# metasnv-tool/metaSNV

Hardware: AMD Instinct MI355X
Metric: pileup Gbases/s across all samples (higher is better)
Workload: dtype u8

## Files before the change

include/msnv.h:

```cpp
#ifndef MSNV_H
#define MSNV_H

#include <stdint.h>

#ifdef __cplusplus
extern "C" {
#endif

#define MSNV_OK        0
#define MSNV_EINVAL    1
#define MSNV_EIO       2
#define MSNV_EFORMAT   3
#define MSNV_ENODEV    4
#define MSNV_EHIP      5
#define MSNV_ENOMEM    6
#define MSNV_EDOMAIN   7
#define MSNV_ECAPACITY 8

typedef struct msnv_ctx     msnv_ctx;
typedef struct msnv_dataset msnv_dataset;

int         msnv_abi_version(void);
const char *msnv_last_error(void);

// ... 104 lines not shown
                                    const msnv_params *params, msnv_dataset **out);
int  msnv_dataset_attach_ctx(msnv_dataset *ds, msnv_ctx *ctx);
void msnv_dataset_destroy(msnv_dataset *ds);

int  msnv_dataset_set_bed(msnv_dataset *ds, int32_t n, const int32_t *tid, const int64_t *beg, const int64_t *end);
int  msnv_dataset_set_bed_file(msnv_dataset *ds, const char *bed_path);
int  msnv_dataset_set_contig_mask(msnv_dataset *ds, const uint8_t *mask, int32_t n);

int  msnv_dataset_add_sample_records(msnv_dataset *ds, const uint8_t *records, uint64_t n_bytes);
int  msnv_dataset_add_sample_records_many(msnv_dataset *ds, const uint8_t *const *records, const uint64_t *n_bytes, int32_t n, int32_t host_threads);
int  msnv_dataset_add_sample_records_device(msnv_dataset *ds, const void *const *dev_records, const uint64_t *n_bytes, int32_t n);
int  msnv_dataset_add_sample_records_resident(msnv_dataset *ds, void *dev_buffer, uint64_t capacity, const uint64_t *offsets, const uint64_t *n_bytes, int32_t n);
int  msnv_dataset_add_sample_bam(msnv_dataset *ds, const char *bam_path);
int  msnv_dataset_add_sample_bams(msnv_dataset *ds, const char *const *bam_paths, int32_t n, int32_t host_threads);

int  msnv_dataset_stage_sample_bams(msnv_dataset *ds, const char *const *bam_paths, int32_t n, int32_t host_threads);

int  msnv_dataset_pileup_qualities(const msnv_dataset *ds, const uint8_t *records, uint64_t n_bytes, uint8_t *out);

int  msnv_dataset_finalize(msnv_dataset *ds);

typedef struct {
    uint64_t n_samples, n_contigs, n_positions;
    uint64_t n_reads, n_reads_pileup;
    uint64_t n_pileup_bases;
    uint64_t bytes_headers, bytes_cigar, bytes_seq, bytes_qual, bytes_ref, bytes_index;
    uint64_t n_tiles, n_pairs, n_work;
    uint64_t device_bytes;
    uint64_t allele_planes;
    uint64_t sampled_mismatch_ppm;
    uint64_t n_whole_tile_items;
    uint64_t n_listed_tiles;
} msnv_dataset_info;

int  msnv_dataset_info_get(const msnv_dataset *ds, msnv_dataset_info *out);
#define MSNV_PACK_STATS 18
int  msnv_dataset_pack_stats(const msnv_dataset *ds, double *out, int32_t n);
int  msnv_dataset_fetch_column(msnv_dataset *ds, const char *name, uint8_t *out, uint64_t capacity, uint64_t *n_bytes);

typedef struct {
    float    ms_total;
    float    ms_pileup;
    float    ms_gate, ms_gather, ms_decide, ms_coverage;
    uint64_t n_sites;
    uint64_t n_called_pop, n_called_indiv;
    uint64_t n_events, n_overflow;
    uint64_t algorithmic_bytes;
} msnv_run_stats;

int  msnv_pileup_run(msnv_dataset *ds, msnv_run_stats *stats);

int  msnv_pileup_run_many(msnv_dataset *ds, int32_t n, int32_t overlap, msnv_run_stats *stats);
int  msnv_pileup_reserve(msnv_dataset *ds, int32_t n);
int  msnv_coverage_run(msnv_dataset *ds, msnv_run_stats *stats);
int  msnv_fused_run(msnv_dataset *ds, msnv_run_stats *pileup_stats, msnv_run_stats *coverage_stats);
int  msnv_write_coverage(msnv_dataset *ds, int32_t sample_idx, const char *cov_path, const char *detail_path);

typedef struct {
    int32_t        want_median;
    int32_t        window;
    uint32_t       n_regions;
    uint32_t       reserved;
    const int32_t *region_contig;
    const int32_t *region_start;
    const int32_t *region_end;
} msnv_cov_extras;
int  msnv_coverage_extras_run(msnv_dataset *ds, const msnv_cov_extras *what);
int  msnv_coverage_medians(msnv_dataset *ds, int32_t *out, uint64_t capacity);
int  msnv_coverage_window_count(const msnv_dataset *ds, uint64_t *n_windows);
int  msnv_coverage_window_sums(msnv_dataset *ds, int32_t sample_idx, uint64_t *out, uint64_t capacity);
int  msnv_coverage_region_sums(msnv_dataset *ds, uint64_t *out, uint64_t capacity);
int  msnv_coverage_extras_launches(const msnv_dataset *ds, uint32_t *n_launches);
typedef struct { const char *contig; int32_t start, end; const char *alias; } msnv_cov_region;
int  msnv_write_coverage_ex(msnv_dataset *ds, int32_t sample_idx, const char *cov_path, const char *detail_path, const char *profile_path,
                            const char *specific_path, const msnv_cov_region *regions, uint32_t n_regions);
typedef struct {
    const char *bam_path;
    int32_t     max_cov;
    int32_t     min_mapq;
    const char *out_cov_path;
    const char *out_detail_path;
    int32_t     want_median;
    int32_t     window;
    const char *out_profile_path;
    const char *regions_path;
    const char *out_specific_path;
} msnv_cov_ex_args;
int  msnv_coverage_ex(msnv_ctx *ctx, const msnv_cov_ex_args *args);

int  msnv_write_calls(msnv_dataset *ds, const char *called_path, const char *indiv_path,
                      const char *ann_path, const char *fasta_path);

typedef struct {
    int32_t  tid;
    int32_t  pos;
    uint32_t cov;
    uint32_t n[4];
    uint8_t  pop_mask;
    uint8_t  ind_mask;
    uint8_t  refchar;
    uint8_t  dropped;
} msnv_site;

typedef struct { uint16_t cov; uint16_t n[4]; } msnv_site_sample;

#define MSNV_ANN_VALID      1
// ... 104 lines not shown
```

metasnv_amd/_lib.py:

```python
import ctypes as C
import os

from . import knobs

_HERE = os.path.dirname(os.path.abspath(__file__))
LIB_PATH = knobs.library() or os.path.join(_HERE, "csrc", "libmsnv.so")


class MsnvError(RuntimeError):
    def __init__(self, code, msg):
        super().__init__("libmsnv error %d: %s" % (code, msg))
        self.code = code


OK, EINVAL, EIO, EFORMAT, ENODEV, EHIP, ENOMEM, EDOMAIN, ECAPACITY = range(9)
DIV, DIV_NS = 0, 1


class Params(C.Structure):
    _fields_ = [("min_coverage", C.c_int32), ("calling_threshold", C.c_int32), ("min_fraction", C.c_double),
                ("min_baseq", C.c_int32), ("flag_filter", C.c_int32), ("count_orphans", C.c_int32),
                ("max_depth", C.c_int32), ("min_mapq", C.c_int32), ("drop_first_line", C.c_int32),
                ("cov_max", C.c_int32), ("cov_min_mapq", C.c_int32), ("ignore_overlaps", C.c_int32), ("token_limit", C.c_int32)]

# ... 75 lines not shown

class BamData(C.Structure):
    _fields_ = [("n_contigs", C.c_int32), ("names", C.POINTER(C.c_char_p)), ("lengths", C.POINTER(C.c_int64)),
                ("records", C.POINTER(C.c_uint8)), ("n_record_bytes", C.c_uint64), ("header_text", C.c_char_p)]


class SynthParams(C.Structure):
    _fields_ = [("n_species", C.c_int32), ("contig_len", C.c_int64), ("n_samples", C.c_int32), ("read_len", C.c_int32),
                ("mean_cov", C.c_double), ("sigma_cov", C.c_double), ("frac_absent", C.c_double),
                ("snv_density", C.c_double), ("error_rate", C.c_double), ("frac_lowq", C.c_double),
                ("frac_indel_reads", C.c_double), ("frac_clip_reads", C.c_double), ("frac_flagged", C.c_double),
                ("lowercase_ref", C.c_int32), ("seed", C.c_uint64), ("frac_paired", C.c_double),
                ("contigs_per_species_max", C.c_int32), ("species_per_sample", C.c_int32),
                ("frac_aux", C.c_double), ("frac_noseq", C.c_double)]


P = C.POINTER
_vp = C.c_void_p
SYMBOLS = [
    ("msnv_abi_version", C.c_int, []),
    ("msnv_last_error", C.c_char_p, []),
    ("msnv_device_count", C.c_int, []),
    ("msnv_ctx_create", C.c_int, [C.c_int, P(_vp)]),
    ("msnv_ctx_destroy", None, [_vp]),
    ("msnv_params_default", None, [P(Params)]),
    ("msnv_coverage", C.c_int, [_vp, P(CovArgs)]),
    ("msnv_call", C.c_int, [_vp, P(CallArgs)]),
    ("msnv_call_from_mpileup", C.c_int, [_vp, P(MpileupArgs), P(C.c_uint64)]),
    ("msnv_bam_records_many", C.c_int, [_vp, P(C.c_char_p), C.c_int32, C.c_int32, P(P(C.c_uint8)), P(C.c_uint64)]),
    ("msnv_bgzf_inflate", C.c_int, [_vp, C.c_char_p, C.c_int32, P(P(C.c_uint8)), P(C.c_uint64), P(C.c_uint64)]),
    ("msnv_dataset_create", C.c_int, [_vp, P(RefDesc), P(Params), P(_vp)]),
    ("msnv_dataset_create_from_files", C.c_int, [_vp, C.c_char_p, C.c_char_p, P(Params), P(_vp)]),
    ("msnv_dataset_attach_ctx", C.c_int, [_vp, _vp]),
    ("msnv_dataset_set_feed_ctx", C.c_int, [_vp, _vp]),
    ("msnv_dataset_destroy", None, [_vp]),
    ("msnv_dataset_set_bed", C.c_int, [_vp, C.c_int32, P(C.c_int32), P(C.c_int64), P(C.c_int64)]),
    ("msnv_dataset_set_bed_file", C.c_int, [_vp, C.c_char_p]),
    ("msnv_dataset_set_contig_mask", C.c_int, [_vp, P(C.c_uint8), C.c_int32]),
    ("msnv_dataset_add_sample_records", C.c_int, [_vp, _vp, C.c_uint64]),
    ("msnv_dataset_add_sample_records_many", C.c_int, [_vp, P(_vp), P(C.c_uint64), C.c_int32, C.c_int32]),
    ("msnv_dataset_stage_sample_bams", C.c_int, [_vp, P(C.c_char_p), C.c_int32, C.c_int32]),
    ("msnv_dataset_add_sample_records_device", C.c_int, [_vp, P(_vp), P(C.c_uint64), C.c_int32]),
    ("msnv_dataset_add_sample_records_resident", C.c_int, [_vp, _vp, C.c_uint64, P(C.c_uint64), P(C.c_uint64), C.c_int32]),
    ("msnv_dataset_pack_stats", C.c_int, [_vp, P(C.c_double), C.c_int32]),
    ("msnv_dataset_fetch_column", C.c_int, [_vp, C.c_char_p, _vp, C.c_uint64, P(C.c_uint64)]),
    ("msnv_dataset_add_sample_bam", C.c_int, [_vp, C.c_char_p]),
    ("msnv_dataset_add_sample_bams", C.c_int, [_vp, P(C.c_char_p), C.c_int32, C.c_int32]),
    ("msnv_dataset_pileup_qualities", C.c_int, [_vp, _vp, C.c_uint64, _vp]),
    ("msnv_dataset_finalize", C.c_int, [_vp]),
    ("msnv_dataset_info_get", C.c_int, [_vp, P(DatasetInfo)]),
    ("msnv_pileup_run", C.c_int, [_vp, P(RunStats)]),
    ("msnv_pileup_run_many", C.c_int, [_vp, C.c_int32, C.c_int32, P(RunStats)]),
    ("msnv_pileup_reserve", C.c_int, [_vp, C.c_int32]),
    ("msnv_host_cores", C.c_int32, []),
    ("msnv_dataset_deal_bams_device", C.c_int, [_vp, P(C.c_char_p), C.c_int32, C.c_int32, P(C.c_int32), C.c_int32, C.c_int32, C.c_void_p, C.c_uint64, C.c_uint64,
                                                P(C.c_uint64), P(SampleStats), P(C.c_uint64)]),
    ("msnv_dataset_inflate_bams_device", C.c_int, [_vp, P(C.c_char_p), C.c_int32, C.c_int32, C.c_void_p, C.c_uint64, P(C.c_uint64), P(C.c_uint64), P(SampleStats), P(C.c_uint64)]),
    ("msnv_records_deal_device", C.c_int, [_vp, P(C.c_void_p), P(C.c_uint64), C.c_int32, C.c_int32, P(C.c_int32), C.c_int32, C.c_int32, C.c_int32, C.c_void_p, C.c_uint64, C.c_uint64,
                                           P(C.c_uint64), P(SampleStats), P(C.c_uint64)]),
    ("msnv_coverage_run", C.c_int, [_vp, P(RunStats)]),
    ("msnv_fused_run", C.c_int, [_vp, P(RunStats), P(RunStats)]),
    ("msnv_write_coverage", C.c_int, [_vp, C.c_int32, C.c_char_p, C.c_char_p]),
    ("msnv_coverage_extras_run", C.c_int, [_vp, P(CovExtras)]),
    ("msnv_coverage_medians", C.c_int, [_vp, P(C.c_int32), C.c_uint64]),
    ("msnv_coverage_window_count", C.c_int, [_vp, P(C.c_uint64)]),
    ("msnv_coverage_window_sums", C.c_int, [_vp, C.c_int32, P(C.c_uint64), C.c_uint64]),
    ("msnv_coverage_region_sums", C.c_int, [_vp, P(C.c_uint64), C.c_uint64]),
    ("msnv_coverage_extras_launches", C.c_int, [_vp, P(C.c_uint32)]),
    ("msnv_write_coverage_ex", C.c_int, [_vp, C.c_int32, C.c_char_p, C.c_char_p, C.c_char_p, C.c_char_p, P(CovRegion), C.c_uint32]),
    ("msnv_coverage_ex", C.c_int, [_vp, P(CovExArgs)]),
    ("msnv_write_calls", C.c_int, [_vp, C.c_char_p, C.c_char_p, C.c_char_p, C.c_char_p]),
    ("msnv_dataset_first_line", C.c_int, [_vp, P(C.c_int32), P(C.c_int32)]),
    ("msnv_dataset_first_lines", C.c_int, [_vp, P(C.c_int32), P(C.c_int32), C.c_int32]),
    ("msnv_write_calls_records", C.c_int, [P(RefDesc), C.c_int32, P(Site), P(SiteSample), C.c_uint64, C.c_char_p, C.c_char_p, C.c_char_p, C.c_char_p, P(SiteAnn)]),
    ("msnv_records_partition", C.c_int, [_vp, C.c_uint64, P(C.c_int32), C.c_int32, C.c_int32, C.c_int32, _vp, P(C.c_uint64), P(SampleStats)]),
    ("msnv_dataset_sample_stats", C.c_int, [_vp, C.c_int32, P(SampleStats)]),
    ("msnv_coverage_fetch", C.c_int, [_vp, P(C.c_uint64), C.c_uint64]),
    ("msnv_coverage_rows_count", C.c_int, [_vp, P(C.c_uint64)]),
    ("msnv_coverage_fetch_rows", C.c_int, [_vp, P(C.c_uint32), P(C.c_uint32), P(C.c_uint64), C.c_uint64]),
    ("msnv_write_coverage_records", C.c_int, [P(RefDesc), C.c_int32, P(SampleStats), P(C.c_uint64), C.c_char_p, C.c_char_p]),
    ("msnv_annotate_run", C.c_int, [_vp, C.c_char_p, C.c_char_p, P(C.c_double)]),
    ("msnv_results_fetch_ann", C.c_int, [_vp, P(SiteAnn), C.c_uint64]),
    ("msnv_results_count", C.c_int, [_vp, P(C.c_uint64)]),
    ("msnv_results_fetch", C.c_int, [_vp, P(Site), P(SiteSample), C.c_uint64]),
    ("msnv_results_cells_count", C.c_int, [_vp, P(C.c_uint64), P(C.c_uint64)]),
    ("msnv_results_fetch_cells", C.c_int, [_vp, P(Site), P(C.c_uint64), P(C.c_uint32), P(SiteSample), C.c_uint64, C.c_uint64]),
    ("msnv_write_calls_cells", C.c_int, [P(RefDesc), C.c_int32, P(Site), P(C.c_uint64), P(C.c_uint32), P(SiteSample), C.c_uint64, C.c_char_p, C.c_char_p,
                                        C.c_char_p, C.c_char_p, P(SiteAnn)]),
    ("msnv_records_contig_bases", C.c_int, [_vp, C.c_uint64, C.c_int32, P(C.c_uint64)]),
    ("msnv_parse_float", C.c_int, [C.c_char_p, P(C.c_double)]),
    ("msnv_dist_file", C.c_int, [_vp, C.c_char_p, C.c_char_p, C.c_char_p, C.c_double, P(C.c_int32), P(C.c_uint64), P(C.c_double)]),
    ("msnv_div_file", C.c_int, [_vp, C.c_char_p, C.c_int32, C.c_int32, C.c_int64, P(C.c_double), P(C.c_double), C.c_int32, P(C.c_int64),
                                C.c_uint64, C.c_char_p, C.c_char_p, P(C.c_int32), P(C.c_uint64), P(C.c_double)]),
    ("msnv_genotyping_subset", C.c_int, [P(C.c_char_p), C.c_int32, P(C.c_char_p), C.c_int32, C.c_char_p, P(C.c_uint64), P(C.c_uint64)]),
    ("msnv_snv_allele_freq", C.c_int, [_vp, C.c_char_p, C.c_int32, P(C.c_uint64), P(C.c_double)]),
    ("msnv_format_float", C.c_int, [C.c_double, C.c_char_p, C.c_int32]),
    ("msnv_filter_files", C.c_int, [_vp, P(C.c_char_p), C.c_int32, C.c_int32, P(FilterSpecies), C.c_int32, C.c_double, C.c_double,
                                   C.c_char_p, P(C.c_uint64), P(C.c_double)]),
    ("msnv_host_stats", C.c_int, [P(C.c_uint64)]),
    ("msnv_host_timers", C.c_int, [P(C.c_double), C.c_int32, C.c_int32]),
    ("msnv_filter_resident", C.c_int, [_vp, C.c_int32, P(FilterSpecies), C.c_int32, C.c_double, C.c_double, C.c_char_p, C.c_char_p, C.c_char_p,
                                      P(C.c_uint64), P(C.c_double)]),
    ("msnv_bam_write_bed_header", C.c_int, [C.c_char_p, C.c_char_p]),
    ("msnv_bam_read", C.c_int, [C.c_char_p, P(BamData)]),
    ("msnv_bam_read_header", C.c_int, [C.c_char_p, P(BamData)]),
    ("msnv_bam_data_free", None, [P(BamData)]),
# ... 37 lines not shown
```

metasnv_amd/core.py:

```python
import ctypes as C

import numpy as np

from . import _lib
from ._lib import lib, check, Params, SynthParams, DatasetInfo, RunStats, Site, SiteSample, SiteAnn, RefDesc, SampleStats, COV_WORDS

SITE_DTYPE = np.dtype([("tid", "<i4"), ("pos", "<i4"), ("cov", "<u4"), ("n", "<u4", (4,)),
                       ("pop_mask", "u1"), ("ind_mask", "u1"), ("refchar", "u1"), ("dropped", "u1")])
SAMPLE_DTYPE = np.dtype([("cov", "<u2"), ("n", "<u2", (4,))])
ANN_DTYPE = np.dtype([("gene", "<i4"), ("codon", "u1", (4, 8))])
STATS_FIELDS = [n for n, _ in SampleStats._fields_]
assert SITE_DTYPE.itemsize == C.sizeof(Site) and SAMPLE_DTYPE.itemsize == C.sizeof(SiteSample) and ANN_DTYPE.itemsize == C.sizeof(SiteAnn)


def default_params(**kw):
    p = Params()
    lib.msnv_params_default(C.byref(p))
    for k, v in kw.items():
        if not hasattr(p, k):
            raise AttributeError("msnv_params has no field %r" % k)
        setattr(p, k, v)
    return p


# ... 158 lines not shown
        return out

    def add_sample_bam(self, path):
        check(lib.msnv_dataset_add_sample_bam(self._h, path.encode()))
        self.n_samples += 1

    def add_sample_bams(self, paths, host_threads=0):
        arr = _cstr_array(paths)
        check(lib.msnv_dataset_add_sample_bams(self._h, arr, len(paths), host_threads))
        self.n_samples += len(paths)

    def stage_sample_bams(self, paths, host_threads=0):
        arr = _cstr_array(paths)
        check(lib.msnv_dataset_stage_sample_bams(self._h, arr, len(paths), host_threads))
        self.n_samples += len(paths)

    def add_synth_samples(self, synth_p, first, count, host_threads=0):
        check(lib.msnv_dataset_add_synth_samples(self._h, C.byref(synth_p), first, count, host_threads))
        self.n_samples += count

    def finalize(self):
        check(lib.msnv_dataset_finalize(self._h))
        return self.info()

    def info(self):
        i = DatasetInfo()
        check(lib.msnv_dataset_info_get(self._h, C.byref(i)))
        return {k: getattr(i, k) for k, _ in DatasetInfo._fields_}

    PACK_STATS = ["scan_ms", "measure_ms", "depth_ms", "emit_ms", "tile_sort_ms", "upload_wall_s", "download_wall_s", "host_prepass_wall_s",
                  "record_bytes", "records", "pieces", "prepass_samples", "scan_segments_redone", "deep_runs_split", "dense_samples", "quick_rounds_redone", "device_edit_samples",
                  "columns_adopted"]

    def pack_stats(self):
        a = (C.c_double * len(self.PACK_STATS))()
        check(lib.msnv_dataset_pack_stats(self._h, a, len(self.PACK_STATS)))
        return dict(zip(self.PACK_STATS, [float(x) for x in a]))

    def column(self, name):
        n = C.c_uint64()
        check(lib.msnv_dataset_fetch_column(self._h, name.encode(), None, 0, C.byref(n)))
        out = np.zeros(n.value, dtype=np.uint8)
        if n.value:
            check(lib.msnv_dataset_fetch_column(self._h, name.encode(), out.ctypes.data, out.size, C.byref(n)))
        return out

    def run(self):
        st = RunStats()
        check(lib.msnv_pileup_run(self._h, C.byref(st)))
        return {k: getattr(st, k) for k, _ in RunStats._fields_}

    def reserve_passes(self, n):
        check(lib.msnv_pileup_reserve(self._h, int(n)))

    def run_many(self, n, overlap=False):
        arr = (RunStats * n)()
        check(lib.msnv_pileup_run_many(self._h, n, 1 if overlap else 0, arr))
        return [{k: getattr(s, k) for k, _ in RunStats._fields_} for s in arr]

    def coverage_run(self):
        st = RunStats()
        check(lib.msnv_coverage_run(self._h, C.byref(st)))
        return {k: getattr(st, k) for k, _ in RunStats._fields_}

    def fused_run(self):
        sp, sc = RunStats(), RunStats()
        check(lib.msnv_fused_run(self._h, C.byref(sp), C.byref(sc)))
        return ({k: getattr(sp, k) for k, _ in RunStats._fields_}, {k: getattr(sc, k) for k, _ in RunStats._fields_})

    def coverage_accumulators(self):
        acc = np.zeros((max(1, self.n_samples), len(self.names), COV_WORDS), dtype=np.uint64)
        check(lib.msnv_coverage_fetch(self._h, acc.ctypes.data_as(C.POINTER(C.c_uint64)), acc.size))
        return acc

    def coverage_rows(self):
        n = C.c_uint64()
        check(lib.msnv_coverage_rows_count(self._h, C.byref(n)))
        smp, ctg = np.zeros(n.value, dtype=np.uint32), np.zeros(n.value, dtype=np.uint32)
        acc = np.zeros((n.value, COV_WORDS), dtype=np.uint64)
        check(lib.msnv_coverage_fetch_rows(self._h, smp.ctypes.data_as(C.POINTER(C.c_uint32)), ctg.ctypes.data_as(C.POINTER(C.c_uint32)),
                                           acc.ctypes.data_as(C.POINTER(C.c_uint64)), n.value))
        return smp, ctg, acc

    def sample_stats(self, sample_idx):
        st = SampleStats()
        check(lib.msnv_dataset_sample_stats(self._h, sample_idx, C.byref(st)))
        return np.array([getattr(st, k) for k in STATS_FIELDS], dtype=np.uint32)

    def write_coverage(self, sample_idx, cov_path, detail_path, profile_path=None, specific_path=None, regions=None):
        if profile_path is None and specific_path is None and not getattr(self, "_extras_median", False):
            check(lib.msnv_write_coverage(self._h, sample_idx, cov_path.encode(), detail_path.encode()))
            return
        regions = list(regions or [])
        arr = (_lib.CovRegion * max(1, len(regions)))()
        for i, (name, start, end, alias) in enumerate(regions):
            arr[i] = _lib.CovRegion(name.encode(), int(start), int(end), alias.encode())
        check(lib.msnv_write_coverage_ex(self._h, sample_idx, cov_path.encode(), detail_path.encode(),
                                         profile_path.encode() if profile_path is not None else None,
                                         specific_path.encode() if specific_path is not None else None, arr, len(regions)))

    def coverage_extras(self, median=False, window=0, regions=None):
        regions = [(self.names.index(c) if isinstance(c, str) else int(c), int(s), int(e)) for c, s, e in (regions or [])]
        cols = [np.ascontiguousarray([r[k] for r in regions], dtype=np.int32) for k in range(3)]
        what = _lib.CovExtras(1 if median else 0, int(window), len(regions), 0, *[c.ctypes.data_as(C.POINTER(C.c_int32)) for c in cols])
        check(lib.msnv_coverage_extras_run(self._h, C.byref(what)))
        self._extras_median = bool(median)
# ... 318 lines not shown
```

metasnv_amd/csrc/api.cpp:

```cpp
#include <algorithm>
#include <chrono>
#include <climits>
#include <cstring>
#include <stdexcept>
#include <thread>
#include <unordered_map>

#include "bamfeed.h"
#include "devpack.h"
#include "filter.h"

using namespace msnv;

extern "C" int msnv_abi_version(void) { return 3; }

extern "C" void msnv_params_default(msnv_params *p) {
    if (!p) return;
    p->min_coverage = 4; p->calling_threshold = 4; p->min_fraction = 0.01;
    p->min_baseq = 13; p->flag_filter = 0x704; p->count_orphans = 0; p->max_depth = 8000; p->min_mapq = 0;
    p->drop_first_line = 1;
    p->cov_max = 10; p->cov_min_mapq = 1;
    p->ignore_overlaps = 0;
    p->token_limit = 10000;
}
// ... 463 lines not shown
    HostTimerScope ts(HT_UPLOAD_WALL);
    try { return finalize_dataset(*ds); }
    catch (const std::exception &e) { return fail(MSNV_ENOMEM, "building the device dataset failed: %s", e.what()); }
}

extern "C" int msnv_dataset_pack_stats(const msnv_dataset *ds, double *out, int32_t n) {
    clear_error();
    if (!ds || !out || n < 0) return fail(MSNV_EINVAL, "msnv_dataset_pack_stats: bad argument");
    if (devpack_sync_pending(*const_cast<msnv_dataset *>(ds))) clear_error();
    const DevPackTables &t = ds->dp;
    const double v[MSNV_PACK_STATS] = {t.ms_scan, t.ms_measure, t.ms_depth, t.ms_emit, t.ms_sort, t.wall_upload_s, t.wall_download_s, t.wall_prepass_s,
                                       (double)t.raw_bytes, (double)t.n_records, (double)t.n_pieces, (double)t.n_prepass_samples, (double)t.n_scan_redone, (double)t.n_deep_runs_split, (double)t.n_dense_samples, (double)t.n_quick_redone, (double)t.n_device_edit_samples,
                                       (double)t.n_columns_adopted};
    for (int i = 0; i < n; ++i) out[i] = i < MSNV_PACK_STATS ? v[i] : 0.0;
    return MSNV_OK;
}

extern "C" int msnv_dataset_fetch_column(msnv_dataset *ds, const char *name, uint8_t *out, uint64_t capacity, uint64_t *n_bytes) {
    clear_error();
    if (!ds || !name || !n_bytes) return fail(MSNV_EINVAL, "msnv_dataset_fetch_column: NULL argument");
    if (!ds->finalized || !ds->dev) return fail(MSNV_EINVAL, "msnv_dataset_fetch_column: dataset is not finalized");
    if (int rc = dev_set_device(ds->ctx->device)) return rc;
    const DeviceCols &d = *ds->dev;
    const std::string k(name);
    const void *p = nullptr; uint64_t n = 0;
    const uint64_t S = d.n_samples, nt = d.n_tiles;
    if (k == "hdr") { p = d.hdr; n = d.n_reads * sizeof(ReadHdr); }
    else if (k == "hdr4") { p = d.hdr4; n = d.hdr4 ? d.n_reads * 4 : 0; }
    else if (k == "hdr8m") { p = d.hdr8m; n = d.n_hdr8m * sizeof(PieceHdr); }
    else if (k == "blk") { p = d.blk; n = d.blk ? d.n_blk * 4 : 0; }
    else if (k == "seq") { p = d.seq; n = d.n_seq_bytes; }
    else if (k == "qual") { p = d.qual; n = d.n_seq_bytes / 4; }
    else if (k == "s_read_base") { p = d.s_read_base; n = (S + 1) * 8; }
    else if (k == "s_seq_base") { p = d.s_seq_base; n = (S + 1) * 8; }
    else if (k == "ref4") { p = d.ref4; n = (nt * TILE / 8 + 1) * 4; }
    else if (k == "pairs") { p = d.pairs; n = (uint64_t)d.n_pairs * sizeof(TilePair); }
    else if (k == "work") { p = d.work; n = (uint64_t)d.n_work * sizeof(WorkItem); }
    else if (k == "chunks") { p = d.chunks; n = d.n_chunks * sizeof(ChunkDesc); }
    else if (k == "cov_iv") { p = d.cov_iv; n = d.n_cov_iv * sizeof(Pair32); }
    else if (k == "cov_pairs") { p = d.cov_pairs; n = (uint64_t)d.n_cov_pairs * sizeof(TilePair); }
    else if (k == "cov_work") { p = d.cov_work; n = (uint64_t)d.n_cov_work * sizeof(WorkItem); }
    else return fail(MSNV_EINVAL, "msnv_dataset_fetch_column: no column named %s", name);
    *n_bytes = n;
    if (!out) return MSNV_OK;
    if (capacity < n) return fail(MSNV_ECAPACITY, "msnv_dataset_fetch_column: %s holds %llu bytes, capacity %llu", name, (unsigned long long)n, (unsigned long long)capacity);
    if (n && !p) return fail(MSNV_EINVAL, "msnv_dataset_fetch_column: %s is not allocated in this layout", name);
    return dev_download(out, p, n);
}

extern "C" int msnv_dataset_info_get(const msnv_dataset *ds, msnv_dataset_info *out) {
    clear_error();
    if (!ds || !out) return fail(MSNV_EINVAL, "msnv_dataset_info_get: NULL argument");
    *out = ds->info;
    if (ds->dev) { out->n_whole_tile_items = ds->dev->n_fused_tiles; out->n_listed_tiles = ds->dev->last_ovf_tiles; }
    return MSNV_OK;
}

extern "C" int msnv_pileup_reserve(msnv_dataset *ds, int32_t n) {
    clear_error();
    if (!ds || !ds->finalized || n <= 0) return fail(MSNV_EINVAL, "msnv_pileup_reserve: dataset is not finalized or n <= 0");
    if (int rc = dev_set_device(ds->ctx->device)) return rc;
    return dev_reserve_passes(*ds->dev, n);
}

extern "C" int msnv_pileup_run_many(msnv_dataset *ds, int32_t n, int32_t overlap, msnv_run_stats *stats) {
    clear_error();
    if (!ds || !ds->finalized || n <= 0) return fail(MSNV_EINVAL, "msnv_pileup_run_many: dataset is not finalized or n <= 0");
    if (!ds->have_results) return fail(MSNV_EINVAL, "msnv_pileup_run_many: run msnv_pileup_run once first (it sizes the sparse buffers)");
    if (int rc = dev_set_device(ds->ctx->device)) return rc;
    RunCounts c{};
    std::vector<msnv_run_stats> tmp((size_t)n);
    int rc = dev_run_pipeline_many(*ds->dev, ds->params, ds->ctx->stream, n, overlap != 0, tmp.data(), &c);
    if (rc == MSNV_ECAPACITY) return fail(rc, "%s", msnv_last_error());
    if (rc) return rc;
    ds->have_results = true; ds->results_fetched = false; ds->ann_valid = false;
    ds->last_counts_sites = c.n_sites;
    ds->last_stats = tmp.back();
    if (stats) memcpy(stats, tmp.data(), tmp.size() * sizeof(msnv_run_stats));
    return MSNV_OK;
}

static void gpos_to_contig(const msnv_dataset &ds, uint32_t gpos, int32_t &tid, int32_t &pos) {
    const uint32_t tile = gpos / TILE;
    tid = (int32_t)ds.tile_contig[tile];
    pos = (int32_t)(gpos - ds.tile_base[(size_t)tid] * TILE);
}

extern "C" int msnv_pileup_run(msnv_dataset *ds, msnv_run_stats *stats) {
    clear_error();
    if (!ds || !ds->finalized) return fail(MSNV_EINVAL, "msnv_pileup_run: dataset is not finalized");
    if (int rc = dev_set_device(ds->ctx->device)) return rc;
    DeviceCols &d = *ds->dev;
    msnv_run_stats st{};
    RunCounts c{};
    int rc = dev_run_pipeline(d, ds->params, ds->ctx->stream, &st, &c);
    for (int attempt = 0; rc == MSNV_ECAPACITY && attempt < 3; ++attempt) {
        auto grow = [&](void **p, uint32_t &cap, uint32_t need, size_t elem) -> int {
            if (need <= cap) return MSNV_OK;
            dev_free(*p); *p = nullptr;
            cap = (uint32_t)std::min<uint64_t>(0x7fffffffull, (uint64_t)need + need / 4 + 1024);
            return dev_alloc(p, (uint64_t)cap * elem, &d.device_bytes);
        };
        if (int r2 = grow((void **)&d.events, d.cap_events, c.n_events, sizeof(Pair32))) return r2;
        if (int r2 = grow((void **)&d.overflow, d.cap_overflow, c.n_overflow, sizeof(Pair32))) return r2;
        const uint32_t old_cap_sites = d.cap_sites;
        if (int r2 = grow((void **)&d.sites, d.cap_sites, c.n_sites, sizeof(SiteRec))) return r2;
        if (d.cap_sites != old_cap_sites) {
            dev_free(d.unc_sites); d.unc_sites = nullptr;
            if (int r2 = dev_alloc((void **)&d.unc_sites, (uint64_t)d.cap_sites * sizeof(uint32_t), &d.device_bytes)) return r2;
        }
        clear_error();
        rc = dev_run_pipeline(d, ds->params, ds->ctx->stream, &st, &c);
    }
    if (rc == MSNV_ECAPACITY) return fail(rc, "%s", msnv_last_error());
    if (rc) return rc;

    ds->have_results = true;
    ds->results_fetched = false;
    ds->ann_valid = false;
    ds->last_counts_sites = c.n_sites;
    ds->last_stats = st;
    if (stats) *stats = st;
    return MSNV_OK;
}

static int fetch_results(msnv_dataset *ds) {
    if (ds->results_fetched) return MSNV_OK;
    DeviceCols &d = *ds->dev;
    const uint32_t n = ds->last_counts_sites;
    std::vector<SiteRec> sites(n);
    std::vector<uint8_t> flags(n);
    std::vector<uint32_t> tbase(ds->n_tiles + 1), tcnt(ds->n_tiles + 1);
    if (int r2 = dev_download(sites.data(), d.sites, (uint64_t)n * sizeof(SiteRec))) return r2;
    if (int r2 = dev_download(flags.data(), d.site_flags, n)) return r2;
    if (int r2 = dev_download(tbase.data(), d.tile_site_base, (uint64_t)ds->n_tiles * 4)) return r2;
    if (int r2 = dev_download(tcnt.data(), d.tile_site_cnt, (uint64_t)ds->n_tiles * 4)) return r2;
    std::vector<unsigned long long> tcell(ds->n_tiles + 1);
    if (int r2 = dev_download(tcell.data(), d.tile_cell_base, (uint64_t)ds->n_tiles * sizeof(unsigned long long))) return r2;
    const uint64_t n_cells = d.last_cells;
    std::vector<msnv_site_sample> raw((size_t)n_cells);
    {
        std::vector<uint16_t> col((size_t)n_cells);
        if (int r2 = dev_download(col.data(), d.cov_col, col.size() * sizeof(uint16_t))) return r2;
        for (size_t i = 0; i < raw.size(); ++i) raw[i].cov = col[i];
        for (int x = 0; x < 4; ++x) {
            if (int r2 = dev_download(col.data(), d.ncol + (uint64_t)x * d.cap_cells, col.size() * sizeof(uint16_t))) return r2;
            for (size_t i = 0; i < raw.size(); ++i) raw[i].n[x] = col[i];
        }
    }

    ds->sites.clear(); ds->site_samples.clear(); ds->site_dev_index.clear();
    ds->site_row.clear(); ds->site_cell_sample.clear(); ds->site_cells.clear();
    ds->sites.reserve(n);
    ds->site_row.push_back(0);
    for (uint32_t t = 0; t < ds->n_tiles; ++t) {
// ... 620 lines not shown
```

metasnv_amd/csrc/device.h:

```cpp
#pragma once

#include <cstdint>

#include <string>
#include <vector>

#include "dataset.h"

namespace msnv {

struct Pair32 { uint32_t x, y; };
struct MergedGroupDev { uint64_t hdr_base; uint32_t tile, pair_lo, n_pairs, n_pieces; };

constexpr uint8_t ANN_GENE_MINUS = 1, ANN_GENE_LINEAR = 2;
struct AnnGene   { int64_t start; int32_t contig; uint32_t flags; };
struct AnnContig { int64_t cg_base, cg_len; uint32_t goff, pad; };
struct AnnHost {
    std::vector<uint32_t> seg_beg, seg_end;
    std::vector<int32_t>  seg_gene;
    std::vector<AnnGene>  genes;
    std::vector<AnnContig> contigs;
    std::vector<uint8_t>  codons;
};
struct AnnDev {
    uint32_t *seg_beg = nullptr, *seg_end = nullptr; int32_t *seg_gene = nullptr;
    AnnGene *genes = nullptr; AnnContig *contigs = nullptr; uint8_t *codons = nullptr;
    uint32_t n_seg = 0;
    msnv_site_ann *out = nullptr; uint64_t cap_out = 0;
    uint32_t *err = nullptr;
    bool ready = false;
    std::string key;
    std::vector<std::string> gene_names;
};
int  ann_build(msnv_dataset &ds, const Annotation &an, AnnHost &h);
void ann_gene_names(const Annotation &an, const std::vector<std::string> &contigs, std::vector<std::string> &out);
int  dev_ann_upload(DeviceCols &d, const AnnHost &h);
int  dev_annotate(DeviceCols &d, uint32_t n_sites, uint32_t drop_gpos, void *stream, double *ms, uint32_t err_gpos[2]);

struct DeviceCols {
    ReadHdr  *hdr = nullptr;
    PieceHdr *hdr8 = nullptr;
    uint32_t *hdr4 = nullptr;
    PieceHdr *hdr8m = nullptr;
    uint32_t *tile_pair_merged = nullptr;
    uint32_t  n_work_merged = 0;
    MergedGroupDev *merged_groups = nullptr; uint32_t n_merged_groups = 0;
    uint32_t *blk = nullptr;
    bool      dense = true;
    uint8_t  *seq = nullptr;
    uint8_t  *qual = nullptr;
    uint64_t *s_read_base = nullptr, *s_seq_base = nullptr;
    uint32_t *ref4 = nullptr;
    uint32_t *ref_lc = nullptr;
    TilePair *pairs = nullptr;
    uint32_t *tile_pair_start = nullptr;
    WorkItem *work = nullptr;
    ChunkDesc *chunks = nullptr;
    uint32_t *tile_vbeg = nullptr, *tile_vend = nullptr;
    uint32_t  n_tiles = 0, n_pairs = 0, n_work = 0, n_work_narrow = 0, n_samples = 0;
    uint64_t  n_reads = 0, n_seq_bytes = 0, n_chunks = 0, n_hdr8m = 0, n_blk = 0;
    uint32_t *tot = nullptr;
    uint32_t *active_tiles = nullptr;
    uint32_t  n_active_tiles = 0;
    uint8_t  *part = nullptr;
    uint64_t *slot_off = nullptr;
    uint32_t *tile_slot_u16 = nullptr;
    uint32_t *tile_slot_wide = nullptr;
    uint64_t  part_bytes = 0;
    uint32_t *tile_slot_start = nullptr;
    uint8_t  *spill = nullptr;
    uint8_t  *aspill = nullptr;
    bool      allele_planes = false;
    Pair32   *events = nullptr;
    Pair32   *overflow = nullptr;
    uint32_t *counters = nullptr;
    uint32_t  cnt_parity = 0;
    uint32_t *ind4 = nullptr;
    uint32_t *unc_bits = nullptr;
    uint32_t *tile_dirty = nullptr;
    uint32_t *unc_sites = nullptr;
    struct GateTileH { uint32_t tile, slot_lo, slot_16, slot_w, slot_hi, vbeg, vend, n_slots; uint64_t row0; uint32_t tot_mode, staged, pair_lo, n_plane_pairs, pad0, pad1; } *gate_tiles = nullptr;
    unsigned long long *site_row = nullptr;
    GateTileH *gate_tiles_dense = nullptr, *gate_tiles_staged = nullptr;
    uint32_t *gather_tiles = nullptr; uint32_t n_gather_tiles = 0;
    TileStage *tile_stage = nullptr;
    uint32_t *tile_stage_idx = nullptr;
    uint32_t  max_group_pairs = 0;
    uint32_t  n_groups_solo = 0;
    uint32_t  n_work_fused = 0;
    uint32_t  n_fused_tiles = 0;
    bool      fuse_disabled = false;
    int       qlow_cutoff = 0;
    uint32_t  last_ovf_tiles = 0;
    bool      wide_tot = false;
    bool      use_dirty = false;
    uint32_t  gather_split = 4;
    bool      any_split = false;
    unsigned long long *site_bits = nullptr;
    uint32_t *site_rank = nullptr;
    uint32_t  cap_events = 0, cap_overflow = 0, cap_sites = 0;
    SiteRec  *sites = nullptr;
    uint32_t *tile_site_base = nullptr, *tile_site_cnt = nullptr;
    uint32_t *tile_nslots = nullptr;
    unsigned long long *tile_cell_base = nullptr;
    uint64_t  cap_cells = 0, last_cells = 0;
    uint16_t *ncol = nullptr;
    uint16_t *cov_col = nullptr;
    uint8_t  *site_flags = nullptr;
    uint8_t  *site_elig = nullptr;
    uint64_t  cap_out_sites = 0, last_sites = 0;
    Pair32   *cov_iv = nullptr;
    uint64_t *s_cov_base = nullptr;
    TilePair *cov_pairs = nullptr;
    WorkItem *cov_work = nullptr;
    uint32_t *tile_len = nullptr;
    uint32_t *tile_contig_dev = nullptr;
    unsigned long long *cov_acc = nullptr;
    uint64_t  n_cov_rows = 0;
    uint32_t  cov_copies = 1;
    uint32_t  n_cov_pairs = 0, n_cov_work = 0, n_cov_work_wide = 0, n_contigs = 0;
    uint64_t  n_cov_iv = 0;
    uint64_t  device_bytes = 0;
    uint64_t  algorithmic_bytes = 0;
    std::vector<std::pair<void *, uint64_t>> blocks;
    AnnDev    ann;
    struct AltBufs {
        uint32_t *tot = nullptr; uint8_t *part = nullptr; uint8_t *spill = nullptr, *aspill = nullptr; Pair32 *events = nullptr, *overflow = nullptr;
        TileStage *tile_stage = nullptr;
        uint32_t *counters = nullptr; SiteRec *sites = nullptr; uint32_t *tile_site_base = nullptr, *tile_site_cnt = nullptr; unsigned long long *tile_cell_base = nullptr;
        uint16_t *ncol = nullptr; uint16_t *cov_col = nullptr; uint8_t *site_flags = nullptr, *site_elig = nullptr; uint32_t *ind4 = nullptr, *unc_bits = nullptr, *tile_dirty = nullptr, *unc_sites = nullptr; unsigned long long *site_row = nullptr; unsigned long long *site_bits = nullptr; uint32_t *site_rank = nullptr;
        uint32_t cap_events = 0, cap_overflow = 0, cap_sites = 0, cnt_parity = 0; uint64_t cap_out_sites = 0, cap_cells = 0;
    } alt;
    void     *stream2 = nullptr;
    std::vector<void *> event_pool;
    uint32_t *pinned_cnt = nullptr; size_t pinned_cnt_cap = 0;
    void     *timing_events[6] = {nullptr, nullptr, nullptr, nullptr, nullptr, nullptr};
};

constexpr uint32_t EV_LISTS = 32, EV_CNT_STRIDE = 16;
constexpr uint32_t CNT_CELLS = 16 + EV_LISTS * EV_CNT_STRIDE;
constexpr uint32_t CNT_TALLY = CNT_CELLS + 16;
constexpr uint32_t CNT_UNC = CNT_TALLY + 16;
constexpr uint32_t CNT_STAGE = CNT_UNC + 8;
constexpr uint32_t CNT_WORDS = CNT_UNC + 16;

struct RunCounts { uint32_t n_events, n_overflow, n_sites, err; uint64_t n_cells; };

int  dev_set_device(int device);
uint32_t dev_resident_workgroups(uint32_t per_cu);
int  dev_alloc(void **p, uint64_t bytes, uint64_t *acct);
void dev_free(void *p);
void dev_free_batch(const std::vector<void *> &ptrs);
int dev_memset_async(void *dst, int v, uint64_t bytes, void *stream);
void dev_cache_trim();
int  dev_upload(void *dst, const void *src, uint64_t bytes);
int  dev_download(void *dst, const void *src, uint64_t bytes);
int  dev_copy_bytes(void *dst_device, const void *src, uint64_t bytes, bool src_on_device, void *stream);
int  dev_memset(void *dst, int v, uint64_t bytes);
int  dev_stream_wait(void *stream);
int  dev_stream_create(void **stream);
void dev_stream_destroy(void *stream);

constexpr int COV_BINS = 16;
int  dev_run_coverage(DeviceCols &d, int max_cov, void *stream, msnv_run_stats *stats);
int  dev_coverage_scanned(DeviceCols &d, void *stream, unsigned long long *scanned);
constexpr uint32_t CX_BINS = 2048, CX_ROW_WORDS = CX_BINS + 2;
struct CovxRegion { uint32_t start, end, max_end, id; };
struct CovxJob {
    bool want_median = false; uint32_t window = 0, n_samples = 0;
    std::vector<uint32_t> contig_tile_base;
    std::vector<uint32_t> row_contig;
    std::vector<uint64_t> row_len, row_scanned, row_win_off;
    std::vector<CovxRegion> regs; std::vector<uint32_t> reg_off;
    std::vector<int32_t> row_median; std::vector<uint64_t> win, reg_sum;
    uint32_t n_launches = 0;
};
int  dev_run_coverage_extras(DeviceCols &d, CovxJob &job, void *stream);
int  dev_run_pipeline(DeviceCols &d, const msnv_params &p, void *stream, msnv_run_stats *stats, RunCounts *counts);
int  dev_run_pipeline_many(DeviceCols &d, const msnv_params &p, void *stream, int n, bool overlap, msnv_run_stats *stats, RunCounts *counts);
void dev_free_all(DeviceCols &d);
int  dev_reserve_passes(DeviceCols &d, int n);
void warm_devpack(void *stream), warm_kernels(void *stream), warm_textcall(void *stream), warm_annotate(void *stream);

struct InfBlock { unsigned long long in_off, out_off; uint32_t in_size, out_size; };
int  dev_inflate_staging(msnv_ctx *ctx, uint64_t in_bytes, uint64_t out_bytes, uint8_t **in, uint8_t **out);
void dev_inflate_release(msnv_ctx *ctx);
void dev_inflate_release_device(msnv_ctx *ctx);
int  dev_inflate(msnv_ctx *ctx, uint64_t comp_bytes, const std::vector<InfBlock> &blocks, uint64_t out_bytes, std::vector<uint32_t> &status, double *ms_kernel);
int  dev_inflate_device_buffers(msnv_ctx *ctx, uint64_t in_bytes, uint64_t out_bytes);
int  dev_inflate_resident(msnv_ctx *ctx, const uint8_t *host_in, uint64_t comp_bytes, const std::vector<InfBlock> &blocks, const std::vector<uint32_t> &blk_in_file,
                          uint32_t check_every, std::vector<uint32_t> &status, double *ms_kernel);
int  dev_inflate_patch(msnv_ctx *ctx, uint64_t out_off, const uint8_t *data, uint32_t n);

int  text_call(msnv_ctx *ctx, const char *text, uint64_t n_text, const msnv_params &p, const char *ref_fasta, const char *ann_path,
               const char *called_path, const char *indiv_path, uint64_t stats[8]);
int  dist_file(msnv_ctx *ctx, const char *freq_path, const char *mann_path, const char *allele_path, double threshold,
               int32_t *n_samples_out, uint64_t *n_pos_out, double *ms_kernel);
int  div_file(msnv_ctx *ctx, const char *freq_path, int32_t mode, int32_t matched, int64_t genome_length, const double *h, const double *v,
              int32_t n_cov, const int64_t *row_order, uint64_t n_order, const char *out_a, const char *out_b, int32_t *n_samples_out,
              uint64_t *n_rows_out, double *ms_kernel);
int dev_dist(const double *xt_host, int n_samples, long n_pos, double threshold, void *stream, double *mann, double *allele, double *ms_kernel);
int dev_div(const double *xs, const uint64_t *bits, long n_single, long n_words, const double *xg, const long *goff, long n_groups, long n_grouped,
            int n_samples, void *stream, double *out, double *ms_kernel);
int dev_allele_freq(const std::vector<uint32_t> &cov, const std::vector<uint32_t> &cnt, const std::vector<uint32_t> &row_line,
                    uint32_t n_samples, long long min_depth, void *stream, std::vector<double> &freq, double *ms_kernel);

}
```

metasnv_amd/csrc/kernels.hip:

```cpp
#include <hip/hip_runtime.h>

#include <algorithm>
#include <cstdio>
#include <cstdlib>
#include <cstring>
#include <mutex>
#include <unordered_map>
#include <vector>

#include "device.h"

namespace msnv {

#define HIP_TRY(expr)                                                                         \
    do {                                                                                      \
        hipError_t e_ = (expr);                                                               \
        if (e_ != hipSuccess) return fail(MSNV_EHIP, "%s failed: %s", #expr, hipGetErrorString(e_)); \
    } while (0)

constexpr int LANES_PER_READ = 8;
static_assert(LANES_PER_READ * 16 == SEG_MAX, "segment pieces are sized for 8 lanes of 16 bases");

struct PileupArgs {
    const ReadHdr  *hdr;
    const uint32_t *blk;
    const PieceHdr *hdr8;
    const uint32_t *hdr4;
    const PieceHdr *hdr8m;
    uint32_t        n_narrow;
    const uint8_t  *seq;
    const uint8_t  *qual;
    const uint64_t *s_read_base, *s_seq_base;
    const uint32_t *ref4;
    const TilePair *pairs;
    const WorkItem *work;
    const ChunkDesc *chunks;
    uint32_t       *tot;
    uint8_t        *part;
    uint64_t        npos;
    uint8_t        *spill;
    uint8_t        *aspill;
    Pair32         *events;   uint32_t cap_events;
    Pair32         *overflow; uint32_t cap_overflow;
    uint32_t       *counters;
    uint32_t       *ev_count;
    uint32_t        min_baseq;
    uint32_t       *ind4;
    uint32_t       *unc_bits;
    uint32_t       *slot_dirty;
    uint32_t        min_snvs;
    uint32_t        n_fused_lo;
    int             min_cov; double min_frac;
    const uint32_t *ref_lc, *tile_vbeg, *tile_vend, *tile_stage_idx;
    TileStage      *tile_stage;
    uint32_t       *stage_ovf;
};

__device__ __forceinline__ uint32_t allele_index(uint32_t code) {
    return (code == 1u) ? 0u : (code == 2u) ? 1u : (code == 4u) ? 2u : (code == 8u) ? 3u : 4u;
}
__device__ __forceinline__ uint32_t nz_bytes(uint32_t x) {
    return (((x & 0x7f7f7f7fu) + 0x7f7f7f7fu) | x) & 0x80808080u;
}
__device__ __forceinline__ uint32_t count_nz_bytes(const uint4 a, const uint4 b) {
    return (uint32_t)__popc(nz_bytes(a.x) | nz_bytes(a.y) >> 1 | nz_bytes(a.z) >> 2 | nz_bytes(a.w) >> 3 |
                            nz_bytes(b.x) >> 4 | nz_bytes(b.y) >> 5 | nz_bytes(b.z) >> 6 | nz_bytes(b.w) >> 7);
}
__device__ __forceinline__ uint32_t nz_nibbles(uint32_t x) {
    return (((x & 0x77777777u) + 0x77777777u) | x) & 0x88888888u;
}
__device__ __forceinline__ uint32_t nibflags_to_bits(uint32_t f) {
    const uint32_t e = f & 0x08080808u, o = (f >> 4) & 0x08080808u;
    return (__builtin_amdgcn_udot4(o, 0x80200802u, __builtin_amdgcn_udot4(e, 0x40100401u, 0u, false), false)) >> 3;
}
__device__ __forceinline__ uint4 any_uint4() {
    uint4 v;
    asm volatile("" : "=v"(v.x), "=v"(v.y), "=v"(v.z), "=v"(v.w));
    return v;
}
__device__ __forceinline__ uint2 lowq_fetch(const uint8_t *qlow, const uint64_t bit) {
    uint2 v;
    __builtin_memcpy(&v, qlow + (bit >> 3), 8);
    return v;
}
__device__ __forceinline__ uint32_t lowq_bits(const uint2 v, const uint32_t shift) {
    return (uint32_t)(((unsigned long long)v.y << 32 | v.x) >> shift);
}

template <int CTRL, int ROW_MASK>
__device__ __forceinline__ int dpp_add(int x) {
    return x + __builtin_amdgcn_update_dpp(0, x, CTRL, ROW_MASK, 0xf, false);
}
__device__ __forceinline__ int wave_inclusive_scan(int x) {
    x = dpp_add<0x111, 0xf>(x);
    x = dpp_add<0x112, 0xf>(x);
    x = dpp_add<0x114, 0xf>(x);
    x = dpp_add<0x118, 0xf>(x);
    x = dpp_add<0x142, 0xa>(x);
    x = dpp_add<0x143, 0xc>(x);
    return x;
}

__device__ __forceinline__ uint32_t tot_mode_of(const WorkItem &w) { return (w.part_lo >> 1) & 3u; }
__device__ __forceinline__ void tot_add(uint32_t *tot, const uint32_t mode, const uint32_t t0, const uint32_t p, const uint32_t n0, const uint32_t n1,
                                        const uint32_t n2, const uint32_t n3) {
    uint32_t *base = tot + 4ull * t0;
    if (mode == 0u) atomicAdd(base + p, n0 | n1 << 8 | n2 << 16 | n3 << 24);
    else if (mode == 1u) {
        if (n0 | n1) atomicAdd(base + 2u * p, n0 | n1 << 16);
        if (n2 | n3) atomicAdd(base + 2u * p + 1u, n2 | n3 << 16);
    } else {
        if (n0) atomicAdd(base + 4u * p, n0);
        if (n1) atomicAdd(base + 4u * p + 1u, n1);
        if (n2) atomicAdd(base + 4u * p + 2u, n2);
        if (n3) atomicAdd(base + 4u * p + 3u, n3);
    }
}
__device__ __forceinline__ void tot_add_one(uint32_t *tile_tot, const uint32_t mode, const uint32_t p, const uint32_t x, const uint32_t n) {
    const uint32_t shpack = mode == 0u ? 0x18100800u : mode == 1u ? 0x10001000u : 0u;
    const uint32_t byte_off = ((p << mode) + (x >> (2u - mode))) * 4u;
    atomicAdd(reinterpret_cast<uint32_t *>(reinterpret_cast<char *>(tile_tot) + byte_off), n << ((shpack >> (8u * x)) & 0xffu));
}

constexpr int W_NT = 512;
constexpr int W_PPT = TILE / W_NT;
constexpr int W_HCAP = 256;
constexpr int W_EVCAP = 1024;
static_assert(W_PPT == 4, "wide per-sample pass is written for 4 positions per thread");

struct WideLds {
    int32_t  span[TILE + 4];
    uint32_t exc[TILE / 2];
    unsigned long long al[TILE];
    uint32_t ref[TILE / 8 + 4];
    uint4    hdr[2][W_HCAP];
    Pair32   ev[W_EVCAP];
    int32_t  wsum[W_NT / 64];
    uint32_t evn, ev_base;
};

__device__ __forceinline__ void ev_list(PileupArgs &a) {
    const uint32_t k = blockIdx.x % EV_LISTS;
    a.events += (uint64_t)k * a.cap_events;
    a.ev_count = a.counters + 16u + k * EV_CNT_STRIDE;
}

template <typename LDS, int NT, int CAP>
__device__ __forceinline__ void flush_events(LDS &L, const PileupArgs &a, int tid) {
    const uint32_t n = min(L.evn, (uint32_t)CAP);
    if (tid == 0) L.ev_base = n ? atomicAdd(a.ev_count, n) : 0u;
    __syncthreads();
    const uint32_t base = L.ev_base;
    for (uint32_t i = tid; i < n; i += NT)
        if (base + i < a.cap_events) a.events[base + i] = L.ev[i];
    __syncthreads();
    if (tid == 0) L.evn = 0;
}

template <typename LDS, int CAP>
__device__ __forceinline__ void stage_allele_event(LDS &L, const PileupArgs &a, Pair32 e) {
    const uint32_t i = atomicAdd(&L.evn, 1u);
    if (i < (uint32_t)CAP) { L.ev[i] = e; return; }
    const uint32_t g = atomicAdd(a.ev_count, 1u);
    if (g < a.cap_events) a.events[g] = e;
}

__device__ __forceinline__ void wide_classify(WideLds &L, const uint32_t lq, const uint32_t s0, const uint32_t s1,
                                              const uint32_t P0, const uint32_t vmask) {
    const uint32_t pr = P0;
    const uint32_t wi = pr >> 3, sh = (pr & 7u) * 4u;
    const uint32_t w0 = L.ref[wi], w1 = L.ref[wi + 1], w2 = L.ref[wi + 2];
    const uint32_t r0 = __builtin_amdgcn_alignbit(w1, w0, sh), r1 = __builtin_amdgcn_alignbit(w2, w1, sh);
    const uint32_t nm = nibflags_to_bits(nz_nibbles(s0 ^ r0)) | nibflags_to_bits(nz_nibbles(s1 ^ r1)) << 8;
    uint32_t e = (lq | nm) & vmask;
    while (e) {
        const uint32_t j = (uint32_t)__builtin_ctz(e);
        e &= e - 1u;
        const uint32_t p = P0 + j;
        uint32_t ai = 4u;
        if (!((lq >> j) & 1u)) ai = allele_index(((j < 8u ? s0 : s1) >> (4u * (j & 7u))) & 0xfu);
        if (ai < 4u) atomicAdd(&L.al[p], 1ull << (16u * ai));
        else atomicAdd(&L.exc[p >> 1], 1u << (16u * (p & 1u)));
    }
}

__global__ __launch_bounds__(W_NT) void msnv_pileup_tiles_wide(PileupArgs a) {
    ev_list(a);
    __shared__ WideLds L;
    const WorkItem w = a.work[blockIdx.x];
    const uint32_t t0 = w.tile * TILE;
    const int tid = threadIdx.x, lane = tid & 63, wave = tid >> 6;
    const int lane8 = tid & (LANES_PER_READ - 1), grp = tid / LANES_PER_READ;
    const int b0 = 16 * lane8;

    for (int i = tid; i < (int)(TILE / 8 + 4); i += W_NT)
        L.ref[i] = (i < (int)(TILE / 8)) ? a.ref4[(t0 >> 3) + i] : 0xffffffffu;
    for (int i = tid; i < (int)(TILE + 4); i += W_NT) L.span[i] = 0;
    for (int i = tid; i < (int)(TILE / 2); i += W_NT) L.exc[i] = 0;
    for (int i = tid; i < (int)TILE; i += W_NT) L.al[i] = 0;
    if (tid == 0) L.evn = 0;

    uint32_t tc[W_PPT], tn[W_PPT][4];
#pragma unroll
    for (int j = 0; j < W_PPT; ++j) { tc[j] = 0; tn[j][0] = tn[j][1] = tn[j][2] = tn[j][3] = 0; }

    uint32_t k = w.pair_lo;
    TilePair pr = (k < w.pair_hi) ? a.pairs[k] : TilePair{0, 0, 0, 0};
    uint32_t rbeg = pr.read_lo;
    uint4 hreg = make_uint4(0, 0, 0, 0);
    if (k < w.pair_hi && tid < W_HCAP && rbeg + (uint32_t)tid < pr.read_hi)
        hreg = *reinterpret_cast<const uint4 *>(a.hdr + a.s_read_base[pr.sample] + rbeg + tid);
    int buf = 0;

    while (k < w.pair_hi) {
        const uint32_t nrd = min((uint32_t)W_HCAP, pr.read_hi - rbeg);
        const bool last_chunk = rbeg + nrd >= pr.read_hi;
        const uint32_t sample = pr.pad >> 8;
        if (tid < W_HCAP) L.hdr[buf][tid] = hreg;
        uint32_t nk = k, nrbeg = rbeg + nrd;
        TilePair npr = pr;
        if (last_chunk) { nk = k + 1; if (nk < w.pair_hi) { npr = a.pairs[nk]; nrbeg = npr.read_lo; } }
        hreg = make_uint4(0, 0, 0, 0);
        if (nk < w.pair_hi && tid < W_HCAP && nrbeg + (uint32_t)tid < npr.read_hi)
            hreg = *reinterpret_cast<const uint4 *>(a.hdr + a.s_read_base[npr.sample] + nrbeg + tid);
        __syncthreads();

        const uint8_t *seq = a.seq + a.s_seq_base[pr.sample];
        const uint64_t qbit0 = 2ull * a.s_seq_base[pr.sample];
        for (uint32_t r = (uint32_t)grp; r < nrd; r += W_NT / LANES_PER_READ) {
            const uint4 h = L.hdr[buf][r];
            if (!(h.w & META_PILEUP_OK)) continue;
            const uint32_t s = h.x - t0, len = h.z;
            if (lane8 == 0) { atomicAdd(&L.span[s], 1); atomicAdd(&L.span[s + len], -1); }
            const int vhi = min(max((int)len - b0, 0), 16);
            if (vhi <= 0) continue;
            uint2 sv;
            const uint64_t qbit = qbit0 + 2ull * h.y + (uint32_t)b0;
            const uint2 qv = lowq_fetch(a.qual, qbit);
            __builtin_memcpy(&sv, seq + (uint64_t)h.y + (uint32_t)(b0 >> 1), 8);
            wide_classify(L, lowq_bits(qv, (uint32_t)qbit & 7u), sv.x, sv.y, s + (uint32_t)b0, (1u << vhi) - 1u);
        }

// ... 41 lines not shown
                }
            }
            *reinterpret_cast<uint32_t *>(a.spill + (uint64_t)k * TILE + W_PPT * tid) = packed;
        }
        k = nk; pr = npr; rbeg = nrbeg; buf ^= 1;
        if (last_chunk && k < w.pair_hi) {
            __syncthreads();
            if (L.evn >= (uint32_t)(W_EVCAP / 2)) flush_events<WideLds, W_NT, W_EVCAP>(L, a, tid);
        }
    }
    __syncthreads();
    flush_events<WideLds, W_NT, W_EVCAP>(L, a, tid);

    *reinterpret_cast<uint4 *>(a.part + ((uint64_t)w.part_hi << 32 | (w.part_lo & ~15u)) + 4u * W_PPT * tid) = make_uint4(tc[0], tc[1], tc[2], tc[3]);
    bool any_allele = false;
#pragma unroll
    for (int j = 0; j < W_PPT; ++j) {
        if (tn[j][0] | tn[j][1] | tn[j][2] | tn[j][3]) {
            tot_add(a.tot, tot_mode_of(w), t0, W_PPT * tid + j, tn[j][0], tn[j][1], tn[j][2], tn[j][3]);
            any_allele = true;
        }
    }
    if (any_allele && tot_mode_of(w) != 0u) atomicOr(&a.slot_dirty[w.slot], 1u << ((W_PPT * (uint32_t)tid) >> 6));
}

__device__ __forceinline__ unsigned long long spread_bits(const uint32_t byte) {
    return (unsigned long long)(__umul24(byte >> 4, 0x00204081u) & 0x01010101u) << 32 | (__umul24(byte & 0xfu, 0x00204081u) & 0x01010101u);
}

constexpr int N_NT = 256;
constexpr int N_PPT = TILE / N_NT;
constexpr int N_HCAP = CHUNK_READS;
#if !defined(MSNV_N_EVCAP)
#define MSNV_N_EVCAP 224
#endif
#if !defined(MSNV_N32_WAVES)
#define MSNV_N32_WAVES 8
#endif
constexpr int N_EVCAP = MSNV_N_EVCAP;

static_assert(N_PPT == 8, "narrow per-sample pass is written for 8 positions per thread");

struct alignas(16) NarrowLds {
    uint32_t start[TILE / 4 + 4];
    uint32_t end[TILE / 4 + 4];
    unsigned long long exc[TILE / 8 + 4];
    uint32_t al[TILE];
    uint32_t ref[TILE / 8 + 4];
    uint2    hdr[2][N_HCAP];
    Pair32   ev[N_EVCAP];
    ChunkDesc desc[MAX_CHUNKS_PER_ITEM];
    uint32_t carry[N_NT / 64 + 1];
    uint32_t evn, ev_base;
    uint32_t emask[SEQ_ALIGN_LOG2 < 3 ? 33 : 1];
};

template <typename LDS, int EXC_PAD, bool MERGED = false, bool FUSED = false, bool DA = false>
__device__ __forceinline__ void narrow_pass(LDS &L, const PileupArgs &a, uint32_t (&tc)[N_PPT / 2], bool &dirty, const uint32_t t0,
                                            const int tid, const int lane, const int wave, const uint32_t sample, const uint32_t k,
                                            const uint32_t split, const uint32_t tmode) {
    const uint2 st = *reinterpret_cast<uint2 *>(&L.start[2 * tid]);
    const uint2 en = *reinterpret_cast<uint2 *>(&L.end[2 * tid]);
    const uint2 ex = *reinterpret_cast<uint2 *>(&L.exc[EXC_PAD + tid]);
    int d = (int)L.carry[wave];
    *reinterpret_cast<uint2 *>(&L.start[2 * tid]) = make_uint2(0u, 0u);
    *reinterpret_cast<uint2 *>(&L.end[2 * tid]) = make_uint2(0u, 0u);
    L.exc[EXC_PAD + tid] = 0ull;
    if (lane == 0) L.carry[wave] = 0u;
    if (tid == 0) L.end[TILE / 4] = 0;
    const int mine = (int)(__builtin_amdgcn_udot4(st.x, 0x01010101u, __builtin_amdgcn_udot4(st.y, 0x01010101u, 0u, false), false)) -
                     (int)(__builtin_amdgcn_udot4(en.x, 0x01010101u, __builtin_amdgcn_udot4(en.y, 0x01010101u, 0u, false), false));
    d += wave_inclusive_scan(mine) - mine;
    const uint32_t v0 = ((uint32_t)d + st.x - en.x) * 0x01010101u;
    const uint32_t v1 = ((v0 >> 24) + st.y - en.y) * 0x01010101u;
    const uint32_t c0 = v0 - ex.x, c1 = v1 - ex.y;
    tc[0] += c0 & 0x00ff00ffu; tc[1] += (c0 >> 8) & 0x00ff00ffu;
    tc[2] += c1 & 0x00ff00ffu; tc[3] += (c1 >> 8) & 0x00ff00ffu;
    if (!MERGED) *reinterpret_cast<uint2 *>(a.spill + (uint64_t)k * TILE + N_PPT * tid) = make_uint2(c0, c1);
    if (MERGED && FUSED) {
        *reinterpret_cast<uint2 *>(&L.start[2 * tid]) = make_uint2(c0, c1);
        return;
    }
    if constexpr (DA && !MERGED) {
        uint32_t *row = reinterpret_cast<uint32_t *>(a.aspill) + (uint64_t)k * TILE + N_PPT * tid;
        const uint32_t ge = (0x80u - min(a.min_snvs, 127u)) * 0x01010101u;
#pragma unroll
        for (uint32_t half = 0; half < 2u; ++half) {
            const uint4 v = *reinterpret_cast<uint4 *>(&L.al[N_PPT * tid + 4u * half]);
            const uint32_t w4[4] = {v.x, v.y, v.z, v.w};
            *reinterpret_cast<uint4 *>(row + 4u * half) = v;
            if (!(v.x | v.y | v.z | v.w)) continue;
            *reinterpret_cast<uint4 *>(&L.al[N_PPT * tid + 4u * half]) = make_uint4(0u, 0u, 0u, 0u);
            dirty = true;
            uint32_t todo = 0;
#pragma unroll
            for (uint32_t j = 0; j < 4u; ++j) todo |= (split ? w4[j] != 0u : ((((w4[j] & 0x7f7f7f7fu) + ge) | w4[j]) & 0x80808080u) != 0u) ? 1u << j : 0u;
            while (todo) {
                const uint32_t j = (uint32_t)__builtin_ctz(todo);
                todo &= todo - 1u;
                const uint32_t word = j == 0u ? w4[0] : j == 1u ? w4[1] : j == 2u ? w4[2] : w4[3];
                const uint32_t gpos = t0 + N_PPT * tid + 4u * half + j;
#pragma unroll
                for (uint32_t x = 0; x < 4u; ++x) {
                    const uint32_t n = (word >> (8u * x)) & 0xffu;
                    if (n >= a.min_snvs) atomicOr(&a.ind4[gpos >> 3], 1u << (4u * (gpos & 7u) + x));
                    else if (n && split) atomicOr(&a.unc_bits[gpos >> 5], 1u << (gpos & 31u));
                }
            }
        }
        return;
    }
    uint32_t pm = 0, myev;
    {
        const uint4 a0 = *reinterpret_cast<uint4 *>(&L.al[N_PPT * tid]);
        const uint4 a1 = *reinterpret_cast<uint4 *>(&L.al[N_PPT * tid + 4]);
        const uint32_t alw[N_PPT] = {a0.x, a0.y, a0.z, a0.w, a1.x, a1.y, a1.z, a1.w};
#pragma unroll
        for (int j = 0; j < N_PPT; ++j) pm |= (alw[j] ? 1u : 0u) << j;
        myev = count_nz_bytes(a0, a1);
    }
    if (!__any(pm != 0u)) return;
    dirty |= pm != 0u;
    if (MERGED) {
        while (pm) {
            const uint32_t j = (uint32_t)__builtin_ctz(pm);
            pm &= pm - 1u;
            const uint32_t word = L.al[N_PPT * tid + j];
            L.al[N_PPT * tid + j] = 0u;
            const uint32_t gpos = t0 + N_PPT * tid + j;
            for (uint32_t m = nz_bytes(word); m; m &= m - 1u) {
                const uint32_t x = (uint32_t)__builtin_ctz(m) >> 3;
                const uint32_t n = (word >> (8u * x)) & 0xffu;
                tot_add_one(a.tot + 4ull * t0, tmode, N_PPT * tid + j, x, n);
                if (n >= a.min_snvs) atomicOr(&a.unc_bits[gpos >> 5], 1u << (gpos & 31u));
            }
        }
        return;
    }
    const uint32_t ei = (uint32_t)wave_inclusive_scan((int)myev);
    uint32_t res = 0;
    if (lane == 63 && ei) {
        uint32_t cur = atomicAdd(&L.evn, 0u);
        for (;;) {
            if (cur + ei > (uint32_t)N_EVCAP) { res = 0x80000000u | atomicAdd(a.ev_count, ei); break; }
            const uint32_t seen = atomicCAS(&L.evn, cur, cur + ei);
            if (seen == cur) { res = cur; break; }
            cur = seen;
        }
    }
    res = (uint32_t)__builtin_amdgcn_readlane((int)res, 63);
    const bool direct = (res & 0x80000000u) != 0u;
    uint32_t slot = (res & 0x7fffffffu) + ei - myev;
    while (pm) {
        const uint32_t j = (uint32_t)__builtin_ctz(pm);
        pm &= pm - 1u;
        const uint32_t word = L.al[N_PPT * tid + j];
        L.al[N_PPT * tid + j] = 0u;
        const uint32_t gpos = t0 + N_PPT * tid + j;
        for (uint32_t m = nz_bytes(word); m; m &= m - 1u) {
            const uint32_t x = (uint32_t)__builtin_ctz(m) >> 3;
            const uint32_t n = (word >> (8u * x)) & 0xffu;
            tot_add_one(a.tot + 4ull * t0, tmode, N_PPT * tid + j, x, n);
            if (n >= a.min_snvs) atomicOr(&a.ind4[gpos >> 3], 1u << (4u * (gpos & 7u) + x));
            else if (split) atomicOr(&a.unc_bits[gpos >> 5], 1u << (gpos & 31u));
            const Pair32 e{gpos, sample << 18 | x << 16 | n};
            if (direct) { if (slot < a.cap_events) a.events[slot] = e; }
            else L.ev[slot] = e;
            ++slot;
        }
    }
}

__device__ __forceinline__ void store_part_row(uint8_t *part, const WorkItem &w, const uint32_t (&tc)[N_PPT / 2], const int tid) {
    uint8_t *row = part + ((uint64_t)w.part_hi << 32 | (w.part_lo & ~15u));
    if (w.part_lo & 1u) {
        const uint32_t lo = (tc[0] & 0xffu) | (tc[1] & 0xffu) << 8 | (tc[0] >> 16 & 0xffu) << 16 | (tc[1] >> 16) << 24;
        const uint32_t hi = (tc[2] & 0xffu) | (tc[3] & 0xffu) << 8 | (tc[2] >> 16 & 0xffu) << 16 | (tc[3] >> 16) << 24;
        *reinterpret_cast<uint2 *>(row + N_PPT * tid) = make_uint2(lo, hi);
    } else {
        *reinterpret_cast<uint4 *>(row + 2u * N_PPT * tid) =
            make_uint4((tc[0] & 0xffffu) | tc[1] << 16, tc[0] >> 16 | (tc[1] & 0xffff0000u), (tc[2] & 0xffffu) | tc[3] << 16, tc[2] >> 16 | (tc[3] & 0xffff0000u));
    }
}

__device__ __forceinline__ void store_item_dirty(uint32_t *slot_dirty, const WorkItem &w, const bool dirty, const int tid) {
    if (tot_mode_of(w) == 0u) return;
    const unsigned long long b = __ballot(dirty);
    uint32_t byte = 0;
#pragma unroll
    for (int i = 0; i < 8; ++i) byte |= ((b >> (8 * i)) & 0xffull) ? 1u << i : 0u;
    if ((tid & 63) == 0 && byte) atomicOr(&slot_dirty[w.slot], byte << (8 * (tid >> 6)));
}

__device__ __forceinline__ void desc_refill(ChunkDesc *ring, const ChunkDesc *src, const uint32_t c, const uint32_t nch, const int tid) {
    constexpr uint32_t H = MAX_CHUNKS_PER_ITEM / 2;
    if (c == 0u || (c % H) != 0u || c + H >= nch) return;
    const uint32_t first = c + H, n = min(H, nch - first);
    if ((uint32_t)tid < 2u * n) {
        const uint32_t d = first + (uint32_t)tid / 2u;
        reinterpret_cast<uint4 *>(ring + d % MAX_CHUNKS_PER_ITEM)[tid & 1] = reinterpret_cast<const uint4 *>(src + d)[tid & 1];
    }
}

constexpr int N32_LANES = 4;
constexpr int N32_GROUPS = N_NT / N32_LANES;
constexpr int N32_ROUNDS = N_HCAP / N32_GROUPS;
static_assert(N32_LANES * 32 == SEG_MAX && N32_ROUNDS == 2, "narrow32 is written for 128-base pieces, 128-piece chunks");

__device__ __forceinline__ void narrow_classify32(NarrowLds &L, const uint32_t lq_all, const uint4 sq, const uint32_t P0, const int vhi) {
    const uint32_t wi = P0 >> 3, sh = (P0 & 7u) * 4u;
    const uint32_t w0 = L.ref[wi], w1 = L.ref[wi + 1], w2 = L.ref[wi + 2], w3 = L.ref[wi + 3], w4 = L.ref[wi + 4];
    const uint32_t vmask = (vhi >= 32) ? 0xffffffffu : ((1u << vhi) - 1u);
    const uint32_t lq = lq_all & vmask;
    const unsigned long long m = (unsigned long long)lq << (P0 & 7u);
#pragma unroll
    for (int w = 0; w < 5; ++w) {
        const uint32_t byte = (uint32_t)(m >> (8 * w)) & 0xffu;
        if (byte) atomicAdd(&L.exc[wi + w], spread_bits(byte));
    }
// ... 52 lines not shown
#pragma unroll
            for (int x = 0; x < 4; ++x) {
                if ((int)n[x] < (int)a.min_snvs) continue;
                const bool is_pop = (double)n[x] >= lim;
                ok = true;
                if (lc && rc == (1u << x)) continue;
                if (is_pop) pop |= 1u << x;
                else if (a.solo) ind |= 1u << x;
                else elig |= 1u << x;
            }
            if (!ok) continue;
            const uint32_t slot = atomicAdd(&L.evn, 1u);
            if (slot < STAGE_CAP) st->rec[slot] = StageRec{p | (elig ? 1u << 11 : 0u) | (pop | ind << 4) << 16 | elig << 24, cov, word, 0u};
        }
    }
counted:
    __syncthreads();
    const uint32_t n_cand = L.evn;
    if (tid == 0) st->count = n_cand;
    return n_cand > STAGE_CAP;
}

__device__ __attribute__((noinline)) void fused_tile_spill(NarrowLds &L, const FusedSpillArgs a, const uint32_t t0, const int tid) {
    {
        WorkItem w{};
        w.slot = 0u; w.part_lo = a.flags_snvs & 15u; w.part_hi = 0u;
        const uint2 cv = *reinterpret_cast<uint2 *>(&L.start[2 * tid]);
        const uint32_t tc[N_PPT / 2] = {cv.x & 0x00ff00ffu, (cv.x >> 8) & 0x00ff00ffu, cv.y & 0x00ff00ffu, (cv.y >> 8) & 0x00ff00ffu};
        store_part_row(a.row, w, tc, tid);
        const uint32_t tmode = tot_mode_of(w);
        bool dirty = false;
#pragma unroll 1
        for (uint32_t j = 0; j < (uint32_t)N_PPT; ++j) {
            const uint32_t word = L.al[N_PPT * tid + j];
            if (!word) continue;
            dirty = true;
            const uint32_t gpos = t0 + N_PPT * tid + j;
#pragma unroll
            for (uint32_t x = 0; x < 4; ++x) {
                const uint32_t n = (word >> (8u * x)) & 0xffu;
                if (n) {
                    tot_add_one(a.tot + 4ull * t0, tmode, N_PPT * tid + j, x, n);
                    if (n >= (a.flags_snvs >> 4)) atomicOr(&a.unc_bits[gpos >> 5], 1u << (gpos & 31u));
                }
            }
        }
        store_item_dirty(a.item_dirty, w, dirty, tid);
        if (tid == 0) a.stage_ovf[atomicAdd(&a.counters[CNT_STAGE], 1u)] = a.stage_idx;
    }
}

template <bool MERGED, bool FUSED = false, bool DA = false>
__device__ __forceinline__ void pileup_tiles_narrow32_body(PileupArgs a, NarrowLds &L) {
    ev_list(a);
    const WorkItem w = a.work[blockIdx.x];
    const uint32_t t0 = w.tile * TILE;
    const int tid = threadIdx.x, lane = tid & 63, wave = tid >> 6;
    const int lane4 = tid & (N32_LANES - 1), grp = tid / N32_LANES;
    const int b0 = 32 * lane4;

    for (int i = tid; i < (int)(TILE / 8 + 4); i += N_NT)
        L.ref[i] = (i < (int)(TILE / 8)) ? a.ref4[(t0 >> 3) + i] : 0xffffffffu;
    {
        static_assert(offsetof(NarrowLds, start) == 0 && offsetof(NarrowLds, ref) % 16 == 0 && alignof(NarrowLds) >= 16, "the bins are zeroed as 16-byte words");
        constexpr int n16 = (int)(offsetof(NarrowLds, ref) / 16);
        uint4 *z = reinterpret_cast<uint4 *>(&L);
#pragma unroll
        for (int i = 0; i < (n16 + N_NT - 1) / N_NT; ++i) if (i * N_NT + tid < n16) z[i * N_NT + tid] = make_uint4(0u, 0u, 0u, 0u);
    }
    if (tid == 0) L.evn = 0;
    if (tid < N_NT / 64 + 1) L.carry[tid] = 0;
    if constexpr (SEQ_ALIGN_LOG2 < 3) {
        if (tid < 33) {
            uint32_t m = 0;
#pragma unroll
            for (int k = 0; k < 4; ++k) {
                const int c = min(max(tid - 8 * k, 0), 8);
                m |= (c >= 8 ? 0xffffffffu : (1u << (4 * c)) - 1u) & (0x11111111u << k);
            }
            L.emask[tid] = m;
        }
    }
    uint32_t tc[N_PPT / 2] = {0u, 0u, 0u, 0u};
    bool dirty = false;

    const uint32_t nch = w.chunk_hi - w.chunk_lo;
    constexpr bool fused = MERGED && FUSED;
    uint32_t g_sidx = 0, g_vb = 0, g_ve = 0, g_lcb = 0;
    if constexpr (fused) {
        g_sidx = a.tile_stage_idx[w.tile]; g_vb = a.tile_vbeg[w.tile]; g_ve = a.tile_vend[w.tile];
        g_lcb = reinterpret_cast<const uint8_t *>(a.ref_lc)[(t0 >> 3) + (uint32_t)tid];
    }
    constexpr bool H4 = HDR4 && !MERGED;
    auto fetch_hdr = [&](const uint64_t hdr_base) -> uint2 {
        if constexpr (H4) return make_uint2(a.hdr4[hdr_base + (uint32_t)tid], 0u);
        else return *reinterpret_cast<const uint2 *>(a.hdr8 + hdr_base + tid);
    };
    auto put_hdr = [&](const uint32_t buf, const uint2 h) {
        if constexpr (H4) reinterpret_cast<uint32_t *>(L.hdr[buf])[tid] = h.x; else L.hdr[buf][tid] = h;
    };
    auto get_hdr = [&](const uint32_t buf, const uint32_t i) -> uint2 {
        if constexpr (H4) return make_uint2(reinterpret_cast<const uint32_t *>(L.hdr[buf])[i], 0u); else return L.hdr[buf][i];
    };
    uint2 hreg0 = make_uint2(0, 0);
    if (nch && tid < N_HCAP && (uint32_t)tid < (w.first.nrd_flags & 0xffffu)) hreg0 = fetch_hdr(w.first.hdr_base);
    for (uint32_t i = tid; i < min(nch, (uint32_t)MAX_CHUNKS_PER_ITEM) * 2; i += N_NT)
        reinterpret_cast<uint4 *>(L.desc)[i] = reinterpret_cast<const uint4 *>(a.chunks + w.chunk_lo)[i];
    __syncthreads();
// ... 216 lines not shown
                const bool is_pop = (double)n[x] >= lim;
                ok = true;
                if (lc && rc == (1u << x)) continue;
                if (is_pop) pop |= 1u << x;
                else if (solo) ind |= 1u << x;
                else elig |= 1u << x;
            }
            if (ok) {
                const uint32_t slot = atomicAdd(&L.ev_base, 1u);
                if (slot < STAGE_CAP) st->rec[slot] = StageRec{p | (elig ? 1u << 11 : 0u) | (pop | ind << 4) << 16 | elig << 24, cov, word, 0u};
            }
        }
    }
    __syncthreads();
    const uint32_t n_rec = L.ev_base;
    if (n_rec > STAGE_CAP) return false;
    if (tid == 0) st->count = n_rec;
    return true;
}
__global__ __launch_bounds__(N_NT, MSNV_N32_WAVES) void msnv_pileup_tiles_lean(PileupArgs a) {
    __shared__ NarrowLds L;
    a.hdr8 = a.hdr8m;
    a.work += a.n_fused_lo;
    const WorkItem w = a.work[blockIdx.x];
    const uint32_t nch = w.chunk_hi - w.chunk_lo;
    if (nch >= 1u && nch <= LEAN_MAX_CHUNKS && a.min_snvs >= 1u && a.min_snvs <= 127u && lean_tile(a, L, w, nch)) return;
    __syncthreads();
    pileup_tiles_narrow32_body<true, true>(a, L);
}

__global__ __launch_bounds__(N_NT, MSNV_N32_WAVES) void msnv_pileup_tiles_narrow32(PileupArgs a) {
    __shared__ NarrowLds L;
    if (blockIdx.x < a.n_narrow) pileup_tiles_narrow32_body<false>(a, L);
    else if (blockIdx.x < a.n_fused_lo) { a.hdr8 = a.hdr8m; pileup_tiles_narrow32_body<true>(a, L); }
    else { a.hdr8 = a.hdr8m; pileup_tiles_narrow32_body<true, true>(a, L); }
}
__global__ __launch_bounds__(N_NT, MSNV_N32_WAVES) void msnv_pileup_tiles_narrow32_planes(PileupArgs a) {
    __shared__ NarrowLds L;
    if (blockIdx.x < a.n_narrow) pileup_tiles_narrow32_body<false, false, true>(a, L);
    else if (blockIdx.x < a.n_fused_lo) { a.hdr8 = a.hdr8m; pileup_tiles_narrow32_body<true>(a, L); }
    else { a.hdr8 = a.hdr8m; pileup_tiles_narrow32_body<true, true>(a, L); }
}
constexpr int D_PAD = 4;
struct DenseLds {
    uint32_t start[TILE / 4 + 4];
    uint32_t end[TILE / 4 + 4];
    unsigned long long exc[TILE / 8 + D_PAD + 8];
    uint32_t al[TILE];
    uint32_t ref[TILE / 8 + D_PAD + 8];
    Pair32   ev[N_EVCAP];
    ChunkDesc desc[MAX_CHUNKS_PER_ITEM];
    uint32_t carry[N_NT / 64 + 1];
    uint32_t evn, ev_base;
};

__device__ __forceinline__ uint32_t range_nibbles(const int lo, const int hi, const int k) {
    const int h = min(max(hi - 8 * k, 0), 8), l = min(max(lo - 8 * k, 0), 8);
    const uint32_t below_h = (h == 8) ? 0xffffffffu : ((1u << (4 * h)) - 1u);
    const uint32_t below_l = (l == 8) ? 0xffffffffu : ((1u << (4 * l)) - 1u);
    return below_h & ~below_l & 0x88888888u;
}

__device__ __forceinline__ void dense_segment(DenseLds &L, const uint4 sq, const uint32_t lq, const uint32_t P, const int lo, const int hi) {
    const uint32_t wi = P >> 3, sh = (P & 7u) * 4u;
    const uint32_t below_hi = (hi >= 32) ? 0xffffffffu : ((1u << hi) - 1u);
    const uint32_t below_lo = (lo >= 32) ? 0xffffffffu : ((1u << lo) - 1u);
    const uint32_t lqm = lq & below_hi & ~below_lo;
    const unsigned long long m = (unsigned long long)lqm << (P & 7u);
#pragma unroll
    for (int w = 0; w < 5; ++w) {
        const uint32_t byte = (uint32_t)(m >> (8 * w)) & 0xffu;
        if (byte) atomicAdd(&L.exc[wi + w], spread_bits(byte));
    }
    const uint32_t w0 = L.ref[wi], w1 = L.ref[wi + 1], w2 = L.ref[wi + 2], w3 = L.ref[wi + 3], w4 = L.ref[wi + 4];
    const uint32_t sw[4] = {sq.x, sq.y, sq.z, sq.w};
    const uint32_t rw[4] = {__builtin_amdgcn_alignbit(w1, w0, sh), __builtin_amdgcn_alignbit(w2, w1, sh),
                            __builtin_amdgcn_alignbit(w3, w2, sh), __builtin_amdgcn_alignbit(w4, w3, sh)};
    uint32_t e[4];
#pragma unroll
    for (int k = 0; k < 4; ++k) e[k] = nz_nibbles(sw[k] ^ rw[k]) & range_nibbles(lo, hi, k);
    uint32_t E = (e[0] >> 3) | (e[1] >> 2) | (e[2] >> 1) | e[3];
    while (E) {
        const uint32_t b = (uint32_t)__builtin_ctz(E);
        E &= E - 1u;
        const uint32_t k = b & 3u, j = (b >> 2) + 8u * k;
        const unsigned long long pair = (k & 2u) ? ((unsigned long long)sw[3] << 32 | sw[2]) : ((unsigned long long)sw[1] << 32 | sw[0]);
        if ((lq >> j) & 1u) continue;
        const uint32_t code = (uint32_t)(pair >> (((b & 1u) << 5) | (b & 28u))) & 0xfu;
        const uint32_t pp = P + j;
        if ((code & (code - 1u)) == 0u) atomicAdd(&L.al[pp - 32u], __umul24(code, 0x00204081u) & 0x01010101u);
        else atomicAdd(&L.exc[pp >> 3], 1ull << (8u * (pp & 7u)));
    }
}

__global__ __launch_bounds__(N_NT) void msnv_pileup_tiles_dense(PileupArgs a) {
    ev_list(a);
    __shared__ DenseLds L;
    const WorkItem w = a.work[blockIdx.x];
    const uint32_t t0 = w.tile * TILE;
    const int tid = threadIdx.x, lane = tid & 63, wave = tid >> 6;

    for (int i = tid; i < (int)(TILE / 8 + D_PAD + 8); i += N_NT) {
        const int r = i - D_PAD;
        L.ref[i] = (r >= 0 && r < (int)(TILE / 8)) ? a.ref4[(t0 >> 3) + r] : 0xffffffffu;
        L.exc[i] = 0;
    }
    for (int i = tid; i < (int)(TILE / 4 + 4); i += N_NT) { L.start[i] = 0; L.end[i] = 0; }
    for (int i = tid; i < (int)TILE; i += N_NT) L.al[i] = 0;
    if (tid == 0) L.evn = 0;
    if (tid < N_NT / 64 + 1) L.carry[tid] = 0;
    uint32_t tc[N_PPT / 2] = {0u, 0u, 0u, 0u};
    bool dirty = false;

    const uint32_t nch = w.chunk_hi - w.chunk_lo;
    for (uint32_t i = tid; i < min(nch, (uint32_t)MAX_CHUNKS_PER_ITEM) * 2; i += N_NT)
        reinterpret_cast<uint4 *>(L.desc)[i] = reinterpret_cast<const uint4 *>(a.chunks + w.chunk_lo)[i];
    __syncthreads();
    constexpr int ROUNDS = DENSE_CHUNK_BLOCKS / N_NT;
    uint32_t dnext[ROUNDS];
#pragma unroll
    for (int r = 0; r < ROUNDS; ++r) {
        dnext[r] = BLK_EMPTY;
        if (nch && (uint32_t)(r * N_NT + tid) < (L.desc[0].nrd_flags & 0xffffu)) dnext[r] = a.blk[L.desc[0].hdr_base + (uint32_t)(r * N_NT + tid)];
    }

    for (uint32_t c = 0; c < nch; ++c) {
        const ChunkDesc cd = L.desc[c % MAX_CHUNKS_PER_ITEM];
        const bool last_chunk = (cd.nrd_flags >> 16) != 0u;
        const uint32_t nblk = cd.nrd_flags & 0xffffu;
        uint32_t dcur[ROUNDS];
#pragma unroll
        for (int r = 0; r < ROUNDS; ++r) {
            dcur[r] = dnext[r];
            dnext[r] = BLK_EMPTY;
            if (c + 1 < nch && (uint32_t)(r * N_NT + tid) < (L.desc[(c + 1) % MAX_CHUNKS_PER_ITEM].nrd_flags & 0xffffu))
                dnext[r] = a.blk[L.desc[(c + 1) % MAX_CHUNKS_PER_ITEM].hdr_base + (uint32_t)(r * N_NT + tid)];
        }
        __syncthreads();
        desc_refill(L.desc, a.chunks + w.chunk_lo, c, nch, tid);
        if (L.evn >= (uint32_t)(N_EVCAP / 2)) flush_events<DenseLds, N_NT, N_EVCAP>(L, a, tid);

        const uint8_t *seq = a.seq + cd.seq_base;
        const uint64_t qbit0 = 2ull * cd.seq_base;
        uint4 sq[ROUNDS]; uint2 ql[ROUNDS];
#pragma unroll
        for (int r = 0; r < ROUNDS; ++r) {
            const uint32_t b = (uint32_t)(r * N_NT + tid);
            sq[r] = any_uint4(); ql[r] = make_uint2(0u, 0u);
            if (b < nblk) {
                ql[r] = lowq_fetch(a.qual, qbit0 + 32ull * b);
                sq[r] = *reinterpret_cast<const uint4 *>(seq + 16ull * b);
// ... 52 lines not shown
    if (tail0 + 2u * tid < n) *reinterpret_cast<uint16_t *>(p + tail0 + 2u * tid) = 0;
}

template <int NT>
__device__ __forceinline__ void zero_cells(uint16_t *ncol, uint16_t *cov_col, const unsigned long long cap_cells, const unsigned long long first, const unsigned long long n, const uint32_t tid) {
    if (n <= (unsigned long long)NT) {
        if (tid < (uint32_t)n) {
#pragma unroll
            for (int x = 0; x < 4; ++x) ncol[(uint64_t)x * cap_cells + first + tid] = 0;
            cov_col[first + tid] = 0;
        }
        return;
    }
#pragma unroll
    for (int x = 0; x < 4; ++x) zero_span<NT>(reinterpret_cast<uint8_t *>(ncol + (uint64_t)x * cap_cells + first), n * sizeof(uint16_t), tid);
    zero_span<NT>(reinterpret_cast<uint8_t *>(cov_col + first), n * sizeof(uint16_t), tid);
}

struct GateTile { uint32_t tile, slot_lo, slot_16, slot_w, slot_hi, vbeg, vend, n_slots; uint64_t row0; uint32_t tot_mode, staged, pair_lo, n_plane_pairs, pad0, pad1; };

struct GateArgs {
    uint32_t *tot; const uint8_t *part; const uint64_t *slot_off; const uint32_t *tile_slot_start, *tile_slot_u16, *tile_slot_wide; uint64_t npos;
    const uint32_t *tile_vbeg, *tile_vend; int min_cov, min_snvs; double min_frac;
    uint32_t *ind4, *unc_bits;
    const uint32_t *ref4, *ref_lc;
    unsigned long long *site_bits; uint32_t *site_rank; SiteRec *sites; uint32_t cap_sites; uint32_t *counters, *counters_next;
    uint32_t *tile_site_base, *tile_site_cnt; const uint32_t *active_tiles;
    uint16_t *ncol; uint16_t *cov_col; uint8_t *site_flags; uint32_t cap_out;
    const uint32_t *tile_nslots; unsigned long long *tile_cell_base; unsigned long long cap_cells;
    const GateTile *gate_tiles; uint32_t *tile_dirty; uint32_t *unc_sites; uint32_t use_dirty; unsigned long long *block_row;
    uint8_t *site_elig; uint32_t any_split;
    uint32_t n_active, tiles_per_wg;
    const TileStage *tile_stage;
    const uint8_t *aspill;
    uint32_t zero_next;
    const uint32_t *tile_list;
    uint32_t solo_cells;
};

constexpr uint32_t GATE_STAGE = 384;
constexpr uint32_t GATE_MAX_TILES = 8;
struct GateStageTile { uint32_t tile, site_rel, total, n_slots; unsigned long long cell_rel; };
struct GateLds {
    SiteRec  rec[GATE_STAGE];
    uint16_t fl[GATE_STAGE];
    uint8_t  unc[GATE_STAGE];
    uint32_t blk_rel[GATE_MAX_TILES][TILE / 64];
    GateStageTile tiles[GATE_MAX_TILES];
    uint32_t wave[GATE_NT / 64];
    uint32_t pop, ind, base;
    unsigned long long cell;
};

__device__ __forceinline__ void gate_flush(GateLds &L, const GateArgs &a, const uint32_t n_tiles, const uint32_t n_sites, const unsigned long long n_cells, const int tid) {
    if (n_tiles == 0u) return;
    if (tid == 0) {
        L.base = atomicAdd(&a.counters[2], n_sites);
        L.cell = atomicAdd(reinterpret_cast<unsigned long long *>(&a.counters[CNT_CELLS]), (n_cells + 7ull) & ~7ull);
    }
    __syncthreads();
    const uint32_t base = L.base; const unsigned long long cb = L.cell;
    if ((uint32_t)tid < n_tiles) {
        const GateStageTile t = L.tiles[tid];
        a.tile_site_base[t.tile] = base + t.site_rel; a.tile_site_cnt[t.tile] = t.total; a.tile_cell_base[t.tile] = cb + t.cell_rel;
    }
    if ((unsigned long long)base + n_sites <= a.cap_out && cb + n_cells <= a.cap_cells) {
        zero_cells<GATE_NT>(a.ncol, a.cov_col, a.cap_cells, cb, n_cells, (uint32_t)tid);
    }
    if ((uint32_t)tid < n_tiles * (TILE / 64)) {
        const uint32_t k = (uint32_t)tid / (TILE / 64), blk = (uint32_t)tid % (TILE / 64);
        const GateStageTile t = L.tiles[k];
        const uint32_t rel = L.blk_rel[k][blk];
        a.site_rank[(uint64_t)t.tile * (TILE / 64) + blk] = base + rel;
        a.block_row[(uint64_t)t.tile * (TILE / 64) + blk] = cb + t.cell_rel + (unsigned long long)(rel - t.site_rel) * t.n_slots;
    }
    for (uint32_t i = (uint32_t)tid; i < n_sites; i += GATE_NT) {
        const uint32_t idx = base + i;
        if (idx >= a.cap_sites) continue;
        a.sites[idx] = L.rec[i];
        if (idx < a.cap_out) { a.site_flags[idx] = (uint8_t)(L.fl[i] & 0xffu); a.site_elig[idx] = (uint8_t)(L.fl[i] >> 8); }
        if (L.unc[i]) {
            const uint32_t u = atomicAdd(&a.counters[CNT_UNC], 1u);
            if (u < a.cap_sites) a.unc_sites[u] = idx;
        }
    }
    __syncthreads();
}

template <bool MULTI, bool WIDE_TOT, bool PLANES = false>
__global__ __launch_bounds__(GATE_NT) void msnv_gate_sites(const GateArgs a) {
    constexpr int NN = WIDE_TOT ? 4 * GATE_PPT : 2 * GATE_PPT;
    constexpr int ROWS = MULTI ? 8 : 16;
    uint32_t *const tot = a.tot; const uint8_t *const part = a.part;
    const int min_cov = a.min_cov, min_snvs = a.min_snvs; const double min_frac = a.min_frac;
    unsigned long long *const site_bits = a.site_bits; SiteRec *const sites = a.sites;
    const uint32_t cap_sites = a.cap_sites; uint32_t *const counters = a.counters;
    uint16_t *const cov_col = a.cov_col;
    const uint32_t cap_out = a.cap_out;
    __shared__ GateLds L;
    const int tid = threadIdx.x, lane = tid & 63, wave = tid >> 6;
    const uint32_t p0 = (uint32_t)GATE_PPT * (uint32_t)tid;
    if (tid == 0) { L.pop = 0; L.ind = 0; }
    if (blockIdx.x == 0 && a.zero_next) for (uint32_t i = threadIdx.x; i < CNT_WORDS; i += GATE_NT) a.counters_next[i] = 0u;
    const bool listed = MULTI && a.tile_list != nullptr;
    const uint32_t ti_step = listed ? gridDim.x : 1u;
    const uint32_t ti_lo = listed ? blockIdx.x : MULTI ? blockIdx.x * a.tiles_per_wg : blockIdx.x;
    const uint32_t ti_hi = listed ? min(a.counters[CNT_STAGE], a.n_active) : MULTI ? min(a.n_active, ti_lo + a.tiles_per_wg) : ti_lo + 1u;
    if (MULTI && ti_lo >= ti_hi) return;
    auto tile_at = [&](const uint32_t ti) -> GateTile { return a.gate_tiles[listed ? a.tile_list[ti] : ti]; };
    uint32_t st_tiles = 0, st_sites = 0; unsigned long long st_cells = 0;
    GateTile gt_next = tile_at(ti_lo);
    for (uint32_t ti = ti_lo; ti < ti_hi; ti += ti_step) {
        const GateTile gt = gt_next;
        if (ti + ti_step < ti_hi) gt_next = tile_at(ti + ti_step);
        const uint32_t tile = gt.tile;
        const uint32_t t0 = tile * TILE;
        const uint32_t vb = gt.vbeg, ve = gt.vend;
        const uint64_t g0 = (uint64_t)t0 + p0;

        const uint32_t slot_lo = gt.slot_lo, slot_hi = gt.slot_hi;
        const uint32_t slot_16 = gt.slot_16, slot_w = gt.slot_w;
        const bool solo = MULTI && a.solo_cells && gt.staged == 2u;
        const bool consult = a.use_dirty && gt.tot_mode != 0u;
        uint32_t dirty = 0;
        if (consult) for (uint32_t sl = slot_lo; sl < slot_hi; ++sl) dirty |= a.tile_dirty[sl];
        const bool my_dirty = !consult || ((dirty >> (p0 >> 6)) & 1u);
        uint32_t *const tb = tot + 4ull * t0;
        const uint4 z4 = make_uint4(0u, 0u, 0u, 0u);
        uint4 e0 = z4, e1 = z4;
        if (gt.tot_mode == 0u) { e0 = reinterpret_cast<const uint4 *>(tb + p0)[0]; e1 = reinterpret_cast<const uint4 *>(tb + p0)[1]; }
        const uint32_t ind4w = my_dirty ? a.ind4[g0 >> 3] : 0u;
        const uint32_t uncb = my_dirty ? reinterpret_cast<const uint8_t *>(a.unc_bits)[g0 >> 3] : 0u;
        const uint32_t refw = a.ref4[g0 >> 3];
        const uint32_t lcb = reinterpret_cast<const uint8_t *>(a.ref_lc)[g0 >> 3];
        uint32_t covs[GATE_PPT];
    #pragma unroll
        for (int j = 0; j < GATE_PPT; ++j) covs[j] = 0;
        if (slot_16 > slot_lo) {
            const uint8_t *p8 = part + gt.row0 + p0;
            const uint32_t n8 = slot_16 - slot_lo;
            for (uint32_t r0 = 0; r0 < n8; r0 += 255u) {
                uint32_t h[4] = {0u, 0u, 0u, 0u};
                const uint32_t r1 = min(n8, r0 + 255u);
                uint32_t s = r0;
                for (; s + (uint32_t)ROWS <= r1; s += (uint32_t)ROWS) {
                    uint2 v[ROWS];
    #pragma unroll
                    for (int u = 0; u < ROWS; ++u) v[u] = *reinterpret_cast<const uint2 *>(p8 + (uint64_t)(s + (uint32_t)u) * TILE);
    #pragma unroll
                    for (int u = 0; u < ROWS; ++u) {
                        h[0] += v[u].x & 0x00ff00ffu; h[1] += (v[u].x >> 8) & 0x00ff00ffu;
                        h[2] += v[u].y & 0x00ff00ffu; h[3] += (v[u].y >> 8) & 0x00ff00ffu;
// ... 87 lines not shown
                        for (int u = 0; u < 4; ++u) {
                            const uint32_t w8[8] = {v[u][0].x, v[u][0].y, v[u][0].z, v[u][0].w, v[u][1].x, v[u][1].y, v[u][1].z, v[u][1].w};
#pragma unroll
                            for (int j = 0; j < GATE_PPT; ++j) { ae[j] += w8[j] & 0x00ff00ffu; ao[j] += (w8[j] >> 8) & 0x00ff00ffu; }
                        }
                    }
                    for (; sidx < r1; ++sidx) {
                        const uint4 *q = reinterpret_cast<const uint4 *>(p32 + (uint64_t)sidx * TILE);
                        const uint4 v0 = q[0], v1 = q[1];
                        const uint32_t w8[8] = {v0.x, v0.y, v0.z, v0.w, v1.x, v1.y, v1.z, v1.w};
#pragma unroll
                        for (int j = 0; j < GATE_PPT; ++j) { ae[j] += w8[j] & 0x00ff00ffu; ao[j] += (w8[j] >> 8) & 0x00ff00ffu; }
                    }
#pragma unroll
                    for (int j = 0; j < GATE_PPT; ++j) {
                        if (WIDE_TOT) { nn[4 * j] += ae[j] & 0xffffu; nn[4 * j + 1] += ao[j] & 0xffffu; nn[4 * j + 2] += ae[j] >> 16; nn[4 * j + 3] += ao[j] >> 16; }
                        else { nn[2 * j] += (ae[j] & 0xffffu) | ao[j] << 16; nn[2 * j + 1] += (ae[j] >> 16) | (ao[j] & 0xffff0000u); }
                    }
                }
            }
        }
        auto n_of = [&](const int j, const int x) -> uint32_t { return WIDE_TOT ? nn[4 * j + x] : (nn[2 * j + (x >> 1)] >> (16 * (x & 1))) & 0xffffu; };
        if (ind4w) a.ind4[g0 >> 3] = 0u;
        if (uncb) reinterpret_cast<uint8_t *>(a.unc_bits)[g0 >> 3] = 0;
        uint32_t okm = 0, uncm = 0, flw[2] = {0u, 0u}, elig[2] = {0u, 0u};
    #pragma unroll
        for (int j = 0; j < GATE_PPT; ++j) {
            const uint32_t p = p0 + (uint32_t)j, cov = covs[j];
            if (cov != 0u && p >= vb && p < ve && (int)cov >= min_cov &&
                (int)(n_of(j, 0) + n_of(j, 1) + n_of(j, 2) + n_of(j, 3)) >= min_snvs) {
                const uint32_t indx = (ind4w >> (4 * j)) & 15u;
                const bool unc = (uncb >> j) & 1u;
                const double lim = (double)(int)cov * min_frac;
                const uint32_t rc = (refw >> (4 * j)) & 15u;
                const bool lc = (lcb >> j) & 1u;
                bool ok = false;
                uint32_t pop = 0, ind = 0;
    #pragma unroll
                for (int x = 0; x < 4; ++x) {
                    if ((int)n_of(j, x) < min_snvs) continue;
                    const bool is_pop = (double)n_of(j, x) >= lim, is_ind = ((indx >> x) & 1u) || (solo && unc);
                    ok |= is_pop || is_ind || unc;
                    if (lc && rc == (1u << x)) continue;
                    if (is_pop) pop |= 1u << x; else if (is_ind) ind |= 1u << x;
                    else if (unc) { uncm |= 1u << j; elig[j >> 2] |= (1u << x) << (8 * (j & 3)); }
                }
                okm |= (ok ? 1u : 0u) << j;
                flw[j >> 2] |= (pop | ind << 4) << (8 * (j & 3));
            }
        }
        {
            unsigned long long w = (unsigned long long)okm << (8u * ((uint32_t)lane & 7u));
            w |= __shfl_xor(w, 1); w |= __shfl_xor(w, 2); w |= __shfl_xor(w, 4);
            if ((lane & 7) == 0) site_bits[g0 >> 6] = w;
        }
        const uint32_t mycnt = (uint32_t)__popc(okm);
        const uint32_t incl = (uint32_t)wave_inclusive_scan((int)mycnt);
        if (lane == 63) L.wave[wave] = incl;
        __syncthreads();
        uint32_t total = 0, mybase = incl - mycnt;
#pragma unroll
        for (int wv = 0; wv < GATE_NT / 64; ++wv) {
            if (wv < wave) mybase += L.wave[wv];
            total += L.wave[wv];
        }
        const uint32_t n_slots = gt.n_slots;
        if (tid == 0 && dirty) for (uint32_t sl = slot_lo; sl < slot_hi; ++sl) a.tile_dirty[sl] = 0u;
        const uint32_t okm_certain = a.any_split ? okm & ~uncm : okm;
        if (okm_certain) {
            uint32_t np = 0, ni = 0;
#pragma unroll
            for (int j = 0; j < GATE_PPT; ++j) { const uint32_t f = ((okm_certain >> j) & 1u) ? (flw[j >> 2] >> (8 * (j & 3))) & 0xffu : 0u; np += (f & 15u) ? 1u : 0u; ni += (f >> 4) ? 1u : 0u; }
            if (np) atomicAdd(&L.pop, np);
            if (ni) atomicAdd(&L.ind, ni);
        }
        if (total == 0u) {
            if (tid == 0) { a.tile_site_base[tile] = 0u; a.tile_site_cnt[tile] = 0u; a.tile_cell_base[tile] = 0ull; }
            __syncthreads();
            continue;
        }
        if (st_sites + total > GATE_STAGE || st_tiles == GATE_MAX_TILES) {
            gate_flush(L, a, st_tiles, st_sites, st_cells, tid);
            st_tiles = 0; st_sites = 0; st_cells = 0;
        }
        if (total <= GATE_STAGE && !solo) {
            if ((n_slots & 7u) == 0u) st_cells = (st_cells + 7ull) & ~7ull;
            if (tid == 0) L.tiles[st_tiles] = GateStageTile{tile, st_sites, total, n_slots, st_cells};
            if ((lane & 7) == 0) L.blk_rel[st_tiles][p0 >> 6] = st_sites + mybase;
            uint32_t i = st_sites + mybase;
#pragma unroll
            for (int j = 0; j < GATE_PPT; ++j) {
                if (okm & (1u << j)) {
                    SiteRec s;
                    s.gpos = (uint32_t)(g0 + (uint32_t)j); s.cov = covs[j];
                    s.n[0] = n_of(j, 0); s.n[1] = n_of(j, 1); s.n[2] = n_of(j, 2); s.n[3] = n_of(j, 3);
                    L.rec[i] = s;
                    L.fl[i] = (uint16_t)(((flw[j >> 2] >> (8 * (j & 3))) & 0xffu) | ((elig[j >> 2] >> (8 * (j & 3))) & 0xffu) << 8);
                    L.unc[i] = (uint8_t)((a.any_split && ((uncm >> j) & 1u)) ? 1u : 0u);
                    ++i;
                }
            }
            ++st_tiles; st_sites += total; st_cells += (unsigned long long)total * n_slots;
            __syncthreads();
            continue;
        }
        if (tid == 0) {
            const uint32_t base = atomicAdd(&counters[2], total);
            L.base = base;
            a.tile_site_base[tile] = base;
            a.tile_site_cnt[tile] = total;
            const unsigned long long cb = atomicAdd(reinterpret_cast<unsigned long long *>(&counters[CNT_CELLS]), ((unsigned long long)total * n_slots + 7ull) & ~7ull);
            L.cell = cb;
            a.tile_cell_base[tile] = cb;
        }
        __syncthreads();
        const uint32_t base = L.base; const unsigned long long s_cell = L.cell;
        const bool fits = (uint64_t)base + total <= cap_out && s_cell + (unsigned long long)total * n_slots <= a.cap_cells;
        if (fits && !solo) {
            const uint64_t n_cells = (uint64_t)total * n_slots;
            zero_cells<GATE_NT>(a.ncol, cov_col, a.cap_cells, s_cell, n_cells, (uint32_t)tid);
        }
        if ((lane & 7) == 0) {
            a.site_rank[g0 >> 6] = base + mybase;
            a.block_row[g0 >> 6] = s_cell + (unsigned long long)mybase * n_slots;
        }
        uint32_t idx = base + mybase;
#pragma unroll
        for (int j = 0; j < GATE_PPT; ++j) {
            if (okm & (1u << j)) {
                if (idx < cap_sites) {
                    SiteRec s;
                    s.gpos = (uint32_t)(g0 + (uint32_t)j); s.cov = covs[j];
                    s.n[0] = n_of(j, 0); s.n[1] = n_of(j, 1); s.n[2] = n_of(j, 2); s.n[3] = n_of(j, 3);
                    sites[idx] = s;
                    if (idx < cap_out) a.site_flags[idx] = (uint8_t)((flw[j >> 2] >> (8 * (j & 3))) & 0xffu);
                    if (idx < cap_out) a.site_elig[idx] = (uint8_t)((elig[j >> 2] >> (8 * (j & 3))) & 0xffu);
                    if (a.any_split && ((uncm >> j) & 1u)) {
                        const uint32_t u = atomicAdd(&counters[CNT_UNC], 1u);
                        if (u < cap_sites) a.unc_sites[u] = idx;
                    }
                    if (solo && fits) {
                        const unsigned long long cell = s_cell + (idx - base);
#pragma unroll
                        for (int x = 0; x < 4; ++x) a.ncol[(uint64_t)x * a.cap_cells + cell] = (uint16_t)s.n[x];
                        cov_col[cell] = (uint16_t)s.cov;
                    }
                }
                ++idx;
            }
        }
        __syncthreads();
    }
    gate_flush(L, a, st_tiles, st_sites, st_cells, tid);
    __syncthreads();
    if (tid == 0 && (L.pop | L.ind)) atomicAdd(reinterpret_cast<unsigned long long *>(&counters[CNT_TALLY]), (unsigned long long)L.pop | (unsigned long long)L.ind << 32);
}

constexpr int GS_WAVES = 4;
constexpr int GS_TILES = 16;
__global__ __launch_bounds__(64 * GS_WAVES) void msnv_gate_staged(const GateArgs a, const GateTile *__restrict__ tiles, const uint32_t n_tiles) {
    __shared__ uint32_t s_sites[GS_WAVES]; __shared__ unsigned long long s_cells[GS_WAVES];
    __shared__ uint32_t s_base, s_np, s_ni; __shared__ unsigned long long s_cb;
    const int lane = threadIdx.x & 63, wave = threadIdx.x >> 6;
    const uint32_t w0 = (blockIdx.x * (uint32_t)GS_WAVES + (uint32_t)wave) * (uint32_t)GS_TILES;
    if (blockIdx.x == 0 && a.zero_next) for (uint32_t i = threadIdx.x; i < CNT_WORDS; i += 64 * GS_WAVES) a.counters_next[i] = 0u;
    if (threadIdx.x == 0) { s_np = 0; s_ni = 0; }
    const uint32_t n_here = w0 < n_tiles ? min((uint32_t)GS_TILES, n_tiles - w0) : 0u;
    GateTile gt{};
    uint32_t cnt = 0;
    bool mine = (uint32_t)lane < n_here;
    if (mine) {
        gt = tiles[w0 + (uint32_t)lane]; cnt = a.tile_stage[gt.row0].count;
        if (cnt > STAGE_CAP) { mine = false; cnt = 0u; }
    }
    const unsigned long long cells = (unsigned long long)cnt * gt.n_slots;
    uint32_t site_rel = cnt; unsigned long long cell_rel = cells;
#pragma unroll
    for (int o = 1; o < GS_TILES; o <<= 1) {
        const uint32_t t = (uint32_t)__shfl_up((int)site_rel, o); const unsigned long long u = (unsigned long long)__shfl_up((long long)cell_rel, o);
        if (lane >= o) { site_rel += t; cell_rel += u; }
    }
    const uint32_t tot_sites = (uint32_t)__shfl((int)site_rel, GS_TILES - 1); const unsigned long long tot_cells = (unsigned long long)__shfl((long long)cell_rel, GS_TILES - 1);
    site_rel -= cnt; cell_rel -= cells;
    if (lane == 0) { s_sites[wave] = tot_sites; s_cells[wave] = tot_cells; }
    __syncthreads();
    if (threadIdx.x == 0) {
        uint32_t ts = 0; unsigned long long tc = 0;
        for (int k = 0; k < GS_WAVES; ++k) { ts += s_sites[k]; tc += s_cells[k]; }
        s_base = ts ? atomicAdd(&a.counters[2], ts) : 0u;
        s_cb = ts ? atomicAdd(reinterpret_cast<unsigned long long *>(&a.counters[CNT_CELLS]), (tc + 7ull) & ~7ull) : 0ull;
    }
    __syncthreads();
    uint32_t base = s_base; unsigned long long cb = s_cb;
    uint32_t wg_sites = 0; unsigned long long wg_cells = 0;
    for (int k = 0; k < GS_WAVES; ++k) { if (k < wave) { base += s_sites[k]; cb += s_cells[k]; } wg_sites += s_sites[k]; wg_cells += s_cells[k]; }
    if (mine) { a.tile_site_base[gt.tile] = cnt ? base + site_rel : 0u; a.tile_site_cnt[gt.tile] = cnt; a.tile_cell_base[gt.tile] = cnt ? cb + cell_rel : 0ull; }
    const bool fits = (unsigned long long)s_base + wg_sites <= a.cap_out && s_cb + wg_cells <= a.cap_cells;
    uint32_t np = 0, ni = 0;
    const unsigned long long mine_mask = __ballot(mine);
    for (uint32_t t = 0; t < n_here; ++t) {
        if (!((mine_mask >> t) & 1ull)) continue;
        const uint32_t tile = (uint32_t)__shfl((int)gt.tile, (int)t), n = (uint32_t)__shfl((int)cnt, (int)t), n_slots = (uint32_t)__shfl((int)gt.n_slots, (int)t);
        const uint32_t kind = (uint32_t)__shfl((int)gt.staged, (int)t), srel = (uint32_t)__shfl((int)site_rel, (int)t);
        const unsigned long long crel = (unsigned long long)__shfl((long long)cell_rel, (int)t), sidx = (unsigned long long)__shfl((long long)gt.row0, (int)t);
        StageRec r{0xffffffffu, 0u, 0u, 0u};
        if ((uint32_t)lane < n) r = a.tile_stage[sidx].rec[lane];
        const uint32_t pos = r.pos_flags & (TILE - 1u);
        uint32_t rank = 0, before = 0; unsigned long long word = 0;
// ... 412 lines not shown
#pragma unroll
                    for (uint32_t x = 0; x < 4; ++x) {
                        const uint32_t cnt = (al >> (8u * x)) & 0xffu;
                        if (cnt) a.ncol[(uint64_t)x * a.cells.cap_cells + cell] = (uint16_t)cnt;
                        if (cnt >= a.min_snvs) ind |= 1u << x;
                    }
                    if (ind && a.ind_in_gather) {
                        const uint32_t site = base + j0 + i / m;
                        ind &= a.site_elig[site];
                        if (ind) {
                            uint32_t *wordp = reinterpret_cast<uint32_t *>(a.site_flags + (site & ~3u));
                            const uint32_t sh = 8u * (site & 3u);
                            const uint32_t old = atomicOr(wordp, (ind << 4) << sh);
                            if ((((old >> sh) & 0xffu) >> 4) == 0u) ++my_tally;
                        }
                    }
                }
            }
            sync();
        }
    }
#pragma unroll
    for (int o = 32; o >= 1; o >>= 1) my_tally += (uint32_t)__shfl_xor((int)my_tally, o);
    if ((tid & 63u) == 0u && my_tally) atomicAdd(reinterpret_cast<unsigned long long *>(&a.counters[CNT_TALLY]), (unsigned long long)my_tally << 32);
}
__device__ __forceinline__ void gather_merged_block(const TailArgs &a, const uint32_t bid, uint32_t *s_pool) {
    if (a.merged_per_block == 1u) { gather_merged_group<256, GM_CELLS, MERGE_MAX_PAIRS, GM_HITS>(a, a.merged_groups[bid], s_pool, threadIdx.x); return; }
    const uint32_t gi = bid * GMW_GROUPS + (threadIdx.x >> 6);
    if (gi < a.n_merged_run) gather_merged_group<64, GMW_CELLS, GMW_PAIRS, GMW_HITS>(a, a.merged_groups[gi], s_pool + (threadIdx.x >> 6) * GMW_WORDS, threadIdx.x & 63u);
}
static bool merged_wave_form(const DeviceCols &d) {
    const int forced = knob::merged_gather();
    return d.max_group_pairs <= GMW_PAIRS && forced != 1;
}

template <bool HAS_MERGED>
__global__ __launch_bounds__(256) void msnv_gather_scatter(TailArgs a) {
    const uint32_t n_scatter = a.scatter_blocks * EV_LISTS;
    if (blockIdx.x == gridDim.x - 1u) {
        if (threadIdx.x < 64) {
            const uint32_t c = threadIdx.x < EV_LISTS ? a.counters[16u + threadIdx.x * EV_CNT_STRIDE] : 0u;
            unsigned long long total = c; uint32_t fullest = c;
#pragma unroll
            for (int o = 32; o >= 1; o >>= 1) { total += __shfl_xor(total, o); fullest = max(fullest, (uint32_t)__shfl_xor((int)fullest, o)); }
            if (fullest > a.cap_list) total = (unsigned long long)fullest * EV_LISTS;
            if (threadIdx.x == 0) a.counters[0] = (uint32_t)min(total, 0xffffffffull);
        }
        return;
    }
    __shared__ __attribute__((aligned(16))) uint32_t s_pool[TAIL_POOL_WORDS];
    if (blockIdx.x < n_scatter) { if (!(a.debug_skip & 1u)) scatter_events_block(a, blockIdx.x % a.scatter_blocks, blockIdx.x / a.scatter_blocks); }
    else if (HAS_MERGED && blockIdx.x < n_scatter + a.n_merged_blocks) { if (!(a.debug_skip & 4u)) gather_merged_block(a, blockIdx.x - n_scatter, s_pool); }
    else if (!(a.debug_skip & 2u)) gather_cov_block(a, blockIdx.x - n_scatter - a.n_merged_blocks, s_pool);
}

__global__ __launch_bounds__(256) void msnv_decide_sites(const SiteRec *sites, const uint32_t *unc_sites, uint32_t *counters, uint32_t cap_sites, uint32_t cap_out,
                                                         const uint32_t *ref4, const uint32_t *ref_lc, const uint16_t *ncol,
                                                         const CellMap cells, int min_snvs, double min_frac, uint8_t *site_flags) {
    __shared__ uint32_t s_pop, s_ind;
    if (threadIdx.x == 0) { s_pop = 0; s_ind = 0; }
    __syncthreads();
    const uint32_t n_unc = min(counters[CNT_UNC], cap_sites), n_sites = counters[2];
    const int lane = threadIdx.x & 63;
    if (n_sites <= cap_sites && n_sites <= cap_out && *reinterpret_cast<const unsigned long long *>(&counters[CNT_CELLS]) <= cells.cap_cells) {
        for (uint32_t u = blockIdx.x * (blockDim.x >> 6) + (threadIdx.x >> 6); u < n_unc; u += gridDim.x * (blockDim.x >> 6)) {
            const uint32_t site = unc_sites[u];
            const SiteRec s = sites[site];
            const uint32_t rc = (ref4[s.gpos >> 3] >> (4 * (s.gpos & 7))) & 0xfu;
            const bool lc = (ref_lc[s.gpos >> 5] >> (s.gpos & 31)) & 1u;
            uint32_t pop = 0, ind = 0;
            for (int x = 0; x < 4; ++x) {
                if (lc && rc == (1u << x)) continue;
                const uint32_t nx = s.n[x];
                if ((int)nx < min_snvs) continue;
                if ((double)nx >= (double)(int)s.cov * min_frac) { pop |= 1u << x; continue; }
                bool any = false;
                const uint32_t tile = s.gpos / TILE, n_slots = cells.tile_nslots[tile];
                const uint64_t row = cell_of(cells, tile, site, 0u);
                for (uint32_t i = lane; i < n_slots; i += 64)
                    any |= (int)ncol[(uint64_t)x * cells.cap_cells + row + i] >= min_snvs;
                if (__any(any)) ind |= 1u << x;
            }
            if (lane == 0) {
                site_flags[site] = (uint8_t)(pop | ind << 4);
                if (pop) atomicAdd(&s_pop, 1u);
                if (ind) atomicAdd(&s_ind, 1u);
            }
        }
    }
    __syncthreads();
    if (threadIdx.x == 0) {
        if (s_pop) atomicAdd(&counters[4], s_pop);
        if (s_ind) atomicAdd(&counters[5], s_ind);
    }
}

constexpr int C_NT = 64;
static_assert(C_NT / 64 * COV_PW == COV_ITEM_PAIRS, "coverage work items are sized for COV_PW pairs per wavefront");

__device__ __forceinline__ int wave_reduce_add(int x) {
    x = wave_inclusive_scan(x);
    return __builtin_amdgcn_readlane(x, 63);
}
__device__ __forceinline__ uint32_t row_sum16(uint32_t x) {
    x = (uint32_t)dpp_add<0xB1, 0xf>((int)x);
    x = (uint32_t)dpp_add<0x4E, 0xf>((int)x);
// ... 292 lines not shown
    {
        std::lock_guard<std::mutex> lk(g_cache_mu);
        for (void *p : ptrs) {
            if (!p) continue;
            auto it = g_cache_live.find(p);
            if (it == g_cache_live.end()) { foreign.push_back(p); continue; }
            g_cache_free.push_back(it->second); g_cache_free_bytes += it->second.bytes;
            g_cache_live.erase(it);
        }
    }
    int dev = 0;
    (void)hipGetDevice(&dev);
    const uint64_t cap = cache_cap_bytes(dev);
    {
        std::lock_guard<std::mutex> lk(g_cache_mu);
        while (g_cache_free_bytes > cap && !g_cache_free.empty()) {
            size_t big = 0;
            for (size_t i = 1; i < g_cache_free.size(); ++i) if (g_cache_free[i].bytes > g_cache_free[big].bytes) big = i;
            evict.push_back(g_cache_free[big]); g_cache_free_bytes -= g_cache_free[big].bytes;
            g_cache_free[big] = g_cache_free.back(); g_cache_free.pop_back();
        }
    }
    for (const CacheBlock &e : evict) (void)hipFree(e.p);
    for (void *p : foreign) (void)hipFree(p);
}
int dev_upload(void *dst, const void *src, uint64_t bytes) {
    if (!bytes) return MSNV_OK;
    HIP_TRY(hipMemcpy(dst, src, bytes, hipMemcpyHostToDevice));
    return MSNV_OK;
}
int dev_download(void *dst, const void *src, uint64_t bytes) { if (bytes) HIP_TRY(hipMemcpy(dst, src, bytes, hipMemcpyDeviceToHost)); return MSNV_OK; }
int dev_copy_bytes(void *dst_device, const void *src, uint64_t bytes, bool src_on_device, void *stream) {
    if (!bytes) return MSNV_OK;
    HIP_TRY(hipMemcpyAsync(dst_device, src, bytes, src_on_device ? hipMemcpyDeviceToDevice : hipMemcpyHostToDevice, (hipStream_t)stream));
    HIP_TRY(hipStreamSynchronize((hipStream_t)stream));
    return MSNV_OK;
}
int dev_memset(void *dst, int v, uint64_t bytes) {
    if (bytes) { HIP_TRY(hipMemset(dst, v, bytes)); HIP_TRY(hipStreamSynchronize(nullptr)); }
    return MSNV_OK;
}
int dev_memset_async(void *dst, int v, uint64_t bytes, void *stream) {
    if (bytes) HIP_TRY(hipMemsetAsync(dst, v, bytes, (hipStream_t)stream));
    return MSNV_OK;
}
int dev_stream_wait(void *stream) { HIP_TRY(hipStreamSynchronize((hipStream_t)stream)); return MSNV_OK; }
int dev_stream_create(void **stream) { hipStream_t s; HIP_TRY(hipStreamCreateWithFlags(&s, hipStreamNonBlocking)); *stream = s; return MSNV_OK; }
void dev_stream_destroy(void *stream) { if (stream) (void)hipStreamDestroy((hipStream_t)stream); }

void dev_free_all(DeviceCols &d) {
    void *ptrs[] = {d.hdr, d.hdr8, d.hdr4, d.hdr8m, d.merged_groups, d.tile_pair_merged, d.blk, d.seq, d.qual, d.s_read_base, d.s_seq_base, d.ref4, d.ref_lc, d.pairs,
                    d.tile_pair_start, d.work, d.chunks, d.tile_vbeg, d.tile_vend, d.tot, d.part, d.tile_slot_start, d.tile_slot_u16, d.tile_slot_wide, d.slot_off, d.spill, d.events, d.overflow, d.counters, d.ind4, d.tile_dirty, d.unc_sites, d.site_row, d.gate_tiles,
                    d.sites, d.tile_site_base, d.tile_site_cnt, d.tile_cell_base, d.tile_nslots, d.ncol, d.cov_col, d.site_flags, d.site_elig,
                    d.cov_iv, d.s_cov_base, d.cov_pairs, d.cov_work, d.tile_len, d.tile_contig_dev, d.cov_acc, d.tile_stage, d.tile_stage_idx, d.alt.tile_stage, d.gate_tiles_dense, d.gate_tiles_staged, d.gather_tiles};
    auto in_block = [&](void *p) { for (const auto &b : d.blocks) if ((char *)p >= (char *)b.first && (char *)p < (char *)b.first + b.second) return true; return false; };
    for (void *p : ptrs) if (p && !in_block(p)) dev_free(p);
    void *aptrs[] = {d.ann.seg_beg, d.ann.seg_end, d.ann.seg_gene, d.ann.genes, d.ann.contigs, d.ann.codons, d.ann.out, d.ann.err};
    for (void *p : aptrs) dev_free(p);
    for (void *e : d.timing_events) if (e) (void)hipEventDestroy((hipEvent_t)e);
    for (void *e : d.event_pool) (void)hipEventDestroy((hipEvent_t)e);
    if (d.pinned_cnt) (void)hipHostFree(d.pinned_cnt);
    void *alts[] = {d.aspill, d.alt.aspill, d.alt.tot, d.alt.part, d.alt.spill, d.alt.events, d.alt.overflow, d.alt.counters, d.alt.ind4, d.alt.tile_dirty, d.alt.unc_sites, d.alt.site_row, d.alt.sites, d.alt.tile_site_base,
                    d.alt.tile_site_cnt, d.alt.tile_cell_base, d.alt.ncol, d.alt.cov_col, d.alt.site_flags, d.alt.site_elig, d.alt.site_bits, d.site_bits, d.alt.site_rank, d.site_rank, d.active_tiles};
    for (void *p : alts) if (p && !in_block(p)) dev_free(p);
    for (const auto &b : d.blocks) dev_free(b.first);
    if (d.stream2) (void)hipStreamDestroy((hipStream_t)d.stream2);
    d = DeviceCols{};
}

static int ensure_out(DeviceCols &d, uint64_t n_sites, uint64_t n_cells) {
    if (n_sites > d.cap_out_sites) {
        dev_free(d.site_flags); d.site_flags = nullptr;
        dev_free(d.site_elig); d.site_elig = nullptr;
        const uint64_t cap = std::max<uint64_t>(n_sites + n_sites / 4, 1024);
        if (int rc = dev_alloc((void **)&d.site_flags, cap + 4, &d.device_bytes)) return rc;
        if (int rc = dev_alloc((void **)&d.site_elig, cap + 4, &d.device_bytes)) return rc;
        d.cap_out_sites = cap;
    }
    if (n_cells > d.cap_cells) {
        dev_free(d.ncol); dev_free(d.cov_col);
        d.ncol = nullptr; d.cov_col = nullptr;
        const uint64_t cap = (std::max<uint64_t>(n_cells + n_cells / 4, 1u << 16) + 7) & ~7ull;
        if (int rc = dev_alloc((void **)&d.ncol, 4 * cap * sizeof(uint16_t) + 16, &d.device_bytes)) return rc;
        if (int rc = dev_alloc((void **)&d.cov_col, cap * sizeof(uint16_t) + 16, &d.device_bytes)) return rc;
        d.cap_cells = cap;
    }
    return MSNV_OK;
}

static inline uint32_t *stage_ovf_list(const DeviceCols &d) { return d.tile_stage ? reinterpret_cast<uint32_t *>(d.tile_stage + d.n_active_tiles) : nullptr; }

static int enqueue_pass(DeviceCols &d, const msnv_params &p, hipStream_t st, hipEvent_t ev_begin, hipEvent_t ev_pile0, hipEvent_t ev_pile1,
                        hipEvent_t ev3, hipEvent_t ev4, uint32_t *host_cnt, hipEvent_t wait_before_pileup = nullptr) {
    const uint64_t npos = (uint64_t)d.n_tiles * TILE;
    if (p.min_baseq != d.qlow_cutoff) return fail(MSNV_EINVAL, "the dataset's quality column was packed for -Q %d, the pass asks for -Q %d", d.qlow_cutoff, p.min_baseq);
    if (ev_begin) HIP_TRY(hipEventRecord(ev_begin, st));
    uint32_t *const counters = d.counters + d.cnt_parity * CNT_WORDS, *const counters_next = d.counters + (d.cnt_parity ^ 1u) * CNT_WORDS;
    d.cnt_parity ^= 1u;
    if (wait_before_pileup) HIP_TRY(hipStreamWaitEvent(st, wait_before_pileup, 0));
    const uint32_t use_stage = (d.n_fused_tiles && !d.fuse_disabled && p.calling_threshold >= 1) ? 1u : 0u;
    HIP_TRY(hipEventRecord(ev_pile0, st));
    if (d.n_work) {
        PileupArgs a;
        a.hdr = d.hdr; a.hdr8 = d.hdr8; a.hdr4 = d.hdr4; a.blk = d.blk; a.seq = d.seq; a.qual = d.qual;
        a.s_read_base = d.s_read_base; a.s_seq_base = d.s_seq_base;
        a.ref4 = d.ref4; a.pairs = d.pairs; a.work = d.work; a.chunks = d.chunks; a.tot = d.tot; a.part = d.part; a.npos = npos; a.spill = d.spill; a.aspill = d.aspill;
        a.events = d.events; a.cap_events = d.cap_events / EV_LISTS; a.ev_count = nullptr; a.overflow = d.overflow; a.cap_overflow = d.cap_overflow;
        a.counters = counters; a.min_baseq = (uint32_t)std::max(0, p.min_baseq);
        a.ind4 = d.ind4; a.unc_bits = d.unc_bits; a.slot_dirty = d.tile_dirty; a.min_snvs = (uint32_t)std::max(0, p.calling_threshold);
        a.n_fused_lo = d.n_work_narrow + d.n_work_merged - (use_stage ? d.n_work_fused : 0u); a.min_cov = p.min_coverage; a.min_frac = p.min_fraction; a.ref_lc = d.ref_lc; a.tile_vbeg = d.tile_vbeg; a.tile_vend = d.tile_vend;
        a.tile_stage = d.tile_stage; a.tile_stage_idx = d.tile_stage_idx; a.stage_ovf = stage_ovf_list(d);
        const uint32_t n_narrow = d.n_work_narrow, n_merged = d.n_work_merged;
        a.hdr8m = d.hdr8m; a.n_narrow = n_narrow;
        if (n_narrow && d.dense) hipLaunchKernelGGL(msnv_pileup_tiles_dense, dim3(n_narrow), dim3(N_NT), 0, st, a);
        else {
            const bool lean_off = knob::lean_off();
            const uint32_t n_lean = (use_stage && !lean_off) ? d.n_work_fused : 0u, n_all = n_narrow + n_merged - n_lean;
            if (n_all && d.allele_planes) hipLaunchKernelGGL(msnv_pileup_tiles_narrow32_planes, dim3(n_all), dim3(N_NT), 0, st, a);
            else if (n_all) hipLaunchKernelGGL(msnv_pileup_tiles_narrow32, dim3(n_all), dim3(N_NT), 0, st, a);
            if (n_lean) hipLaunchKernelGGL(msnv_pileup_tiles_lean, dim3(n_lean), dim3(N_NT), 0, st, a);
        }
        if (d.n_work > n_narrow + n_merged) {
            PileupArgs b = a;
            b.work = d.work + n_narrow + n_merged;
            hipLaunchKernelGGL(msnv_pileup_tiles_wide, dim3(d.n_work - n_narrow - n_merged), dim3(W_NT), 0, st, b);
        }
        HIP_TRY(hipGetLastError());
    }
    HIP_TRY(hipEventRecord(ev_pile1, st));
    const uint32_t cap_out = (uint32_t)std::min<uint64_t>(d.cap_out_sites, 0xffffffffull);
    const bool need_decide = d.any_split;
    if (d.n_active_tiles) {
        GateArgs g;
        g.tot = d.tot; g.part = d.part; g.slot_off = d.slot_off; g.tile_slot_start = d.tile_slot_start; g.tile_slot_u16 = d.tile_slot_u16; g.tile_slot_wide = d.tile_slot_wide;
        g.npos = npos; g.tile_vbeg = d.tile_vbeg; g.tile_vend = d.tile_vend; g.min_cov = p.min_coverage; g.min_snvs = p.calling_threshold; g.min_frac = p.min_fraction;
        g.ind4 = d.ind4; g.unc_bits = d.unc_bits; g.ref4 = d.ref4; g.ref_lc = d.ref_lc;
        g.site_bits = d.site_bits; g.site_rank = d.site_rank; g.sites = d.sites; g.cap_sites = d.cap_sites; g.counters = counters; g.counters_next = counters_next;
        g.tile_site_base = d.tile_site_base; g.tile_site_cnt = d.tile_site_cnt; g.active_tiles = d.active_tiles;
        g.ncol = d.ncol; g.cov_col = d.cov_col; g.site_flags = d.site_flags; g.cap_out = cap_out;
        g.gate_tiles = reinterpret_cast<const GateTile *>(d.gate_tiles); g.tile_dirty = d.tile_dirty; g.unc_sites = d.unc_sites;
        g.use_dirty = d.use_dirty ? 1u : 0u; g.block_row = d.site_row; g.site_elig = d.site_elig; g.any_split = d.any_split ? 1u : 0u;
        static_assert(sizeof(GateTile) == sizeof(DeviceCols::GateTileH) && sizeof(GateTile) == 64, "gate tile descriptor");
        g.tile_nslots = d.tile_nslots; g.tile_cell_base = d.tile_cell_base; g.cap_cells = d.cap_cells;
        g.tile_stage = d.tile_stage; g.tiles_per_wg = 1u;
        const uint32_t n_staged = use_stage ? d.n_fused_tiles : 0u, n_dense = d.n_active_tiles - n_staged;
        if (use_stage) g.gate_tiles = reinterpret_cast<const GateTile *>(d.gate_tiles_dense);
        g.n_active = n_dense;
        g.zero_next = 1u; g.tile_list = nullptr; g.solo_cells = 0u;
        if (n_dense) {
            g.tiles_per_wg = knob::gate_tiles(n_dense >= 32768u ? 8u : n_dense >= 8192u ? 4u : 1u, (int)GATE_MAX_TILES);
            const dim3 grid((n_dense + g.tiles_per_wg - 1) / g.tiles_per_wg);
            g.aspill = d.aspill;
            if (d.allele_planes) {
                if (g.tiles_per_wg == 1u) {
                    if (d.wide_tot) hipLaunchKernelGGL((msnv_gate_sites<false, true, true>), grid, dim3(GATE_NT), 0, st, g);
                    else hipLaunchKernelGGL((msnv_gate_sites<false, false, true>), grid, dim3(GATE_NT), 0, st, g);
                } else {
                    if (d.wide_tot) hipLaunchKernelGGL((msnv_gate_sites<true, true, true>), grid, dim3(GATE_NT), 0, st, g);
                    else hipLaunchKernelGGL((msnv_gate_sites<true, false, true>), grid, dim3(GATE_NT), 0, st, g);
                }
            } else if (g.tiles_per_wg == 1u) {
                if (d.wide_tot) hipLaunchKernelGGL((msnv_gate_sites<false, true>), grid, dim3(GATE_NT), 0, st, g);
                else hipLaunchKernelGGL((msnv_gate_sites<false, false>), grid, dim3(GATE_NT), 0, st, g);
            } else {
                if (d.wide_tot) hipLaunchKernelGGL((msnv_gate_sites<true, true>), grid, dim3(GATE_NT), 0, st, g);
                else hipLaunchKernelGGL((msnv_gate_sites<true, false>), grid, dim3(GATE_NT), 0, st, g);
            }
            g.zero_next = 0u;
        }
        if (n_staged) {
            hipLaunchKernelGGL(msnv_gate_staged, dim3((n_staged + GS_WAVES * GS_TILES - 1) / (GS_WAVES * GS_TILES)), dim3(64 * GS_WAVES), 0, st, g, reinterpret_cast<const GateTile *>(d.gate_tiles_staged), n_staged);
            g.gate_tiles = reinterpret_cast<const GateTile *>(d.gate_tiles); g.tile_list = stage_ovf_list(d); g.n_active = n_staged; g.solo_cells = 1u;
            g.tiles_per_wg = 1u; g.zero_next = 0u; g.aspill = d.aspill;
            const dim3 grid(std::min<uint32_t>(n_staged, std::max<uint32_t>(64u, std::min<uint32_t>(4096u, d.last_ovf_tiles))));
            if (d.allele_planes) {
                if (d.wide_tot) hipLaunchKernelGGL((msnv_gate_sites<true, true, true>), grid, dim3(GATE_NT), 0, st, g);
                else hipLaunchKernelGGL((msnv_gate_sites<true, false, true>), grid, dim3(GATE_NT), 0, st, g);
            } else {
                if (d.wide_tot) hipLaunchKernelGGL((msnv_gate_sites<true, true>), grid, dim3(GATE_NT), 0, st, g);
                else hipLaunchKernelGGL((msnv_gate_sites<true, false>), grid, dim3(GATE_NT), 0, st, g);
            }
        }
        HIP_TRY(hipGetLastError());
    } else HIP_TRY(hipMemsetAsync(counters_next, 0, CNT_WORDS * sizeof(uint32_t), st));
    if (ev3) HIP_TRY(hipEventRecord(ev3, st));
    if (d.n_active_tiles) {
        TailArgs ta;
        ta.sites = d.sites; ta.tile_site_base = d.tile_site_base; ta.tile_site_cnt = d.tile_site_cnt; ta.tile_pair_start = d.tile_pair_start;
        ta.pairs = d.pairs; ta.spill = d.spill; ta.ncol = d.ncol; ta.cov_col = d.cov_col; ta.cap_out = cap_out; ta.active_tiles = d.gather_tiles;
        ta.cells = CellMap{d.tile_site_base, d.tile_cell_base, d.tile_nslots, d.cap_cells, d.site_row};
        ta.gather_split = d.gather_split;
        ta.has_wide = d.n_work > d.n_work_narrow + d.n_work_merged ? 1u : 0u;
        ta.aspill = d.allele_planes ? d.aspill : nullptr;
        const uint32_t tail_skip = knob::tail_skip();
        ta.debug_skip = tail_skip;
        ta.n_gather_blocks = d.n_gather_tiles * d.gather_split;
        ta.tile_pair_merged = d.tile_pair_merged; ta.merged_groups = d.merged_groups; ta.chunks = d.chunks; ta.hdr8m = d.hdr8m;
        ta.seq = d.seq; ta.qual = d.qual; ta.ref4 = d.ref4; ta.n_merged_run = d.n_merged_groups - (use_stage ? d.n_groups_solo : 0u);
        ta.merged_per_block = merged_wave_form(d) ? GMW_GROUPS : 1u; ta.n_merged_blocks = (ta.n_merged_run + ta.merged_per_block - 1u) / ta.merged_per_block; ta.min_baseq = (uint32_t)std::max(0, p.min_baseq);
        ta.site_flags = d.site_flags; ta.site_elig = d.site_elig; ta.ind_in_gather = d.any_split ? 0u : 1u; ta.min_snvs = (uint32_t)std::max(1, p.calling_threshold);
        ta.events = d.events; ta.overflow = d.overflow; ta.counters = counters; ta.cap_list = d.cap_events / EV_LISTS; ta.cap_overflow = d.cap_overflow;
        ta.site_bits = d.site_bits; ta.site_rank = d.site_rank;
        const uint32_t scatter_blocks = knob::scatter_blocks(SCATTER_BLOCKS_PER_LIST);
        ta.scatter_blocks = scatter_blocks;
        const dim3 grid(ta.n_gather_blocks + ta.n_merged_blocks + ta.scatter_blocks * EV_LISTS + 1u);
        if (ta.n_merged_blocks) hipLaunchKernelGGL(msnv_gather_scatter<true>, grid, dim3(256), 0, st, ta);
        else hipLaunchKernelGGL(msnv_gather_scatter<false>, grid, dim3(256), 0, st, ta);
        HIP_TRY(hipGetLastError());
    }
    if (ev4) HIP_TRY(hipEventRecord(ev4, st));
    if (need_decide && d.n_active_tiles) {
        static const uint32_t decide_grid = dev_resident_workgroups(8);
        hipLaunchKernelGGL(msnv_decide_sites, dim3(decide_grid), dim3(256), 0, st, d.sites, d.unc_sites, counters, d.cap_sites, cap_out, d.ref4, d.ref_lc,
                           d.ncol, CellMap{d.tile_site_base, d.tile_cell_base, d.tile_nslots, d.cap_cells, d.site_row}, p.calling_threshold, p.min_fraction, d.site_flags);
        HIP_TRY(hipGetLastError());
    }
    HIP_TRY(hipMemcpyAsync(host_cnt, counters, CNT_WORDS * sizeof(uint32_t), hipMemcpyDeviceToHost, st));
    return MSNV_OK;
}

static int check_counts(DeviceCols &d, const uint32_t *cnt, RunCounts *counts) {
    RunCounts c{cnt[0], cnt[1], cnt[2], cnt[3], (uint64_t)cnt[CNT_CELLS] | (uint64_t)cnt[CNT_CELLS + 1] << 32};
    d.last_sites = c.n_sites; d.last_cells = c.n_cells;
    if (counts) *counts = c;
    d.last_ovf_tiles = cnt[CNT_STAGE];
    if (c.n_events > d.cap_events / EV_LISTS * EV_LISTS || c.n_overflow > d.cap_overflow || c.n_sites > d.cap_sites || c.n_sites > d.cap_out_sites || c.n_cells > d.cap_cells)
        return fail_quiet(MSNV_ECAPACITY, "device buffer too small: events %u/%u overflow %u/%u sites %u/%u out %u/%llu cells %llu/%llu",
                          c.n_events, d.cap_events, c.n_overflow, d.cap_overflow, c.n_sites, d.cap_sites, c.n_sites,
                          (unsigned long long)d.cap_out_sites, (unsigned long long)c.n_cells, (unsigned long long)d.cap_cells);
    return MSNV_OK;
}

int dev_run_pipeline(DeviceCols &d, const msnv_params &p, void *stream_, msnv_run_stats *stats, RunCounts *counts) {
    hipStream_t st = (hipStream_t)stream_;
    hipEvent_t ev[6];
    for (int i = 0; i < 6; ++i) {
        if (!d.timing_events[i]) { hipEvent_t e; HIP_TRY(hipEventCreate(&e)); d.timing_events[i] = e; }
        ev[i] = (hipEvent_t)d.timing_events[i];
    }
    const bool phase_times = knob::phase_times();
    if (int rc = ensure_out(d, std::max<uint64_t>(d.last_sites + d.last_sites / 2, 4096), std::max<uint64_t>(d.last_cells + d.last_cells / 2, 1u << 18))) return rc;
    uint32_t cnt[CNT_WORDS] = {0};
    if (int rc = enqueue_pass(d, p, st, ev[0], ev[1], ev[2], phase_times ? ev[3] : nullptr, phase_times ? ev[4] : nullptr, cnt)) return rc;
    HIP_TRY(hipEventRecord(ev[5], st));
    HIP_TRY(hipStreamSynchronize(st));
    if (int rc = check_counts(d, cnt, counts)) return rc;
    if (stats) {
        float ms = 0;
        HIP_TRY(hipEventElapsedTime(&ms, ev[0], ev[5])); stats->ms_total = ms;
        HIP_TRY(hipEventElapsedTime(&ms, ev[1], ev[2])); stats->ms_pileup = ms;
        if (phase_times) {
            HIP_TRY(hipEventElapsedTime(&ms, ev[2], ev[3])); stats->ms_gate = ms;
            HIP_TRY(hipEventElapsedTime(&ms, ev[3], ev[4])); stats->ms_gather = ms;
            HIP_TRY(hipEventElapsedTime(&ms, ev[4], ev[5])); stats->ms_decide = ms;
        }
        stats->n_sites = cnt[2]; stats->n_events = cnt[0]; stats->n_overflow = cnt[1];
        stats->n_called_pop = cnt[4] + cnt[CNT_TALLY]; stats->n_called_indiv = cnt[5] + cnt[CNT_TALLY + 1];
        stats->algorithmic_bytes = d.algorithmic_bytes;
    }
    return MSNV_OK;
}

static int ensure_alt(DeviceCols &d) {
    DeviceCols::AltBufs &a = d.alt;
    const uint64_t npos = (uint64_t)d.n_tiles * TILE;
    if (a.tot && a.cap_events == d.cap_events && a.cap_overflow == d.cap_overflow && a.cap_sites == d.cap_sites && a.cap_out_sites == d.cap_out_sites && a.cap_cells == d.cap_cells) return MSNV_OK;
    void *old[] = {a.aspill, a.tot, a.part, a.spill, a.events, a.overflow, a.counters, a.ind4, a.tile_dirty, a.unc_sites, a.site_row, a.sites, a.tile_site_base, a.tile_site_cnt, a.tile_cell_base, a.ncol, a.cov_col, a.site_flags, a.site_elig, a.site_bits, a.site_rank, a.tile_stage};
    for (void *p : old) dev_free(p);
    a = DeviceCols::AltBufs{};
    if (int rc = dev_alloc((void **)&a.tot, std::max<uint64_t>(1, 4 * npos) * sizeof(uint32_t), &d.device_bytes)) return rc;
    if (int rc = dev_memset(a.tot, 0, std::max<uint64_t>(1, 4 * npos) * sizeof(uint32_t))) return rc;
    if (int rc = dev_alloc((void **)&a.part, d.part_bytes, &d.device_bytes)) return rc;
    if (int rc = dev_alloc((void **)&a.spill, std::max<uint64_t>(1, d.n_pairs) * TILE, &d.device_bytes)) return rc;
    if (d.allele_planes) {
        if (int rc = dev_alloc((void **)&a.aspill, (uint64_t)d.n_pairs * 4 * TILE, &d.device_bytes)) return rc;
        if (int rc = dev_memset(a.aspill, 0, (uint64_t)d.n_pairs * 4 * TILE)) return rc;
    }
    if (int rc = dev_alloc((void **)&a.events, (uint64_t)d.cap_events * sizeof(Pair32), &d.device_bytes)) return rc;
    if (int rc = dev_alloc((void **)&a.overflow, (uint64_t)d.cap_overflow * sizeof(Pair32), &d.device_bytes)) return rc;
    if (int rc = dev_alloc((void **)&a.sites, (uint64_t)d.cap_sites * sizeof(SiteRec), &d.device_bytes)) return rc;
    if (int rc = dev_alloc((void **)&a.unc_sites, (uint64_t)d.cap_sites * sizeof(uint32_t), &d.device_bytes)) return rc;
    if (int rc = dev_alloc((void **)&a.site_row, (npos / 64 + 1) * sizeof(unsigned long long), &d.device_bytes)) return rc;
    if (int rc = dev_alloc((void **)&a.tile_dirty, ((uint64_t)d.n_work + 1) * sizeof(uint32_t), &d.device_bytes)) return rc;
    if (int rc = dev_memset(a.tile_dirty, 0, ((uint64_t)d.n_work + 1) * sizeof(uint32_t))) return rc;
    if (int rc = dev_alloc((void **)&a.counters, 2 * CNT_WORDS * sizeof(uint32_t), &d.device_bytes)) return rc;
    if (int rc = dev_memset(a.counters, 0, 2 * CNT_WORDS * sizeof(uint32_t))) return rc;
    if (int rc = dev_alloc((void **)&a.ind4, (npos / 8 + npos / 32 + 2) * sizeof(uint32_t), &d.device_bytes)) return rc;
    if (int rc = dev_memset(a.ind4, 0, (npos / 8 + npos / 32 + 2) * sizeof(uint32_t))) return rc;
    a.unc_bits = a.ind4 + npos / 8 + 1; a.cnt_parity = 0;
    if (int rc = dev_alloc((void **)&a.site_bits, (npos / 64 + 1) * sizeof(unsigned long long), &d.device_bytes)) return rc;
    if (int rc = dev_alloc((void **)&a.site_rank, (npos / 64 + 1) * sizeof(uint32_t), &d.device_bytes)) return rc;
    if (int rc = dev_alloc((void **)&a.tile_site_base, ((uint64_t)d.n_tiles + 1) * sizeof(uint32_t), &d.device_bytes)) return rc;
    if (int rc = dev_alloc((void **)&a.tile_site_cnt, ((uint64_t)d.n_tiles + 1) * sizeof(uint32_t), &d.device_bytes)) return rc;
    if (int rc = dev_memset(a.tile_site_cnt, 0, ((uint64_t)d.n_tiles + 1) * sizeof(uint32_t))) return rc;
    if (int rc = dev_memset(a.tile_site_base, 0, ((uint64_t)d.n_tiles + 1) * sizeof(uint32_t))) return rc;
    if (int rc = dev_alloc((void **)&a.tile_cell_base, ((uint64_t)d.n_tiles + 1) * sizeof(unsigned long long), &d.device_bytes)) return rc;
    if (int rc = dev_alloc((void **)&a.ncol, 4 * d.cap_cells * sizeof(uint16_t) + 16, &d.device_bytes)) return rc;
    if (int rc = dev_alloc((void **)&a.cov_col, d.cap_cells * sizeof(uint16_t) + 16, &d.device_bytes)) return rc;
    if (int rc = dev_alloc((void **)&a.site_flags, d.cap_out_sites + 4, &d.device_bytes)) return rc;
    if (int rc = dev_alloc((void **)&a.site_elig, d.cap_out_sites + 4, &d.device_bytes)) return rc;
    if (d.n_fused_tiles && !a.tile_stage) {
        if (int rc = dev_alloc((void **)&a.tile_stage, (uint64_t)d.n_active_tiles * sizeof(TileStage) + (uint64_t)d.n_fused_tiles * sizeof(uint32_t), &d.device_bytes)) return rc;
        if (int rc = dev_memset(a.tile_stage, 0, (uint64_t)d.n_active_tiles * sizeof(TileStage))) return rc;
    }
    a.cap_events = d.cap_events; a.cap_overflow = d.cap_overflow; a.cap_sites = d.cap_sites; a.cap_out_sites = d.cap_out_sites; a.cap_cells = d.cap_cells;
    return MSNV_OK;
}
static void swap_sets(DeviceCols &d) {
    DeviceCols::AltBufs &a = d.alt;
    std::swap(d.tot, a.tot); std::swap(d.part, a.part); std::swap(d.spill, a.spill); std::swap(d.events, a.events);
    if (a.aspill) std::swap(d.aspill, a.aspill);
    std::swap(d.overflow, a.overflow); std::swap(d.counters, a.counters); std::swap(d.sites, a.sites);
    std::swap(d.tile_site_base, a.tile_site_base); std::swap(d.tile_site_cnt, a.tile_site_cnt); std::swap(d.tile_cell_base, a.tile_cell_base); std::swap(d.ncol, a.ncol); std::swap(d.cov_col, a.cov_col);
    std::swap(d.site_flags, a.site_flags); std::swap(d.site_elig, a.site_elig); std::swap(d.ind4, a.ind4); std::swap(d.unc_bits, a.unc_bits); std::swap(d.cnt_parity, a.cnt_parity);
    if (a.tile_stage) std::swap(d.tile_stage, a.tile_stage);
    std::swap(d.tile_dirty, a.tile_dirty); std::swap(d.unc_sites, a.unc_sites); std::swap(d.site_row, a.site_row); std::swap(d.site_bits, a.site_bits); std::swap(d.site_rank, a.site_rank);
}

int dev_reserve_passes(DeviceCols &d, int n) {
    while (d.event_pool.size() < (size_t)4 * n + 2) { hipEvent_t e; HIP_TRY(hipEventCreate(&e)); d.event_pool.push_back(e); }
    if (d.pinned_cnt_cap < (size_t)n) {
        if (d.pinned_cnt) (void)hipHostFree(d.pinned_cnt);
        d.pinned_cnt = nullptr; d.pinned_cnt_cap = 0;
        if (hipHostMalloc((void **)&d.pinned_cnt, (size_t)n * CNT_WORDS * sizeof(uint32_t), hipHostMallocDefault) != hipSuccess) return fail(MSNV_ENOMEM, "pinned host memory for %d counter blocks", n);
        d.pinned_cnt_cap = (size_t)n;
    }
    return MSNV_OK;
}

int dev_run_pipeline_many(DeviceCols &d, const msnv_params &p, void *stream_, int n, bool overlap, msnv_run_stats *stats, RunCounts *counts) {
    if (n <= 0) return MSNV_OK;
    hipStream_t s0 = (hipStream_t)stream_, s1 = s0;
    if (int rc = ensure_out(d, std::max<uint64_t>(d.last_sites + d.last_sites / 2, 4096), std::max<uint64_t>(d.last_cells + d.last_cells / 2, 1u << 18))) return rc;
    if (overlap && n > 1) {
        if (!d.stream2) { hipStream_t s; HIP_TRY(hipStreamCreateWithFlags(&s, hipStreamNonBlocking)); d.stream2 = s; }
        s1 = (hipStream_t)d.stream2;
        if (int rc = ensure_alt(d)) return rc;
    }
    const bool two = s1 != s0;
    if (int rc = dev_reserve_passes(d, n)) return rc;
    hipEvent_t *ev = reinterpret_cast<hipEvent_t *>(d.event_pool.data());
    auto cleanup = [] {};
    uint32_t *cnt = d.pinned_cnt;
    int rc = MSNV_OK;
    hipError_t he = hipSuccess;
    bool swapped = false;
    for (int i = 0; i < n && !rc && he == hipSuccess; ++i) {
        hipStream_t st = (i & 1) ? s1 : s0;
        if (two && (i & 1) != (swapped ? 1 : 0)) { swap_sets(d); swapped = !swapped; }
        rc = enqueue_pass(d, p, st, i == 0 ? ev[0] : nullptr, ev[4 * i + 1], ev[4 * i + 2], nullptr, nullptr, cnt + (size_t)CNT_WORDS * i, (two && i > 0) ? ev[4 * (i - 1) + 2] : nullptr);
    }
    if (!rc && he == hipSuccess) he = hipEventRecord(ev[4 * n], s0);
    if (!rc && he == hipSuccess) he = hipEventRecord(ev[4 * n + 1], s1);
    if (he == hipSuccess) he = hipStreamSynchronize(s0);
    if (he == hipSuccess && two) he = hipStreamSynchronize(s1);
    if (two && swapped != (((n - 1) & 1) != 0)) { swap_sets(d); swapped = !swapped; }
    if (!rc && he != hipSuccess) rc = fail(MSNV_EHIP, "batched passes: %s", hipGetErrorString(he));
    float total = 0, t1 = 0;
    if (!rc) {
        (void)hipEventElapsedTime(&total, ev[0], ev[4 * n]);
        if (two && hipEventElapsedTime(&t1, ev[0], ev[4 * n + 1]) == hipSuccess) total = std::max(total, t1);
    }
    for (int i = 0; i < n && !rc; ++i) {
        rc = check_counts(d, cnt + (size_t)CNT_WORDS * i, counts);
        if (rc || !stats) continue;
        float ms = 0;
        msnv_run_stats &s = stats[i];
        s = msnv_run_stats{};
        s.ms_total = total / (float)n;
        if (hipEventElapsedTime(&ms, ev[4 * i + 1], ev[4 * i + 2]) == hipSuccess) s.ms_pileup = ms;
        const uint32_t *c = cnt + (size_t)CNT_WORDS * i;
        s.n_sites = c[2]; s.n_events = c[0]; s.n_overflow = c[1]; s.n_called_pop = c[4] + c[CNT_TALLY]; s.n_called_indiv = c[5] + c[CNT_TALLY + 1];
        s.algorithmic_bytes = d.algorithmic_bytes;
    }
    cleanup();
    return rc;
}

int dev_run_coverage(DeviceCols &d, int max_cov, void *stream_, msnv_run_stats *stats) {
    hipStream_t st = (hipStream_t)stream_;
    if (max_cov < 1 || max_cov >= COV_BINS) return fail(MSNV_EINVAL, "coverage histogram cutoff must be in [1, %d]", COV_BINS - 1);
    hipEvent_t e0, e1;
    HIP_TRY(hipEventCreate(&e0)); HIP_TRY(hipEventCreate(&e1));
    HIP_TRY(hipEventRecord(e0, st));
    HIP_TRY(hipMemsetAsync(d.cov_acc, 0, (uint64_t)d.cov_copies * std::max<uint64_t>(1, d.n_cov_rows) * (1 + COV_BINS) * sizeof(unsigned long long), st));
    if (d.n_cov_work) {
        const uint32_t n_narrow = d.n_cov_work - d.n_cov_work_wide;
        if (n_narrow) hipLaunchKernelGGL(msnv_coverage_tiles<false>, dim3(n_narrow), dim3(C_NT), 0, st, d.cov_iv, d.cov_pairs, d.cov_work,
                                         d.tile_len, d.cov_acc, (uint32_t)d.n_cov_rows, max_cov, d.cov_copies, d.n_cov_iv);
        if (d.n_cov_work_wide) hipLaunchKernelGGL(msnv_coverage_tiles<true>, dim3(d.n_cov_work_wide), dim3(C_NT), 0, st, d.cov_iv, d.cov_pairs, d.cov_work + n_narrow,
                                                  d.tile_len, d.cov_acc, (uint32_t)d.n_cov_rows, max_cov, d.cov_copies, d.n_cov_iv);
        HIP_TRY(hipGetLastError());
    }
    HIP_TRY(hipEventRecord(e1, st));
    HIP_TRY(hipStreamSynchronize(st));
    float ms = 0;
    HIP_TRY(hipEventElapsedTime(&ms, e0, e1));
    if (stats) stats->ms_coverage = ms;
    (void)hipEventDestroy(e0); (void)hipEventDestroy(e1);
    return MSNV_OK;
}

__global__ void msnv_coverage_scanned(const TilePair *pairs, const WorkItem *work, const uint32_t *tile_len, const uint32_t n_work, const uint32_t n_pairs,
// ... 39 lines not shown
```

metasnv_amd/csrc/knobs.h:

```cpp
#pragma once

#include <algorithm>
#include <cstdint>
#include <cstdio>
#include <cstdlib>

namespace msnv {
namespace knob {

inline char first(const char *name) { const char *e = getenv(name); return e ? e[0] : '\0'; }
inline bool present(const char *name) { return getenv(name) != nullptr; }
inline bool int_of(const char *name, int *v) { const char *e = getenv(name); if (e) *v = atoi(e); return e != nullptr; }
inline bool i64_of(const char *name, long long *v) { const char *e = getenv(name); if (e) *v = atoll(e); return e != nullptr; }
inline int       int_or(const char *name, int dflt) { int_of(name, &dflt); return dflt; }
inline long long i64_or(const char *name, long long dflt) { i64_of(name, &dflt); return dflt; }

inline uint32_t inflate_check_every() { const int v = int_or("MSNV_INFLATE_CHECK", 1); return (uint32_t)(v < 0 ? 0 : v); }
constexpr const char *INFLATE = "MSNV_INFLATE";
inline char inflate_where() { const char *e = getenv(INFLATE); return !e ? '\0' : e[0] == 'd' ? 'd' : 'h'; }
inline bool inflate_zlib() { static const bool on = first(INFLATE) == 'z'; return on; }
inline uint64_t inflate_batch_bytes(bool resident = false) { return (uint64_t)std::max<long long>(1, i64_or("MSNV_INFLATE_BATCH_MB", resident ? 2048 : 1024)) << 20; }
inline bool test_no_staging() { return first("MSNV_TEST_NO_STAGING") == '1'; }
inline bool test_resident_fail() { return present("MSNV_TEST_RESIDENT_FAIL"); }
inline bool crc_table() { static const bool on = first("MSNV_CRC") == 't'; return on; }
// ... 1 lines not shown
inline bool finalize_trace() { static const bool on = first("MSNV_FINALIZE_TRACE") == '1'; return on; }
inline bool feed_trace() { static const bool on = first("MSNV_FEED_TRACE") == '1'; return on; }
inline char stage_free() { const char c = first("MSNV_STAGE_FREE"); return c == 's' || c == 'n' ? c : '\0'; }

inline bool pack_on_host() { return first("MSNV_PACK") == 'h'; }
inline uint64_t pack_round_bytes() { return (uint64_t)std::max<long long>(1, i64_or("MSNV_PACK_ROUND_MB", 6144)) << 20; }
inline bool pack_copy() { return present("MSNV_PACK_COPY"); }
inline bool scan_segments() { return first("MSNV_SCAN") == 's'; }
inline bool front_careful() { return first("MSNV_FRONT") == 'c'; }
constexpr long long SCAN_SUB_STREAMS = 4096, SCAN_SUB_ROUND = 6144;
inline uint32_t scan_sub_bytes(long long route_default) { return (uint32_t)std::min<long long>(32768, std::max<long long>(64, i64_or("MSNV_SCAN_SUB", route_default))); }
inline uint64_t scan_seg_bytes() { return (uint64_t)std::max<long long>(1, i64_or("MSNV_SCAN_SEG_KB", 256)) << 10; }
inline bool tile_order_sort() { return first("MSNV_TILE_ORDER") == 's'; }
inline bool depth_on_main() { static const bool on = first("MSNV_DEPTH_STREAM") == 'm'; return on; }
inline bool overlap_on_host() { return first("MSNV_OVERLAP") == 'h'; }
inline bool prepass_on_host() { return first("MSNV_PREPASS") == 'h'; }
inline bool emit_slow() { return first("MSNV_EMIT") == 's'; }
inline bool debug_sync() { static const bool on = present("MSNV_DEBUG_SYNC"); return on; }
inline bool no_adopt() { return present("MSNV_NO_ADOPT"); }

inline char layout() { const char c = first("MSNV_LAYOUT"); return c == 'p' || c == 'd' ? c : '\0'; }
inline bool deep_wide() { return first("MSNV_DEEP") == 'w'; }
inline uint32_t split_at(int max_depth) { return (uint32_t)std::min(max_depth, std::max(32, int_or("MSNV_SPLIT_AT", 192))); }
inline uint32_t group_depth() { return (uint32_t)std::min(250, std::max(16, int_or("MSNV_GROUP_DEPTH", 128))); }
inline bool deep_relocate_off() { return first("MSNV_DEEP_RELOCATE") == '0'; }
inline bool finalize_on_host() { return first("MSNV_FINALIZE") == 'h'; }
inline bool dense_relayout_on_host() { return first("MSNV_DENSE_RELAYOUT") == 'h'; }
inline bool fill_padding() { return present("MSNV_FILL_PADDING"); }

inline uint32_t shallow_pieces() { return (uint32_t)std::max(0, int_or("MSNV_SHALLOW_PIECES", 48)); }
inline bool merge_always() { return first("MSNV_MERGE_ALWAYS") == '1'; }
inline char fuse() { const char c = first("MSNV_FUSE"); return c == '0' || c == '1' ? c : '\0'; }
inline uint32_t fuse_pieces() { return (uint32_t)std::max(1, int_or("MSNV_FUSE_PIECES", 256)); }
inline uint64_t item_pieces() { return std::max<uint64_t>(64, (uint64_t)i64_or("MSNV_ITEM_PIECES", 2000)); }
inline bool item_taper() { return first("MSNV_ITEM_TAPER") != '0'; }
struct TaperAt { double u1 = 1.8, u2 = 0.73, u3 = 0.27; };
inline TaperAt taper_at() { TaperAt t; if (const char *e = getenv("MSNV_TAPER_AT")) sscanf(e, "%lf,%lf,%lf", &t.u1, &t.u2, &t.u3); return t; }
inline uint32_t tot_mode_min() { return (uint32_t)std::min(2, std::max(0, int_or("MSNV_TOT_MODE", 0))); }
inline uint32_t gather_split(uint32_t by_dataset) { int v = 0; return int_of("MSNV_GATHER_SPLIT", &v) ? (uint32_t)std::max(1, v) : by_dataset; }
inline uint64_t chunk_cap(uint64_t bound) { long long v = 0; return i64_of("MSNV_CHUNK_CAP", &v) ? (uint64_t)std::max<long long>(0, v) : bound; }
inline char alleles() { const char *e = getenv("MSNV_ALLELES"); return !e ? '\0' : e[0] == 'p' ? 'p' : 'e'; }
inline uint32_t cap_events(uint32_t by_dataset, long long min_events) { long long v = 0; return i64_of("MSNV_CAP_EVENTS", &v) ? (uint32_t)std::max(min_events, v) : by_dataset; }

inline char cov_index() { const char c = first("MSNV_COV_INDEX"); return c == 'd' || c == 's' ? c : '\0'; }
inline bool cov_late() { return present("MSNV_COV_LATE"); }
inline bool cov_tables_on_host() { return first("MSNV_COV_TABLES") == 'h'; }
inline bool cov_thread() { return present("MSNV_COV_THREAD"); }
inline uint32_t cov_item_intervals() { const long long v = i64_or("MSNV_COV_ITEM", 16384); return (uint32_t)std::min<long long>(v > 0 ? v : 16384, 0x7fffffffll); }
inline uint32_t cov_narrow_max() { return (uint32_t)std::min<long long>(32767, std::max<long long>(1, i64_or("MSNV_COV_NARROW_MAX", 32767))); }

inline int merged_gather() { const char c = first("MSNV_MERGED_GATHER"); return c == 'b' ? 1 : c == 'w' ? 2 : 0; }
inline bool lean_off() { return first("MSNV_LEAN") == '0'; }
inline uint32_t gate_tiles(uint32_t by_tiles, int max_tiles) { int v = 0; return int_of("MSNV_GATE_TILES", &v) ? (uint32_t)std::min(max_tiles, std::max(1, v)) : by_tiles; }
inline uint32_t tail_skip() { static const uint32_t v = (uint32_t)int_or("MSNV_TAIL_SKIP", 0); return v; }
inline uint32_t scatter_blocks(uint32_t default_blocks) { static const uint32_t v = [&] { int x = 0; return int_of("MSNV_SCATTER_BLOCKS", &x) ? (uint32_t)std::max(1, x) : default_blocks; }(); return v; }
inline bool phase_times() { static const bool on = first("MSNV_PHASE_TIMES") == '1'; return on; }
inline bool guard_alloc() { static const bool on = first("MSNV_GUARD_ALLOC") == '1'; return on; }
inline bool guard_fill(int *byte) { return int_of("MSNV_GUARD_FILL", byte); }
inline bool guard_log() { return present("MSNV_GUARD_LOG"); }
inline long long dev_cache_mb() { static const long long mb = [] { long long v = 0; return i64_of("MSNV_DEV_CACHE_MB", &v) ? std::max<long long>(0, v) : -1ll; }(); return mb; }

inline uint64_t text_chunk_bytes(uint64_t default_bytes) { long long v = 0; return i64_of("MSNV_TEXT_CHUNK", &v) ? std::max<uint64_t>(1, (uint64_t)v) : default_bytes; }
inline int text_repeat() { return std::max(1, int_or("MSNV_TEXT_REPEAT", 1)); }

}
}
```

Baseline: 3555.

## Route pileup events into per-tile lists and fuse tile tail into gate kernel

Pileup kernels can now write events into per-tile slices, using a prefix offset table and per-tile counters, instead of 32 shared round-robin lists. When the tile lists fit, a fused gate kernel runs a per-tile tail phase that consumes those lists directly, skipping separate cell zeroing and scatter/gather launches. Counters are also read back through mapped pinned memory to cut copy overhead. This adds device buffers, capacity fallbacks, and an env knob to disable the path, and it risks cases where the lists overflow or are refused.

Result: slower. 3491 (-1.8%).

```diff
diff --git a/include/msnv.h b/include/msnv.h
--- a/include/msnv.h
+++ b/include/msnv.h
@@ -180,6 +180,7 @@
 
 int  msnv_pileup_run_many(msnv_dataset *ds, int32_t n, int32_t overlap, msnv_run_stats *stats);
 int  msnv_pileup_reserve(msnv_dataset *ds, int32_t n);
+int  msnv_pileup_tail_route(const msnv_dataset *ds);
 int  msnv_coverage_run(msnv_dataset *ds, msnv_run_stats *stats);
 int  msnv_fused_run(msnv_dataset *ds, msnv_run_stats *pileup_stats, msnv_run_stats *coverage_stats);
 int  msnv_write_coverage(msnv_dataset *ds, int32_t sample_idx, const char *cov_path, const char *detail_path);
diff --git a/metasnv_amd/_lib.py b/metasnv_amd/_lib.py
--- a/metasnv_amd/_lib.py
+++ b/metasnv_amd/_lib.py
@@ -151,6 +151,7 @@
     ("msnv_pileup_run", C.c_int, [_vp, P(RunStats)]),
     ("msnv_pileup_run_many", C.c_int, [_vp, C.c_int32, C.c_int32, P(RunStats)]),
     ("msnv_pileup_reserve", C.c_int, [_vp, C.c_int32]),
+    ("msnv_pileup_tail_route", C.c_int, [_vp]),
     ("msnv_host_cores", C.c_int32, []),
     ("msnv_dataset_deal_bams_device", C.c_int, [_vp, P(C.c_char_p), C.c_int32, C.c_int32, P(C.c_int32), C.c_int32, C.c_int32, C.c_void_p, C.c_uint64, C.c_uint64,
                                                 P(C.c_uint64), P(SampleStats), P(C.c_uint64)]),
diff --git a/metasnv_amd/core.py b/metasnv_amd/core.py
--- a/metasnv_amd/core.py
+++ b/metasnv_amd/core.py
@@ -234,6 +234,12 @@
 
     def reserve_passes(self, n):
         check(lib.msnv_pileup_reserve(self._h, int(n)))
+
+    def tail_route(self):
+        rc = lib.msnv_pileup_tail_route(self._h)
+        if rc < 0:
+            check(-rc)
+        return rc == 1
 
     def run_many(self, n, overlap=False):
         arr = (RunStats * n)()
diff --git a/metasnv_amd/csrc/api.cpp b/metasnv_amd/csrc/api.cpp
--- a/metasnv_amd/csrc/api.cpp
+++ b/metasnv_amd/csrc/api.cpp
@@ -539,6 +539,7 @@
     clear_error();
     if (!ds || !out) return fail(MSNV_EINVAL, "msnv_dataset_info_get: NULL argument");
     *out = ds->info;
+    if (ds->dev && ds->finalized) out->device_bytes = ds->dev->device_bytes;
     if (ds->dev) { out->n_whole_tile_items = ds->dev->n_fused_tiles; out->n_listed_tiles = ds->dev->last_ovf_tiles; }
     return MSNV_OK;
 }
@@ -565,6 +566,12 @@
     ds->last_stats = tmp.back();
     if (stats) memcpy(stats, tmp.data(), tmp.size() * sizeof(msnv_run_stats));
     return MSNV_OK;
+}
+
+extern "C" int msnv_pileup_tail_route(const msnv_dataset *ds) {
+    clear_error();
+    if (!ds || !ds->finalized || !ds->have_results) return -fail(MSNV_EINVAL, "msnv_pileup_tail_route: no pass has run");
+    return ds->dev->pass_tile_route ? 1 : 0;
 }
 
 static void gpos_to_contig(const msnv_dataset &ds, uint32_t gpos, int32_t &tid, int32_t &pos) {
@@ -588,6 +595,7 @@
             cap = (uint32_t)std::min<uint64_t>(0x7fffffffull, (uint64_t)need + need / 4 + 1024);
             return dev_alloc(p, (uint64_t)cap * elem, &d.device_bytes);
         };
+        if (int r2 = dev_resize_tile_lists(d)) return r2;
         if (int r2 = grow((void **)&d.events, d.cap_events, c.n_events, sizeof(Pair32))) return r2;
         if (int r2 = grow((void **)&d.overflow, d.cap_overflow, c.n_overflow, sizeof(Pair32))) return r2;
         const uint32_t old_cap_sites = d.cap_sites;
diff --git a/metasnv_amd/csrc/device.h b/metasnv_amd/csrc/device.h
--- a/metasnv_amd/csrc/device.h
+++ b/metasnv_amd/csrc/device.h
@@ -75,6 +75,13 @@
     Pair32   *overflow = nullptr;
     uint32_t *counters = nullptr;
     uint32_t  cnt_parity = 0;
+    uint32_t *ev_tile_cnt = nullptr;
+    uint32_t *ev_tile_off = nullptr;
+    uint32_t *ev_tile_last = nullptr;
+    bool      tile_lists_short = false;
+    bool      tile_lists_refused = false;
+    bool      tile_tail_ok = false;
+    bool      pass_tile_route = false;
     uint32_t *ind4 = nullptr;
     uint32_t *unc_bits = nullptr;
     uint32_t *tile_dirty = nullptr;
@@ -127,17 +134,18 @@
     struct AltBufs {
         uint32_t *tot = nullptr; uint8_t *part = nullptr; uint8_t *spill = nullptr, *aspill = nullptr; Pair32 *events = nullptr, *overflow = nullptr;
         TileStage *tile_stage = nullptr;
-        uint32_t *counters = nullptr; SiteRec *sites = nullptr; uint32_t *tile_site_base = nullptr, *tile_site_cnt = nullptr; unsigned long long *tile_cell_base = nullptr;
+        uint32_t *counters = nullptr, *ev_tile_cnt = nullptr; SiteRec *sites = nullptr; uint32_t *tile_site_base = nullptr, *tile_site_cnt = nullptr; unsigned long long *tile_cell_base = nullptr;
         uint16_t *ncol = nullptr; uint16_t *cov_col = nullptr; uint8_t *site_flags = nullptr, *site_elig = nullptr; uint32_t *ind4 = nullptr, *unc_bits = nullptr, *tile_dirty = nullptr, *unc_sites = nullptr; unsigned long long *site_row = nullptr; unsigned long long *site_bits = nullptr; uint32_t *site_rank = nullptr;
         uint32_t cap_events = 0, cap_overflow = 0, cap_sites = 0, cnt_parity = 0; uint64_t cap_out_sites = 0, cap_cells = 0;
     } alt;
     void     *stream2 = nullptr;
     std::vector<void *> event_pool;
-    uint32_t *pinned_cnt = nullptr; size_t pinned_cnt_cap = 0;
+    uint32_t *pinned_cnt = nullptr, *pinned_cnt_dev = nullptr; size_t pinned_cnt_cap = 0;
     void     *timing_events[6] = {nullptr, nullptr, nullptr, nullptr, nullptr, nullptr};
 };
 
 constexpr uint32_t EV_LISTS = 32, EV_CNT_STRIDE = 16;
+constexpr uint32_t CNT_EV_OVER = 8;
 constexpr uint32_t CNT_CELLS = 16 + EV_LISTS * EV_CNT_STRIDE;
 constexpr uint32_t CNT_TALLY = CNT_CELLS + 16;
 constexpr uint32_t CNT_UNC = CNT_TALLY + 16;
@@ -180,6 +188,7 @@
 int  dev_run_pipeline_many(DeviceCols &d, const msnv_params &p, void *stream, int n, bool overlap, msnv_run_stats *stats, RunCounts *counts);
 void dev_free_all(DeviceCols &d);
 int  dev_reserve_passes(DeviceCols &d, int n);
+int  dev_resize_tile_lists(DeviceCols &d);
 void warm_devpack(void *stream), warm_kernels(void *stream), warm_textcall(void *stream), warm_annotate(void *stream);
 
 struct InfBlock { unsigned long long in_off, out_off; uint32_t in_size, out_size; };
diff --git a/metasnv_amd/csrc/kernels.hip b/metasnv_amd/csrc/kernels.hip
--- a/metasnv_amd/csrc/kernels.hip
+++ b/metasnv_amd/csrc/kernels.hip
@@ -44,6 +44,8 @@
     Pair32         *overflow; uint32_t cap_overflow;
     uint32_t       *counters;
     uint32_t       *ev_count;
+    uint32_t       *ev_tile_cnt;
+    const uint32_t *ev_tile_off;
     uint32_t        min_baseq;
     uint32_t       *ind4;
     uint32_t       *unc_bits;
@@ -137,22 +139,34 @@
     Pair32   ev[W_EVCAP];
     int32_t  wsum[W_NT / 64];
     uint32_t evn, ev_base;
+    uint32_t ev_lim;
 };
 
-__device__ __forceinline__ void ev_list(PileupArgs &a) {
+__device__ __forceinline__ void ev_list(PileupArgs &a, const uint32_t tile) {
+    const bool by_tile = a.ev_tile_cnt != nullptr;
     const uint32_t k = blockIdx.x % EV_LISTS;
-    a.events += (uint64_t)k * a.cap_events;
-    a.ev_count = a.counters + 16u + k * EV_CNT_STRIDE;
+    if (!by_tile) a.events += (uint64_t)k * a.cap_events;
+    a.ev_count = by_tile ? a.ev_tile_cnt + (uint64_t)tile * EV_CNT_STRIDE : a.counters + 16u + k * EV_CNT_STRIDE;
+}
+__device__ __forceinline__ uint2 ev_range(const PileupArgs &a) {
+    if (a.ev_tile_cnt == nullptr) return make_uint2(0u, a.cap_events);
+    const uint32_t tile = (uint32_t)(a.ev_count - a.ev_tile_cnt) / EV_CNT_STRIDE, lo = a.ev_tile_off[tile];
+    return make_uint2(lo, a.ev_tile_off[tile + 1u] - lo);
 }
 
 template <typename LDS, int NT, int CAP>
 __device__ __forceinline__ void flush_events(LDS &L, const PileupArgs &a, int tid) {
     const uint32_t n = min(L.evn, (uint32_t)CAP);
-    if (tid == 0) L.ev_base = n ? atomicAdd(a.ev_count, n) : 0u;
+    if (tid == 0 && n) {
+        const uint2 r = ev_range(a);
+        L.ev_base = r.x + min(atomicAdd(a.ev_count, n), r.y); L.ev_lim = r.x + r.y;
+    }
     __syncthreads();
-    const uint32_t base = L.ev_base;
-    for (uint32_t i = tid; i < n; i += NT)
-        if (base + i < a.cap_events) a.events[base + i] = L.ev[i];
+    if (n) {
+        const uint32_t base = (uint32_t)__builtin_amdgcn_readfirstlane((int)L.ev_base), lim = (uint32_t)__builtin_amdgcn_readfirstlane((int)L.ev_lim);
+        for (uint32_t i = tid; i < n; i += NT)
+            if (base + i < lim) a.events[base + i] = L.ev[i];
+    }
     __syncthreads();
     if (tid == 0) L.evn = 0;
 }
@@ -162,7 +176,8 @@
     const uint32_t i = atomicAdd(&L.evn, 1u);
     if (i < (uint32_t)CAP) { L.ev[i] = e; return; }
     const uint32_t g = atomicAdd(a.ev_count, 1u);
-    if (g < a.cap_events) a.events[g] = e;
+    const uint2 r = ev_range(a);
+    if (g < r.y) a.events[r.x + g] = e;
 }
 
 __device__ __forceinline__ void wide_classify(WideLds &L, const uint32_t lq, const uint32_t s0, const uint32_t s1,
@@ -185,9 +200,9 @@
 }
 
 __global__ __launch_bounds__(W_NT) void msnv_pileup_tiles_wide(PileupArgs a) {
-    ev_list(a);
     __shared__ WideLds L;
     const WorkItem w = a.work[blockIdx.x];
+    ev_list(a, w.tile);
     const uint32_t t0 = w.tile * TILE;
     const int tid = threadIdx.x, lane = tid & 63, wave = tid >> 6;
     const int lane8 = tid & (LANES_PER_READ - 1), grp = tid / LANES_PER_READ;
@@ -335,6 +350,7 @@
     ChunkDesc desc[MAX_CHUNKS_PER_ITEM];
     uint32_t carry[N_NT / 64 + 1];
     uint32_t evn, ev_base;
+    uint32_t ev_lim;
     uint32_t emask[SEQ_ALIGN_LOG2 < 3 ? 33 : 1];
 };
 
@@ -421,17 +437,21 @@
         return;
     }
     const uint32_t ei = (uint32_t)wave_inclusive_scan((int)myev);
-    uint32_t res = 0;
+    uint32_t res = 0, lim = 0;
     if (lane == 63 && ei) {
         uint32_t cur = atomicAdd(&L.evn, 0u);
         for (;;) {
-            if (cur + ei > (uint32_t)N_EVCAP) { res = 0x80000000u | atomicAdd(a.ev_count, ei); break; }
+            if (cur + ei > (uint32_t)N_EVCAP) {
+                const uint2 r = ev_range(a);
+                res = 0x80000000u | (r.x + min(atomicAdd(a.ev_count, ei), r.y)); lim = r.x + r.y; break;
+            }
             const uint32_t seen = atomicCAS(&L.evn, cur, cur + ei);
             if (seen == cur) { res = cur; break; }
             cur = seen;
         }
     }
     res = (uint32_t)__builtin_amdgcn_readlane((int)res, 63);
+    lim = (uint32_t)__builtin_amdgcn_readlane((int)lim, 63);
     const bool direct = (res & 0x80000000u) != 0u;
     uint32_t slot = (res & 0x7fffffffu) + ei - myev;
     while (pm) {
@@ -447,7 +467,7 @@
             if (n >= a.min_snvs) atomicOr(&a.ind4[gpos >> 3], 1u << (4u * (gpos & 7u) + x));
             else if (split) atomicOr(&a.unc_bits[gpos >> 5], 1u << (gpos & 31u));
             const Pair32 e{gpos, sample << 18 | x << 16 | n};
-            if (direct) { if (slot < a.cap_events) a.events[slot] = e; }
+            if (direct) { if (slot < lim) a.events[slot] = e; }
             else L.ev[slot] = e;
             ++slot;
         }
@@ -606,8 +626,8 @@
 
 template <bool MERGED, bool FUSED = false, bool DA = false>
 __device__ __forceinline__ void pileup_tiles_narrow32_body(PileupArgs a, NarrowLds &L) {
-    ev_list(a);
     const WorkItem w = a.work[blockIdx.x];
+    ev_list(a, w.tile);
     const uint32_t t0 = w.tile * TILE;
     const int tid = threadIdx.x, lane = tid & 63, wave = tid >> 6;
     const int lane4 = tid & (N32_LANES - 1), grp = tid / N32_LANES;
@@ -930,6 +950,7 @@
     ChunkDesc desc[MAX_CHUNKS_PER_ITEM];
     uint32_t carry[N_NT / 64 + 1];
     uint32_t evn, ev_base;
+    uint32_t ev_lim;
 };
 
 __device__ __forceinline__ uint32_t range_nibbles(const int lo, const int hi, const int k) {
@@ -972,9 +993,9 @@
 }
 
 __global__ __launch_bounds__(N_NT) void msnv_pileup_tiles_dense(PileupArgs a) {
-    ev_list(a);
     __shared__ DenseLds L;
     const WorkItem w = a.work[blockIdx.x];
+    ev_list(a, w.tile);
     const uint32_t t0 = w.tile * TILE;
     const int tid = threadIdx.x, lane = tid & 63, wave = tid >> 6;
 
@@ -1133,6 +1154,7 @@
     unsigned long long cell;
 };
 
+template <bool ZERO = true>
 __device__ __forceinline__ void gate_flush(GateLds &L, const GateArgs &a, const uint32_t n_tiles, const uint32_t n_sites, const unsigned long long n_cells, const int tid) {
     if (n_tiles == 0u) return;
     if (tid == 0) {
@@ -1145,7 +1167,7 @@
         const GateStageTile t = L.tiles[tid];
         a.tile_site_base[t.tile] = base + t.site_rel; a.tile_site_cnt[t.tile] = t.total; a.tile_cell_base[t.tile] = cb + t.cell_rel;
     }
-    if ((unsigned long long)base + n_sites <= a.cap_out && cb + n_cells <= a.cap_cells) {
+    if (ZERO && (unsigned long long)base + n_sites <= a.cap_out && cb + n_cells <= a.cap_cells) {
         zero_cells<GATE_NT>(a.ncol, a.cov_col, a.cap_cells, cb, n_cells, (uint32_t)tid);
     }
     if ((uint32_t)tid < n_tiles * (TILE / 64)) {
@@ -1168,8 +1190,13 @@
     __syncthreads();
 }
 
-template <bool MULTI, bool WIDE_TOT, bool PLANES = false>
-__global__ __launch_bounds__(GATE_NT) void msnv_gate_sites(const GateArgs a) {
+struct TileTailArgs; struct TileTailLds;
+__device__ __forceinline__ void tile_tail_phase(const GateArgs &a, const TileTailArgs &t, const GateLds &L, TileTailLds &T);
+__device__ __forceinline__ void tile_tail_note(TileTailLds &T, uint32_t blk, unsigned long long mask);
+__device__ __forceinline__ void tile_tail_note(TileTailLds &T, uint32_t blk, uint32_t rank, bool first, uint32_t tile, uint32_t total, uint32_t n_slots);
+template <bool MULTI, bool WIDE_TOT, bool PLANES, bool TAIL>
+__device__ __forceinline__ void gate_sites_body(const GateArgs &a, GateLds &L, const TileTailArgs *tt, TileTailLds *T) {
+    static_assert(!TAIL || !MULTI, "the tail phase follows the gate of ONE tile");
     constexpr int NN = WIDE_TOT ? 4 * GATE_PPT : 2 * GATE_PPT;
     constexpr int ROWS = MULTI ? 8 : 16;
     uint32_t *const tot = a.tot; const uint8_t *const part = a.part;
@@ -1178,7 +1205,6 @@
     const uint32_t cap_sites = a.cap_sites; uint32_t *const counters = a.counters;
     uint16_t *const cov_col = a.cov_col;
     const uint32_t cap_out = a.cap_out;
-    __shared__ GateLds L;
     const int tid = threadIdx.x, lane = tid & 63, wave = tid >> 6;
     const uint32_t p0 = (uint32_t)GATE_PPT * (uint32_t)tid;
     if (tid == 0) { L.pop = 0; L.ind = 0; }
@@ -1372,7 +1398,7 @@
         {
             unsigned long long w = (unsigned long long)okm << (8u * ((uint32_t)lane & 7u));
             w |= __shfl_xor(w, 1); w |= __shfl_xor(w, 2); w |= __shfl_xor(w, 4);
-            if ((lane & 7) == 0) site_bits[g0 >> 6] = w;
+            if ((lane & 7) == 0) { site_bits[g0 >> 6] = w; if constexpr (TAIL) tile_tail_note(*T, p0 >> 6, w); }
         }
         const uint32_t mycnt = (uint32_t)__popc(okm);
         const uint32_t incl = (uint32_t)wave_inclusive_scan((int)mycnt);
@@ -1385,6 +1411,7 @@
             total += L.wave[wv];
         }
         const uint32_t n_slots = gt.n_slots;
+        if constexpr (TAIL) { if ((lane & 7) == 0) tile_tail_note(*T, p0 >> 6, mybase, tid == 0, tile, total, n_slots); }
         if (tid == 0 && dirty) for (uint32_t sl = slot_lo; sl < slot_hi; ++sl) a.tile_dirty[sl] = 0u;
         const uint32_t okm_certain = a.any_split ? okm & ~uncm : okm;
         if (okm_certain) {
@@ -1400,7 +1427,7 @@
             continue;
         }
         if (st_sites + total > GATE_STAGE || st_tiles == GATE_MAX_TILES) {
-            gate_flush(L, a, st_tiles, st_sites, st_cells, tid);
+            gate_flush<!TAIL>(L, a, st_tiles, st_sites, st_cells, tid);
             st_tiles = 0; st_sites = 0; st_cells = 0;
         }
         if (total <= GATE_STAGE && !solo) {
@@ -1436,7 +1463,7 @@
         __syncthreads();
         const uint32_t base = L.base; const unsigned long long s_cell = L.cell;
         const bool fits = (uint64_t)base + total <= cap_out && s_cell + (unsigned long long)total * n_slots <= a.cap_cells;
-        if (fits && !solo) {
+        if (!TAIL && fits && !solo) {
             const uint64_t n_cells = (uint64_t)total * n_slots;
             zero_cells<GATE_NT>(a.ncol, cov_col, a.cap_cells, s_cell, n_cells, (uint32_t)tid);
         }
@@ -1471,9 +1498,15 @@
         }
         __syncthreads();
     }
-    gate_flush(L, a, st_tiles, st_sites, st_cells, tid);
+    gate_flush<!TAIL>(L, a, st_tiles, st_sites, st_cells, tid);
     __syncthreads();
     if (tid == 0 && (L.pop | L.ind)) atomicAdd(reinterpret_cast<unsigned long long *>(&counters[CNT_TALLY]), (unsigned long long)L.pop | (unsigned long long)L.ind << 32);
+    if constexpr (TAIL) tile_tail_phase(a, *tt, L, *T);
+}
+template <bool MULTI, bool WIDE_TOT, bool PLANES = false>
+__global__ __launch_bounds__(GATE_NT) void msnv_gate_sites(const GateArgs a) {
+    __shared__ GateLds L;
+    gate_sites_body<MULTI, WIDE_TOT, PLANES, false>(a, L, nullptr, nullptr);
 }
 
 constexpr int GS_WAVES = 4;
@@ -1992,6 +2025,114 @@
     if (blockIdx.x < n_scatter) { if (!(a.debug_skip & 1u)) scatter_events_block(a, blockIdx.x % a.scatter_blocks, blockIdx.x / a.scatter_blocks); }
     else if (HAS_MERGED && blockIdx.x < n_scatter + a.n_merged_blocks) { if (!(a.debug_skip & 4u)) gather_merged_block(a, blockIdx.x - n_scatter, s_pool); }
     else if (!(a.debug_skip & 2u)) gather_cov_block(a, blockIdx.x - n_scatter - a.n_merged_blocks, s_pool);
+}
+
+constexpr uint32_t TT_CELLS = 4096;
+struct TileTailArgs { const Pair32 *events; uint32_t *ev_tile_cnt; const uint32_t *ev_tile_off; uint32_t *ev_tile_last; const TilePair *pairs; const uint32_t *tile_pair_start; const uint8_t *spill;
+                      uint32_t *done;
+                      uint32_t *host_cnt; };
+struct alignas(16) TileTailLds {
+    uint32_t cells[5][TT_CELLS / 2];
+    unsigned long long mask[TILE / 64];
+    uint32_t rank[TILE / 64];
+    uint16_t pos[TILE];
+    uint32_t tile, total, n_slots, pad;
+};
+__device__ __forceinline__ void tile_tail_note(TileTailLds &T, const uint32_t blk, const unsigned long long mask) { T.mask[blk] = mask; }
+__device__ __forceinline__ void tile_tail_note(TileTailLds &T, const uint32_t blk, const uint32_t rank, const bool first, const uint32_t tile, const uint32_t total, const uint32_t n_slots) {
+    T.rank[blk] = rank;
+    if (first) { T.tile = tile; T.total = total; T.n_slots = n_slots; }
+}
+__device__ __forceinline__ void tile_tail_phase(const GateArgs &a, const TileTailArgs &t, const GateLds &L, TileTailLds &T) {
+    const uint32_t tid = threadIdx.x;
+    __syncthreads();
+    const uint32_t tile = T.tile, total = T.total, stride = T.n_slots, t0 = tile * TILE;
+    uint32_t *const cnt_p = t.ev_tile_cnt + (uint64_t)tile * EV_CNT_STRIDE;
+    const uint32_t list_lo = t.ev_tile_off[tile], cap_tile = t.ev_tile_off[tile + 1u] - list_lo;
+    const uint32_t n_all = *cnt_p, n_ev = min(n_all, cap_tile);
+    const uint32_t base = total ? L.base : 0u; const unsigned long long cell0 = total ? L.cell : 0ull;
+    const bool fits = total != 0u && stride - 1u < TT_CELLS && (uint64_t)base + total <= a.cap_out && cell0 + (unsigned long long)total * stride <= a.cap_cells;
+    if (fits) {
+        {
+            const uint32_t p0 = (uint32_t)GATE_PPT * tid, sh = p0 & 63u;
+            const unsigned long long w = T.mask[p0 >> 6];
+            uint32_t bits = (uint32_t)(w >> sh) & 0xffu, r = T.rank[p0 >> 6] + (uint32_t)__popcll(w & ((1ull << sh) - 1ull));
+            while (bits) { const uint32_t j = (uint32_t)__builtin_ctz(bits); bits &= bits - 1u; if (r < TILE) T.pos[r] = (uint16_t)(p0 + j); ++r; }
+        }
+        const uint32_t ps = t.tile_pair_start[tile], np = t.tile_pair_start[tile + 1u] - ps;
+        uint32_t nb_max = TT_CELLS / stride;
+        if ((stride & 7u) && nb_max >= 8u) nb_max &= ~7u;
+        const uint32_t ngrp = np >= (uint32_t)GATE_NT || np == 0u ? 1u : (uint32_t)GATE_NT / np;
+        const uint32_t grp = ngrp == 1u ? 0u : tid / np, k0 = ngrp == 1u ? tid : tid - grp * np;
+        const Pair32 *const list = t.events + list_lo;
+        uint16_t *const cov16 = reinterpret_cast<uint16_t *>(T.cells[0]);
+        for (uint32_t s_lo = 0; s_lo < total; s_lo += nb_max) {
+            const uint32_t nb = min(nb_max, total - s_lo), ncell = nb * stride;
+            __syncthreads();
+            {
+                const uint32_t n16 = (ncell + 7u) >> 3;
+                const uint4 z = make_uint4(0u, 0u, 0u, 0u);
+#pragma unroll
+                for (uint32_t c = 0; c < 5u; ++c) for (uint32_t i = tid; i < n16; i += (uint32_t)GATE_NT) reinterpret_cast<uint4 *>(T.cells[c])[i] = z;
+            }
+            __syncthreads();
+            if (grp < ngrp) for (uint32_t k = k0; k < np; k += (uint32_t)GATE_NT) {
+                const uint32_t slot = t.pairs[ps + k].pad >> 8;
+                const uint8_t *const row = t.spill + (uint64_t)(ps + k) * TILE;
+                if (slot >= stride) continue;
+#pragma unroll 4
+                for (uint32_t j = grp; j < nb; j += ngrp) cov16[j * stride + slot] = (uint16_t)row[T.pos[s_lo + j]];
+            }
+            for (uint32_t i0 = 0; i0 < n_ev; i0 += 4u * (uint32_t)GATE_NT) {
+                Pair32 e[4];
+#pragma unroll
+                for (uint32_t u = 0; u < 4u; ++u) { const uint32_t i = i0 + u * (uint32_t)GATE_NT + tid; e[u] = list[min(i, n_ev - 1u)]; }
+#pragma unroll
+                for (uint32_t u = 0; u < 4u; ++u) {
+                    const uint32_t off = e[u].x - t0;
+                    if (i0 + u * (uint32_t)GATE_NT + tid >= n_ev || off >= TILE) continue;
+                    const unsigned long long w = T.mask[off >> 6], bit = 1ull << (off & 63u);
+                    if (!(w & bit)) continue;
+                    const uint32_t j = T.rank[off >> 6] + (uint32_t)__popcll(w & (bit - 1ull)) - s_lo, slot = e[u].y >> 18;
+                    if (j >= nb || slot >= stride) continue;
+                    const uint32_t c = j * stride + slot;
+                    atomicAdd(&T.cells[1u + ((e[u].y >> 16) & 3u)][c >> 1], (e[u].y & 0xffffu) << (16u * (c & 1u)));
+                }
+            }
+            __syncthreads();
+            const unsigned long long first = cell0 + (unsigned long long)s_lo * stride;
+            const bool wide = (first & 7ull) == 0ull;
+            const uint32_t n16 = wide ? ncell >> 3 : 0u;
+#pragma unroll
+            for (uint32_t c = 0; c < 5u; ++c) {
+                uint16_t *const dst = (c == 0u ? a.cov_col : a.ncol + (uint64_t)(c - 1u) * a.cap_cells) + first;
+                for (uint32_t i = tid; i < n16; i += (uint32_t)GATE_NT) reinterpret_cast<uint4 *>(dst)[i] = reinterpret_cast<const uint4 *>(T.cells[c])[i];
+                for (uint32_t i = 8u * n16 + tid; i < ncell; i += (uint32_t)GATE_NT) dst[i] = reinterpret_cast<const uint16_t *>(T.cells[c])[i];
+            }
+        }
+    }
+    __syncthreads();
+    if (tid == 0u) {
+        t.ev_tile_last[tile] = n_all;
+        if (n_all) { *cnt_p = 0u; atomicAdd(&a.counters[0], n_all); if (n_all > cap_tile) atomicAdd(&a.counters[CNT_EV_OVER], 1u); }
+    }
+    if (t.host_cnt) {
+        if (tid == 0u) { __threadfence(); T.pad = atomicAdd(t.done, 1u); }
+        __syncthreads();
+        if (T.pad == gridDim.x - 1u) {
+            __threadfence();
+            for (uint32_t i = tid; i < CNT_WORDS; i += (uint32_t)GATE_NT)
+                t.host_cnt[i] = __hip_atomic_load(&a.counters[i], __ATOMIC_RELAXED, __HIP_MEMORY_SCOPE_AGENT);
+            if (tid == 0u) *t.done = 0u;
+            __threadfence_system();
+        }
+    }
+}
+template <bool WIDE_TOT>
+__global__ __launch_bounds__(GATE_NT) void msnv_tile_tail(const GateArgs a, const TileTailArgs t) {
+    __shared__ GateLds L;
+    __shared__ TileTailLds T;
+    gate_sites_body<false, WIDE_TOT, false, true>(a, L, &t, &T);
 }
 
 __global__ __launch_bounds__(256) void msnv_decide_sites(const SiteRec *sites, const uint32_t *unc_sites, uint32_t *counters, uint32_t cap_sites, uint32_t cap_out,
@@ -2390,7 +2531,7 @@
     void *ptrs[] = {d.hdr, d.hdr8, d.hdr4, d.hdr8m, d.merged_groups, d.tile_pair_merged, d.blk, d.seq, d.qual, d.s_read_base, d.s_seq_base, d.ref4, d.ref_lc, d.pairs,
                     d.tile_pair_start, d.work, d.chunks, d.tile_vbeg, d.tile_vend, d.tot, d.part, d.tile_slot_start, d.tile_slot_u16, d.tile_slot_wide, d.slot_off, d.spill, d.events, d.overflow, d.counters, d.ind4, d.tile_dirty, d.unc_sites, d.site_row, d.gate_tiles,
                     d.sites, d.tile_site_base, d.tile_site_cnt, d.tile_cell_base, d.tile_nslots, d.ncol, d.cov_col, d.site_flags, d.site_elig,
-                    d.cov_iv, d.s_cov_base, d.cov_pairs, d.cov_work, d.tile_len, d.tile_contig_dev, d.cov_acc, d.tile_stage, d.tile_stage_idx, d.alt.tile_stage, d.gate_tiles_dense, d.gate_tiles_staged, d.gather_tiles};
+                    d.ev_tile_cnt, d.alt.ev_tile_cnt, d.ev_tile_off, d.ev_tile_last, d.cov_iv, d.s_cov_base, d.cov_pairs, d.cov_work, d.tile_len, d.tile_contig_dev, d.cov_acc, d.tile_stage, d.tile_stage_idx, d.alt.tile_stage, d.gate_tiles_dense, d.gate_tiles_staged, d.gather_tiles};
     auto in_block = [&](void *p) { for (const auto &b : d.blocks) if ((char *)p >= (char *)b.first && (char *)p < (char *)b.first + b.second) return true; return false; };
     for (void *p : ptrs) if (p && !in_block(p)) dev_free(p);
     void *aptrs[] = {d.ann.seg_beg, d.ann.seg_end, d.ann.seg_gene, d.ann.genes, d.ann.contigs, d.ann.codons, d.ann.out, d.ann.err};
@@ -2428,8 +2569,46 @@
 
 static inline uint32_t *stage_ovf_list(const DeviceCols &d) { return d.tile_stage ? reinterpret_cast<uint32_t *>(d.tile_stage + d.n_active_tiles) : nullptr; }
 
+static int ensure_tile_lists(DeviceCols &d) {
+    d.tile_tail_ok = d.n_active_tiles && d.n_tiles && !d.n_merged_groups && !d.n_work_merged && !d.n_fused_tiles && !d.allele_planes && !d.any_split &&
+                     d.n_work == d.n_work_narrow + d.n_work_merged && ((d.n_samples + 7u) & ~7u) <= TT_CELLS;
+    if (d.tile_lists_refused) d.tile_tail_ok = false;
+    if (!d.tile_tail_ok || d.ev_tile_cnt) return MSNV_OK;
+    const uint64_t bytes = ((uint64_t)d.n_tiles + 1) * EV_CNT_STRIDE * sizeof(uint32_t);
+    if (int rc = dev_alloc((void **)&d.ev_tile_cnt, bytes, &d.device_bytes)) return rc;
+    if (int rc = dev_memset(d.ev_tile_cnt, 0, bytes)) return rc;
+    if (int rc = dev_alloc((void **)&d.ev_tile_off, ((uint64_t)d.n_tiles + 1) * sizeof(uint32_t), &d.device_bytes)) return rc;
+    if (int rc = dev_alloc((void **)&d.ev_tile_last, ((uint64_t)d.n_tiles + 1) * sizeof(uint32_t), &d.device_bytes)) return rc;
+    if (int rc = dev_memset(d.ev_tile_last, 0, ((uint64_t)d.n_tiles + 1) * sizeof(uint32_t))) return rc;
+    std::vector<uint32_t> active(d.n_active_tiles), off((size_t)d.n_tiles + 1, 0u);
+    if (int rc = dev_download(active.data(), d.active_tiles, active.size() * sizeof(uint32_t))) return rc;
+    const uint32_t each = d.cap_events / d.n_active_tiles;
+    for (uint32_t t : active) if (t < d.n_tiles) off[t + 1] = each;
+    for (size_t t = 0; t < d.n_tiles; ++t) off[t + 1] += off[t];
+    return dev_upload(d.ev_tile_off, off.data(), off.size() * sizeof(uint32_t));
+}
+
+int dev_resize_tile_lists(DeviceCols &d) {
+    if (!d.ev_tile_cnt || !d.tile_lists_short) return MSNV_OK;
+    d.tile_lists_short = false;
+    std::vector<uint32_t> last((size_t)d.n_tiles + 1), off((size_t)d.n_tiles + 1, 0u), active(d.n_active_tiles);
+    if (int rc = dev_download(last.data(), d.ev_tile_last, last.size() * sizeof(uint32_t))) return rc;
+    if (int rc = dev_download(active.data(), d.active_tiles, active.size() * sizeof(uint32_t))) return rc;
+    std::vector<uint8_t> holds_work((size_t)d.n_tiles, 0);
+    for (uint32_t t : active) if (t < d.n_tiles) holds_work[t] = 1;
+    uint64_t total = 0;
+    for (size_t t = 0; t < d.n_tiles; ++t) { if (last[t] || holds_work[t]) total += (uint64_t)last[t] + last[t] / 4 + 64; off[t + 1] = (uint32_t)std::min<uint64_t>(total, 0xffffffffull); }
+    if (total > 0x7fffffffull) { d.tile_lists_refused = true; d.tile_tail_ok = false; return MSNV_OK; }
+    if (total > d.cap_events) {
+        dev_free(d.events); d.events = nullptr;
+        d.cap_events = (uint32_t)total;
+        if (int rc = dev_alloc((void **)&d.events, (uint64_t)d.cap_events * sizeof(Pair32), &d.device_bytes)) return rc;
+    }
+    return dev_upload(d.ev_tile_off, off.data(), off.size() * sizeof(uint32_t));
+}
+
 static int enqueue_pass(DeviceCols &d, const msnv_params &p, hipStream_t st, hipEvent_t ev_begin, hipEvent_t ev_pile0, hipEvent_t ev_pile1,
-                        hipEvent_t ev3, hipEvent_t ev4, uint32_t *host_cnt, hipEvent_t wait_before_pileup = nullptr) {
+                        hipEvent_t ev3, hipEvent_t ev4, uint32_t *host_cnt, hipEvent_t wait_before_pileup = nullptr, uint32_t *mapped_cnt = nullptr) {
     const uint64_t npos = (uint64_t)d.n_tiles * TILE;
     if (p.min_baseq != d.qlow_cutoff) return fail(MSNV_EINVAL, "the dataset's quality column was packed for -Q %d, the pass asks for -Q %d", d.qlow_cutoff, p.min_baseq);
     if (ev_begin) HIP_TRY(hipEventRecord(ev_begin, st));
@@ -2437,13 +2616,15 @@
     d.cnt_parity ^= 1u;
     if (wait_before_pileup) HIP_TRY(hipStreamWaitEvent(st, wait_before_pileup, 0));
     const uint32_t use_stage = (d.n_fused_tiles && !d.fuse_disabled && p.calling_threshold >= 1) ? 1u : 0u;
+    const bool tile_route = d.tile_tail_ok && d.ev_tile_cnt && !knob::tile_tail_off();
+    d.pass_tile_route = tile_route;
     HIP_TRY(hipEventRecord(ev_pile0, st));
     if (d.n_work) {
         PileupArgs a;
         a.hdr = d.hdr; a.hdr8 = d.hdr8; a.hdr4 = d.hdr4; a.blk = d.blk; a.seq = d.seq; a.qual = d.qual;
         a.s_read_base = d.s_read_base; a.s_seq_base = d.s_seq_base;
         a.ref4 = d.ref4; a.pairs = d.pairs; a.work = d.work; a.chunks = d.chunks; a.tot = d.tot; a.part = d.part; a.npos = npos; a.spill = d.spill; a.aspill = d.aspill;
-        a.events = d.events; a.cap_events = d.cap_events / EV_LISTS; a.ev_count = nullptr; a.overflow = d.overflow; a.cap_overflow = d.cap_overflow;
+        a.events = d.events; a.cap_events = d.cap_events / EV_LISTS; a.ev_count = nullptr; a.ev_tile_cnt = tile_route ? d.ev_tile_cnt : nullptr; a.ev_tile_off = d.ev_tile_off; a.overflow = d.overflow; a.cap_overflow = d.cap_overflow;
         a.counters = counters; a.min_baseq = (uint32_t)std::max(0, p.min_baseq);
         a.ind4 = d.ind4; a.unc_bits = d.unc_bits; a.slot_dirty = d.tile_dirty; a.min_snvs = (uint32_t)std::max(0, p.calling_threshold);
         a.n_fused_lo = d.n_work_narrow + d.n_work_merged - (use_stage ? d.n_work_fused : 0u); a.min_cov = p.min_coverage; a.min_frac = p.min_fraction; a.ref_lc = d.ref_lc; a.tile_vbeg = d.tile_vbeg; a.tile_vend = d.tile_vend;
@@ -2485,7 +2666,12 @@
         if (use_stage) g.gate_tiles = reinterpret_cast<const GateTile *>(d.gate_tiles_dense);
         g.n_active = n_dense;
         g.zero_next = 1u; g.tile_list = nullptr; g.solo_cells = 0u;
-        if (n_dense) {
+        if (tile_route) {
+            g.aspill = nullptr;
+            const TileTailArgs tt{d.events, d.ev_tile_cnt, d.ev_tile_off, d.ev_tile_last, d.pairs, d.tile_pair_start, d.spill, d.ev_tile_cnt + (uint64_t)d.n_tiles * EV_CNT_STRIDE, mapped_cnt};
+            if (d.wide_tot) hipLaunchKernelGGL(msnv_tile_tail<true>, dim3(n_dense), dim3(GATE_NT), 0, st, g, tt);
+            else hipLaunchKernelGGL(msnv_tile_tail<false>, dim3(n_dense), dim3(GATE_NT), 0, st, g, tt);
+        } else if (n_dense) {
             g.tiles_per_wg = knob::gate_tiles(n_dense >= 32768u ? 8u : n_dense >= 8192u ? 4u : 1u, (int)GATE_MAX_TILES);
             const dim3 grid((n_dense + g.tiles_per_wg - 1) / g.tiles_per_wg);
             g.aspill = d.aspill;
@@ -2522,7 +2708,7 @@
         HIP_TRY(hipGetLastError());
     } else HIP_TRY(hipMemsetAsync(counters_next, 0, CNT_WORDS * sizeof(uint32_t), st));
     if (ev3) HIP_TRY(hipEventRecord(ev3, st));
-    if (d.n_active_tiles) {
+    if (d.n_active_tiles && !tile_route) {
         TailArgs ta;
         ta.sites = d.sites; ta.tile_site_base = d.tile_site_base; ta.tile_site_cnt = d.tile_site_cnt; ta.tile_pair_start = d.tile_pair_start;
         ta.pairs = d.pairs; ta.spill = d.spill; ta.ncol = d.ncol; ta.cov_col = d.cov_col; ta.cap_out = cap_out; ta.active_tiles = d.gather_tiles;
@@ -2553,16 +2739,19 @@
                            d.ncol, CellMap{d.tile_site_base, d.tile_cell_base, d.tile_nslots, d.cap_cells, d.site_row}, p.calling_threshold, p.min_fraction, d.site_flags);
         HIP_TRY(hipGetLastError());
     }
-    HIP_TRY(hipMemcpyAsync(host_cnt, counters, CNT_WORDS * sizeof(uint32_t), hipMemcpyDeviceToHost, st));
+    if (!(tile_route && mapped_cnt)) HIP_TRY(hipMemcpyAsync(host_cnt, counters, CNT_WORDS * sizeof(uint32_t), hipMemcpyDeviceToHost, st));
     return MSNV_OK;
 }
 
 static int check_counts(DeviceCols &d, const uint32_t *cnt, RunCounts *counts) {
     RunCounts c{cnt[0], cnt[1], cnt[2], cnt[3], (uint64_t)cnt[CNT_CELLS] | (uint64_t)cnt[CNT_CELLS + 1] << 32};
+    bool ev_over = !d.pass_tile_route && c.n_events > d.cap_events / EV_LISTS * EV_LISTS;
+    d.tile_lists_short = d.pass_tile_route && cnt[CNT_EV_OVER] != 0u;
+    if (d.tile_lists_short) ev_over = true;
     d.last_sites = c.n_sites; d.last_cells = c.n_cells;
     if (counts) *counts = c;
     d.last_ovf_tiles = cnt[CNT_STAGE];
-    if (c.n_events > d.cap_events / EV_LISTS * EV_LISTS || c.n_overflow > d.cap_overflow || c.n_sites > d.cap_sites || c.n_sites > d.cap_out_sites || c.n_cells > d.cap_cells)
+    if (ev_over || c.n_overflow > d.cap_overflow || c.n_sites > d.cap_sites || c.n_sites > d.cap_out_sites || c.n_cells > d.cap_cells)
         return fail_quiet(MSNV_ECAPACITY, "device buffer too small: events %u/%u overflow %u/%u sites %u/%u out %u/%llu cells %llu/%llu",
                           c.n_events, d.cap_events, c.n_overflow, d.cap_overflow, c.n_sites, d.cap_sites, c.n_sites,
                           (unsigned long long)d.cap_out_sites, (unsigned long long)c.n_cells, (unsigned long long)d.cap_cells);
@@ -2578,6 +2767,7 @@
     }
     const bool phase_times = knob::phase_times();
     if (int rc = ensure_out(d, std::max<uint64_t>(d.last_sites + d.last_sites / 2, 4096), std::max<uint64_t>(d.last_cells + d.last_cells / 2, 1u << 18))) return rc;
+    if (int rc = ensure_tile_lists(d)) return rc;
     uint32_t cnt[CNT_WORDS] = {0};
     if (int rc = enqueue_pass(d, p, st, ev[0], ev[1], ev[2], phase_times ? ev[3] : nullptr, phase_times ? ev[4] : nullptr, cnt)) return rc;
     HIP_TRY(hipEventRecord(ev[5], st));
@@ -2602,8 +2792,8 @@
 static int ensure_alt(DeviceCols &d) {
     DeviceCols::AltBufs &a = d.alt;
     const uint64_t npos = (uint64_t)d.n_tiles * TILE;
-    if (a.tot && a.cap_events == d.cap_events && a.cap_overflow == d.cap_overflow && a.cap_sites == d.cap_sites && a.cap_out_sites == d.cap_out_sites && a.cap_cells == d.cap_cells) return MSNV_OK;
-    void *old[] = {a.aspill, a.tot, a.part, a.spill, a.events, a.overflow, a.counters, a.ind4, a.tile_dirty, a.unc_sites, a.site_row, a.sites, a.tile_site_base, a.tile_site_cnt, a.tile_cell_base, a.ncol, a.cov_col, a.site_flags, a.site_elig, a.site_bits, a.site_rank, a.tile_stage};
+    if (a.tot && a.cap_events == d.cap_events && a.cap_overflow == d.cap_overflow && a.cap_sites == d.cap_sites && a.cap_out_sites == d.cap_out_sites && a.cap_cells == d.cap_cells && (!d.ev_tile_cnt || a.ev_tile_cnt)) return MSNV_OK;
+    void *old[] = {a.aspill, a.tot, a.part, a.spill, a.events, a.overflow, a.counters, a.ind4, a.tile_dirty, a.unc_sites, a.site_row, a.sites, a.tile_site_base, a.tile_site_cnt, a.tile_cell_base, a.ncol, a.cov_col, a.site_flags, a.site_elig, a.site_bits, a.site_rank, a.tile_stage, a.ev_tile_cnt};
     for (void *p : old) dev_free(p);
     a = DeviceCols::AltBufs{};
     if (int rc = dev_alloc((void **)&a.tot, std::max<uint64_t>(1, 4 * npos) * sizeof(uint32_t), &d.device_bytes)) return rc;
@@ -2626,6 +2816,10 @@
     if (int rc = dev_alloc((void **)&a.ind4, (npos / 8 + npos / 32 + 2) * sizeof(uint32_t), &d.device_bytes)) return rc;
     if (int rc = dev_memset(a.ind4, 0, (npos / 8 + npos / 32 + 2) * sizeof(uint32_t))) return rc;
     a.unc_bits = a.ind4 + npos / 8 + 1; a.cnt_parity = 0;
+    if (d.ev_tile_cnt) {
+        if (int rc = dev_alloc((void **)&a.ev_tile_cnt, ((uint64_t)d.n_tiles + 1) * EV_CNT_STRIDE * sizeof(uint32_t), &d.device_bytes)) return rc;
+        if (int rc = dev_memset(a.ev_tile_cnt, 0, ((uint64_t)d.n_tiles + 1) * EV_CNT_STRIDE * sizeof(uint32_t))) return rc;
+    }
     if (int rc = dev_alloc((void **)&a.site_bits, (npos / 64 + 1) * sizeof(unsigned long long), &d.device_bytes)) return rc;
     if (int rc = dev_alloc((void **)&a.site_rank, (npos / 64 + 1) * sizeof(uint32_t), &d.device_bytes)) return rc;
     if (int rc = dev_alloc((void **)&a.tile_site_base, ((uint64_t)d.n_tiles + 1) * sizeof(uint32_t), &d.device_bytes)) return rc;
@@ -2652,6 +2846,7 @@
     std::swap(d.tile_site_base, a.tile_site_base); std::swap(d.tile_site_cnt, a.tile_site_cnt); std::swap(d.tile_cell_base, a.tile_cell_base); std::swap(d.ncol, a.ncol); std::swap(d.cov_col, a.cov_col);
     std::swap(d.site_flags, a.site_flags); std::swap(d.site_elig, a.site_elig); std::swap(d.ind4, a.ind4); std::swap(d.unc_bits, a.unc_bits); std::swap(d.cnt_parity, a.cnt_parity);
     if (a.tile_stage) std::swap(d.tile_stage, a.tile_stage);
+    if (a.ev_tile_cnt) std::swap(d.ev_tile_cnt, a.ev_tile_cnt);
     std::swap(d.tile_dirty, a.tile_dirty); std::swap(d.unc_sites, a.unc_sites); std::swap(d.site_row, a.site_row); std::swap(d.site_bits, a.site_bits); std::swap(d.site_rank, a.site_rank);
 }
 
@@ -2660,8 +2855,10 @@
     if (d.pinned_cnt_cap < (size_t)n) {
         if (d.pinned_cnt) (void)hipHostFree(d.pinned_cnt);
         d.pinned_cnt = nullptr; d.pinned_cnt_cap = 0;
-        if (hipHostMalloc((void **)&d.pinned_cnt, (size_t)n * CNT_WORDS * sizeof(uint32_t), hipHostMallocDefault) != hipSuccess) return fail(MSNV_ENOMEM, "pinned host memory for %d counter blocks", n);
+        d.pinned_cnt_dev = nullptr;
+        if (hipHostMalloc((void **)&d.pinned_cnt, (size_t)n * CNT_WORDS * sizeof(uint32_t), hipHostMallocMapped) != hipSuccess) return fail(MSNV_ENOMEM, "pinned host memory for %d counter blocks", n);
         d.pinned_cnt_cap = (size_t)n;
+        if (hipHostGetDevicePointer((void **)&d.pinned_cnt_dev, d.pinned_cnt, 0) != hipSuccess) { (void)hipGetLastError(); d.pinned_cnt_dev = nullptr; }
     }
     return MSNV_OK;
 }
@@ -2670,6 +2867,7 @@
     if (n <= 0) return MSNV_OK;
     hipStream_t s0 = (hipStream_t)stream_, s1 = s0;
     if (int rc = ensure_out(d, std::max<uint64_t>(d.last_sites + d.last_sites / 2, 4096), std::max<uint64_t>(d.last_cells + d.last_cells / 2, 1u << 18))) return rc;
+    if (int rc = ensure_tile_lists(d)) return rc;
     if (overlap && n > 1) {
         if (!d.stream2) { hipStream_t s; HIP_TRY(hipStreamCreateWithFlags(&s, hipStreamNonBlocking)); d.stream2 = s; }
         s1 = (hipStream_t)d.stream2;
@@ -2686,7 +2884,8 @@
     for (int i = 0; i < n && !rc && he == hipSuccess; ++i) {
         hipStream_t st = (i & 1) ? s1 : s0;
         if (two && (i & 1) != (swapped ? 1 : 0)) { swap_sets(d); swapped = !swapped; }
-        rc = enqueue_pass(d, p, st, i == 0 ? ev[0] : nullptr, ev[4 * i + 1], ev[4 * i + 2], nullptr, nullptr, cnt + (size_t)CNT_WORDS * i, (two && i > 0) ? ev[4 * (i - 1) + 2] : nullptr);
+        rc = enqueue_pass(d, p, st, i == 0 ? ev[0] : nullptr, ev[4 * i + 1], ev[4 * i + 2], nullptr, nullptr, cnt + (size_t)CNT_WORDS * i, (two && i > 0) ? ev[4 * (i - 1) + 2] : nullptr,
+                          d.pinned_cnt_dev ? d.pinned_cnt_dev + (size_t)CNT_WORDS * i : nullptr);
     }
     if (!rc && he == hipSuccess) he = hipEventRecord(ev[4 * n], s0);
     if (!rc && he == hipSuccess) he = hipEventRecord(ev[4 * n + 1], s1);
diff --git a/metasnv_amd/csrc/knobs.h b/metasnv_amd/csrc/knobs.h
--- a/metasnv_amd/csrc/knobs.h
+++ b/metasnv_amd/csrc/knobs.h
@@ -77,6 +77,7 @@
 inline int merged_gather() { const char c = first("MSNV_MERGED_GATHER"); return c == 'b' ? 1 : c == 'w' ? 2 : 0; }
 inline bool lean_off() { return first("MSNV_LEAN") == '0'; }
 inline uint32_t gate_tiles(uint32_t by_tiles, int max_tiles) { int v = 0; return int_of("MSNV_GATE_TILES", &v) ? (uint32_t)std::min(max_tiles, std::max(1, v)) : by_tiles; }
+inline bool tile_tail_off() { return first("MSNV_TILE_TAIL") == '0'; }
 inline uint32_t tail_skip() { static const uint32_t v = (uint32_t)int_or("MSNV_TAIL_SKIP", 0); return v; }
 inline uint32_t scatter_blocks(uint32_t default_blocks) { static const uint32_t v = [&] { int x = 0; return int_of("MSNV_SCATTER_BLOCKS", &x) ? (uint32_t)std::max(1, x) : default_blocks; }(); return v; }
 inline bool phase_times() { static const bool on = first("MSNV_PHASE_TIMES") == '1'; return on; }
diff --git a/profiles/tail_gaps.py b/profiles/tail_gaps.py
--- /dev/null
+++ b/profiles/tail_gaps.py
@@ -0,0 +1,35 @@
+import csv
+import glob
+import os
+import statistics
+import sys
+
+
+def rows(pattern):
+    out = []
+    for p in glob.glob(os.path.join(sys.argv[1], "**", pattern), recursive=True):
+        out += list(csv.DictReader(open(p)))
+    return out
+
+
+ops = []
+for r in rows("*kernel_trace.csv"):
+    ops.append((int(r["Start_Timestamp"]), int(r["End_Timestamp"]), r["Kernel_Name"].split("(")[0].split("<")[0].replace("msnv::", "").replace("void ", "")))
+for r in rows("*memory_copy_trace.csv"):
+    ops.append((int(r["Start_Timestamp"]), int(r["End_Timestamp"]), "copy " + r.get("Direction", "?")))
+ops.sort()
+starts = [i for i, o in enumerate(ops) if o[2].startswith("msnv_pileup_tiles")]
+starts = starts[-31:]
+per, gaps, tails = {}, [], []
+for a, b in zip(starts, starts[1:]):
+    g = 0
+    for i in range(a, b):
+        per.setdefault(ops[i][2], []).append((ops[i][1] - ops[i][0]) / 1e3)
+        g += max(0, ops[i + 1][0] - ops[i][1]) / 1e3
+    gaps.append(g)
+    tails.append((ops[b][0] - ops[a][1]) / 1e3)
+print("passes", len(gaps))
+for k, v in sorted(per.items()):
+    print("%-40s n/pass %.1f  median %.2f us  mean %.2f us" % (k, len(v) / max(1, len(gaps)), statistics.median(v), statistics.mean(v)))
+print("in-stream gaps per pass: median %.2f us" % statistics.median(gaps))
+print("pileup end -> next pileup start: median %.2f us" % statistics.median(tails))
```
